# Ulixes-8/UNet-Implementations

Measured on NVIDIA B200. Metric: our_unet_512_train_images_per_sec, higher is better.
Workload: dtype bf16

## Files before the change

### include/b200unet.h

```cpp
#ifndef B200UNET_H_
#define B200UNET_H_

#include <stdint.h>

#ifdef __cplusplus
extern "C" {
#endif

#define B200UNET_VERSION 100

int b200unet_version(void);
const char* b200unet_last_error(void);
long long b200unet_launch_count(void);
int b200unet_device_ok(void);
int b200unet_set_reserved_sms(int n);
int b200unet_set_pdl(int on);

typedef struct {
  const void* x;
  int64_t x_pitch;
  const void* w;
  void* y;
  int64_t y_pitch;
  float* stats;
  int N, H, W, Cin, Cout, stride;
} b200unet_conv_fprop_args;
int b200unet_conv_fprop_partials(int N, int OH, int OW, int Cout);
int b200unet_conv_fprop(const b200unet_conv_fprop_args* a, void* stream);

typedef struct {
  const void* dy;
  int64_t dy_pitch;
  const void* wt;
  void* dx;
  int64_t dx_pitch;
  int N, H, W, Cin, Cout, stride;
  const void* bs_y;
  int64_t bs_y_pitch;
  const float* bs_a;
  const float* bs_b;
  float bs_slope;
  float* bs_part;
  void* dx2;
  int64_t dx2_pitch;
  int dx_split;
} b200unet_conv_dgrad_args;
int b200unet_conv_dgrad(const b200unet_conv_dgrad_args* a, void* stream);
int b200unet_conv_dgrad_bwd_slots(int N, int H, int W, int Cin, int Cout, int stride);

typedef struct {
  const void* x;
  int64_t x_pitch;
  const void* dy;
  int64_t dy_pitch;
  float* dw;
  float* workspace;
  int64_t workspace_bytes;
  int N, H, W, Cin, Cout, stride;
} b200unet_conv_wgrad_args;
int64_t b200unet_conv_wgrad_workspace(int N, int H, int W, int Cin, int Cout, int stride);
int b200unet_conv_wgrad(const b200unet_conv_wgrad_args* a, void* stream);

int b200unet_conv_fprop_simt_partials(int OH, int OW);
int b200unet_conv_fprop_simt(const b200unet_conv_fprop_args* a, void* stream);
int b200unet_conv_dgrad_simt(const b200unet_conv_dgrad_args* a, void* stream);
int b200unet_conv_wgrad_simt(const b200unet_conv_wgrad_args* a, void* stream);

int b200unet_pack_conv_weights(const float* w_oihw, void* w_fprop, void* w_dgrad, int Cout, int Cin, void* stream);

int b200unet_stem_partials(int H, int W);
int b200unet_stem_fprop(const float* img_nchw, const float* w_oihw, void* y, int64_t y_pitch, float* stats, int N,
                        int H, int W, void* stream);
int64_t b200unet_stem_wgrad_workspace(int N, int H, int W);
int b200unet_stem_wgrad(const float* img_nchw, const void* dy, int64_t dy_pitch, float* dw_oihw, float* workspace,
                        int64_t workspace_bytes, int N, int H, int W, void* stream);

int b200unet_in_finalize(const float* stats, int P, const float* gamma, const float* beta, const float* drop_scale,
                         float eps, float* mean, float* rstd, float* a, float* b, int N, int C, int64_t HW,
                         void* stream);
int b200unet_in_apply(const void* y, int64_t y_pitch, const float* a, const float* b, float slope, void* z,
                      int64_t z_pitch, int N, int64_t HW, int C, void* stream);
typedef struct {
  const void* dz;
  int64_t dz_pitch;
  const void* dz2;
  int64_t dz2_pitch;
  const void* y;
  int64_t y_pitch;
  const float* a;
  const float* b;
  const float* mean;
  const float* rstd;
  const float* drop_scale;
  const float* gamma;
  float slope;
  void* dy;
  int64_t dy_pitch;
  float* dgamma;
  float* dbeta;
  float* workspace;
  int64_t workspace_bytes;
  int N;
  int64_t HW;
  int C;
  const float* ext_part;
  int ext_P;
  const float* ext_part2;
  int ext_P2;
  int defer_params;
} b200unet_in_bwd_args;
int64_t b200unet_in_backward_workspace(int N, int64_t HW, int C);
int b200unet_in_backward(const b200unet_in_bwd_args* a, void* stream);
int b200unet_in_bwd_params(const float* workspace, int N, int64_t HW, int C, float* dgamma, float* dbeta, void* stream);

int b200unet_upsample2x_fwd(const void* x, int64_t x_pitch, void* out, int64_t out_pitch, int N, int H, int W, int C,
                            void* stream);
int b200unet_upsample2x_bwd(const void* dout, int64_t dout_pitch, void* dx, int64_t dx_pitch, int N, int H, int W,
                            int C, void* stream);

int b200unet_head_fwd(const void* z, int64_t z_pitch, const float* w, const float* bias, float* logits_nchw, int N,
                      int64_t HW, int C, int K, void* stream);
int64_t b200unet_head_bwd_workspace(int N, int64_t HW, int C, int K);
int b200unet_head_bwd(const float* dlogits_nchw, const void* z, int64_t z_pitch, const float* w, void* dz,
                      int64_t dz_pitch, float* dw, float* db, float* workspace, int64_t workspace_bytes, int N,
                      int64_t HW, int C, int K, void* stream);

int64_t b200unet_loss_workspace(int N, int64_t HW);
int b200unet_loss_fwd(const float* logits_nchw, const int64_t* target, const float* class_weights, int dynamic,
                      float weight_ce, float weight_dice, int ignore_index, float smooth, float* loss_out,
                      float* tables, float* workspace, int64_t workspace_bytes, int N, int64_t HW, void* stream);
int b200unet_loss_bwd(const float* logits_nchw, const int64_t* target, const float* tables, const float* grad_out,
                      float weight_ce, float weight_dice, int ignore_index, float* dlogits_nchw, int N, int64_t HW,
                      void* stream);
int b200unet_loss_fwd_u8(const float* logits_nchw, const uint8_t* target, const float* class_weights, int dynamic,
                         float weight_ce, float weight_dice, int ignore_index, float smooth, float* loss_out,
                         float* tables, float* workspace, int64_t workspace_bytes, int N, int64_t HW, void* stream);
int b200unet_loss_bwd_u8(const float* logits_nchw, const uint8_t* target, const float* tables, const float* grad_out,
                         float weight_ce, float weight_dice, int ignore_index, float* dlogits_nchw, int N, int64_t HW,
                         void* stream);

int b200unet_nchw_f32_to_nhwc_bf16(const float* src, void* dst, int64_t dst_pitch, int N, int C, int64_t HW,
                                   void* stream);
int b200unet_nhwc_bf16_to_nchw_f32(const void* src, int64_t src_pitch, float* dst, int N, int C, int64_t HW,
                                   void* stream);

int b200unet_conv_dgrad_s2_supported(int Cin, int Cout);
int b200unet_pack_s2_dgrad_weights(const void* wt, void* ws, int Cin, int Cout, void* stream);
int b200unet_conv_dgrad_s2(const b200unet_conv_dgrad_args* a, void* stream);

int b200unet_upsample2x_norm_fwd(const void* y, int64_t y_pitch, const float* a, const float* b, float slope, void* out,
                                 int64_t out_pitch, int N, int H, int W, int C, void* stream);
int b200unet_head_norm_fwd(const void* y, int64_t y_pitch, const float* a, const float* b, float slope, const float* w,
                           const float* bias, float* logits_nchw, int N, int64_t HW, int C, int K, void* stream);
int b200unet_head_norm_bwd(const float* dlogits_nchw, const void* y, int64_t y_pitch, const float* a, const float* b,
                           float slope, const float* w, void* dz, int64_t dz_pitch, float* dw, float* db,
                           float* workspace, int64_t workspace_bytes, int N, int64_t HW, int C, int K, void* stream);
int b200unet_head_bwd_stat_slots(int N, int64_t HW);
int b200unet_head_norm_bwd_stats(const float* dlogits_nchw, const void* y, int64_t y_pitch, const float* a, const float* b,
                                 float slope, const float* w, void* dz, int64_t dz_pitch, float* dw, float* db,
                                 float* workspace, int64_t workspace_bytes, float* bwd_part, int N, int64_t HW, int C, int K,
                                 void* stream);
int b200unet_head_norm_bwd_stats_f32(const float* dlogits_nchw, const void* y, int64_t y_pitch, const float* a,
                                     const float* b, float slope, const float* w, void* dz, int64_t dz_pitch, float* dw,
                                     float* db, float* workspace, int64_t workspace_bytes, float* bwd_part, int N,
                                     int64_t HW, int C, int K, void* stream);
int b200unet_upsample2x_norm_fwd_f32(const void* y, int64_t y_pitch, const float* a, const float* b, float slope,
                                     void* out, int64_t out_pitch, int N, int H, int W, int C, void* stream);
int b200unet_head_norm_fwd_f32(const void* y, int64_t y_pitch, const float* a, const float* b, float slope,
                               const float* w, const float* bias, float* logits_nchw, int N, int64_t HW, int C, int K,
                               void* stream);
int b200unet_head_norm_bwd_f32(const float* dlogits_nchw, const void* y, int64_t y_pitch, const float* a, const float* b,
                               float slope, const float* w, void* dz, int64_t dz_pitch, float* dw, float* db,
                               float* workspace, int64_t workspace_bytes, int N, int64_t HW, int C, int K, void* stream);

int b200unet_pack_conv_weights_f32(const float* w_oihw, void* w_fprop, void* w_dgrad, int Cout, int Cin, void* stream);
int b200unet_conv_fprop_f32(const b200unet_conv_fprop_args* a, void* stream);
int b200unet_conv_dgrad_f32(const b200unet_conv_dgrad_args* a, void* stream);
int b200unet_conv_wgrad_f32(const b200unet_conv_wgrad_args* a, void* stream);
int b200unet_in_apply_f32(const void* y, int64_t y_pitch, const float* a, const float* b, float slope, void* z,
                          int64_t z_pitch, int N, int64_t HW, int C, void* stream);
int b200unet_in_backward_f32(const b200unet_in_bwd_args* a, void* stream);
int b200unet_upsample2x_fwd_f32(const void* x, int64_t x_pitch, void* out, int64_t out_pitch, int N, int H, int W,
                                int C, void* stream);
int b200unet_upsample2x_bwd_f32(const void* dout, int64_t dout_pitch, void* dx, int64_t dx_pitch, int N, int H,
                                int W, int C, void* stream);
int b200unet_head_fwd_f32(const void* z, int64_t z_pitch, const float* w, const float* bias, float* logits_nchw,
                          int N, int64_t HW, int C, int K, void* stream);
int b200unet_head_bwd_f32(const float* dlogits_nchw, const void* z, int64_t z_pitch, const float* w, void* dz,
                          int64_t dz_pitch, float* dw, float* db, float* workspace, int64_t workspace_bytes, int N,
                          int64_t HW, int C, int K, void* stream);
int b200unet_nchw_f32_to_nhwc_f32(const float* src, void* dst, int64_t dst_pitch, int N, int C, int64_t HW,
                                  void* stream);

int b200unet_image_to_nhwc32_bf16(const float* src, void* dst, int N, int C, int64_t HW, void* stream);

int b200unet_preprocess_u8(const void* image_u8_nhwc, const void* mask_u8, float* image_out_nchw, int64_t* mask_out,
                           const float* mean3, const float* std3, int N, int64_t HW, void* stream);
int b200unet_preprocess_u8_nhwc32(const void* image_u8_nhwc, void* dst_nhwc32, const float* mean3, const float* std3, int N,
                                  int64_t HW, void* stream);
int b200unet_sgd_max_tensors(void);
int b200unet_sgd_nesterov_step(float* const* params, const float* const* grads, float* const* momentum_bufs,
                               const int64_t* numels, int count, float lr, float momentum, float weight_decay,
                               int nesterov, int first_step, void* stream);
typedef struct {
  int64_t offset;
  int32_t numel;
  int32_t flags;
  int32_t first_block;
  int32_t cout, cin, ksize;
  int32_t cout_pad, cin_pad;
  void* wf;
  void* wd;
  void* ws;
} b200unet_flat_tensor;
int b200unet_sgd_flat_block_elems(void);
int b200unet_sgd_flat_step(const b200unet_flat_tensor* table_dev, int count, int total_blocks, float* master,
                           const float* grad, float* momentum_buf, float lr, float momentum, float weight_decay,
                           int nesterov, float grad_scale, const float* lr_dev ,
                           void* stream);
int b200unet_adam_flat_step(const b200unet_flat_tensor* table_dev, int count, int total_blocks, float* master,
                            const float* grad, float* exp_avg, float* exp_avg_sq, float* steps, float* scalars_ws,
                            double lr, const double* lr_dev, double beta1, double beta2, double eps, double weight_decay,
                            int decoupled, float grad_scale, void* stream);
int b200unet_argmax_counts(const float* logits_nchw, const int64_t* target, int ignore_index, int64_t* pred_or_null,
                           int64_t* counts9, int N, int64_t HW, void* stream);

int b200unet_recon_head_fwd(const void* y, int64_t y_pitch, const float* bias, float* out_nchw, int N, int64_t HW,
                            int K, void* stream);
int b200unet_recon_head_fwd_f32(const void* y, int64_t y_pitch, const float* bias, float* out_nchw, int N, int64_t HW,
                                int K, void* stream);
int64_t b200unet_recon_head_bwd_workspace(int N, int64_t HW);
int b200unet_recon_head_bwd(const float* dout_nchw, const float* out_nchw, void* dpre, int64_t dpre_pitch, int Cpad,
                            float* db, float* workspace, int64_t workspace_bytes, int N, int64_t HW, int K,
                            void* stream);
int b200unet_recon_head_bwd_f32(const float* dout_nchw, const float* out_nchw, void* dpre, int64_t dpre_pitch, int Cpad,
                                float* db, float* workspace, int64_t workspace_bytes, int N, int64_t HW, int K,
                                void* stream);
int64_t b200unet_mse_workspace(int64_t n);
int b200unet_mse_fwd(const float* a, const float* b, float* loss_out, float* workspace, int64_t workspace_bytes,
                     int64_t n, void* stream);
int b200unet_mse_bwd(const float* a, const float* b, const float* grad_out, float* da, int64_t n, void* stream);

#ifdef __cplusplus
}
#endif
#endif
```

### unet-implementations_b200/_lib.py

```python
from __future__ import annotations

import ctypes
import os
from ctypes import POINTER, Structure, c_char_p, c_double, c_float, c_int, c_int64, c_void_p

_HERE = os.path.dirname(os.path.abspath(__file__))
LIB_PATH = os.environ.get("B200UNET_LIB") or os.path.join(_HERE, "libb200unet.so")

_lib = None


class ConvFpropArgs(Structure):
    _fields_ = [
        ("x", c_void_p), ("x_pitch", c_int64), ("w", c_void_p), ("y", c_void_p), ("y_pitch", c_int64),
        ("stats", c_void_p), ("N", c_int), ("H", c_int), ("W", c_int), ("Cin", c_int), ("Cout", c_int),
        ("stride", c_int),
    ]


class ConvDgradArgs(Structure):
    _fields_ = [
        ("dy", c_void_p), ("dy_pitch", c_int64), ("wt", c_void_p), ("dx", c_void_p), ("dx_pitch", c_int64),
        ("N", c_int), ("H", c_int), ("W", c_int), ("Cin", c_int), ("Cout", c_int), ("stride", c_int),
        ("bs_y", c_void_p), ("bs_y_pitch", c_int64), ("bs_a", c_void_p), ("bs_b", c_void_p), ("bs_slope", c_float),
        ("bs_part", c_void_p), ("dx2", c_void_p), ("dx2_pitch", c_int64), ("dx_split", c_int),
    ]


class ConvWgradArgs(Structure):
    _fields_ = [
        ("x", c_void_p), ("x_pitch", c_int64), ("dy", c_void_p), ("dy_pitch", c_int64), ("dw", c_void_p),
        ("workspace", c_void_p), ("workspace_bytes", c_int64), ("N", c_int), ("H", c_int), ("W", c_int),
        ("Cin", c_int), ("Cout", c_int), ("stride", c_int),
    ]


class InBwdArgs(Structure):
    _fields_ = [
        ("dz", c_void_p), ("dz_pitch", c_int64), ("dz2", c_void_p), ("dz2_pitch", c_int64), ("y", c_void_p),
        ("y_pitch", c_int64), ("a", c_void_p), ("b", c_void_p), ("mean", c_void_p), ("rstd", c_void_p),
        ("drop_scale", c_void_p), ("gamma", c_void_p), ("slope", c_float), ("dy", c_void_p), ("dy_pitch", c_int64),
        ("dgamma", c_void_p), ("dbeta", c_void_p), ("workspace", c_void_p), ("workspace_bytes", c_int64),
        ("N", c_int), ("HW", c_int64), ("C", c_int),
        ("ext_part", c_void_p), ("ext_P", c_int), ("ext_part2", c_void_p), ("ext_P2", c_int), ("defer_params", c_int),
    ]


class FlatTensor(Structure):
    _fields_ = [
        ("offset", c_int64), ("numel", c_int), ("flags", c_int), ("first_block", c_int), ("cout", c_int), ("cin", c_int),
        ("ksize", c_int), ("cout_pad", c_int), ("cin_pad", c_int), ("wf", c_void_p), ("wd", c_void_p), ("ws", c_void_p),
    ]


_P, _I, _L, _F, _D = c_void_p, c_int, c_int64, c_float, c_double

SIGNATURES = {
    "b200unet_version": (c_int, []),
    "b200unet_last_error": (c_char_p, []),
    "b200unet_device_ok": (c_int, []),
    "b200unet_set_reserved_sms": (c_int, [_I]),
    "b200unet_set_pdl": (c_int, [_I]),
    "b200unet_launch_count": (c_int64, []),
    "b200unet_conv_fprop_partials": (c_int, [_I, _I, _I, _I]),
    "b200unet_conv_fprop": (c_int, [POINTER(ConvFpropArgs), _P]),
    "b200unet_conv_dgrad": (c_int, [POINTER(ConvDgradArgs), _P]),
    "b200unet_conv_dgrad_bwd_slots": (c_int, [_I, _I, _I, _I, _I, _I]),
    "b200unet_conv_dgrad_s2_supported": (c_int, [_I, _I]),
    "b200unet_pack_s2_dgrad_weights": (c_int, [_P, _P, _I, _I, _P]),
    "b200unet_conv_dgrad_s2": (c_int, [POINTER(ConvDgradArgs), _P]),
    "b200unet_conv_wgrad_workspace": (c_int64, [_I, _I, _I, _I, _I, _I]),
    "b200unet_conv_wgrad": (c_int, [POINTER(ConvWgradArgs), _P]),
    "b200unet_conv_fprop_simt_partials": (c_int, [_I, _I]),
    "b200unet_conv_fprop_simt": (c_int, [POINTER(ConvFpropArgs), _P]),
    "b200unet_conv_dgrad_simt": (c_int, [POINTER(ConvDgradArgs), _P]),
    "b200unet_conv_wgrad_simt": (c_int, [POINTER(ConvWgradArgs), _P]),
    "b200unet_pack_conv_weights": (c_int, [_P, _P, _P, _I, _I, _P]),
    "b200unet_stem_partials": (c_int, [_I, _I]),
    "b200unet_stem_fprop": (c_int, [_P, _P, _P, _L, _P, _I, _I, _I, _P]),
    "b200unet_stem_wgrad_workspace": (c_int64, [_I, _I, _I]),
    "b200unet_stem_wgrad": (c_int, [_P, _P, _L, _P, _P, _L, _I, _I, _I, _P]),
    "b200unet_in_finalize": (c_int, [_P, _I, _P, _P, _P, _F, _P, _P, _P, _P, _I, _I, _L, _P]),
    "b200unet_in_apply": (c_int, [_P, _L, _P, _P, _F, _P, _L, _I, _L, _I, _P]),
    "b200unet_in_backward_workspace": (c_int64, [_I, _L, _I]),
    "b200unet_in_backward": (c_int, [POINTER(InBwdArgs), _P]),
    "b200unet_in_bwd_params": (c_int, [_P, _I, _L, _I, _P, _P, _P]),
    "b200unet_upsample2x_fwd": (c_int, [_P, _L, _P, _L, _I, _I, _I, _I, _P]),
    "b200unet_upsample2x_bwd": (c_int, [_P, _L, _P, _L, _I, _I, _I, _I, _P]),
    "b200unet_head_fwd": (c_int, [_P, _L, _P, _P, _P, _I, _L, _I, _I, _P]),
    "b200unet_head_bwd_workspace": (c_int64, [_I, _L, _I, _I]),
    "b200unet_head_bwd": (c_int, [_P, _P, _L, _P, _P, _L, _P, _P, _P, _L, _I, _L, _I, _I, _P]),
    "b200unet_loss_workspace": (c_int64, [_I, _L]),
    "b200unet_loss_fwd": (c_int, [_P, _P, _P, _I, _F, _F, _I, _F, _P, _P, _P, _L, _I, _L, _P]),
    "b200unet_loss_bwd": (c_int, [_P, _P, _P, _P, _F, _F, _I, _P, _I, _L, _P]),
    "b200unet_loss_fwd_u8": (c_int, [_P, _P, _P, _I, _F, _F, _I, _F, _P, _P, _P, _L, _I, _L, _P]),
    "b200unet_loss_bwd_u8": (c_int, [_P, _P, _P, _P, _F, _F, _I, _P, _I, _L, _P]),
    "b200unet_nchw_f32_to_nhwc_bf16": (c_int, [_P, _P, _L, _I, _I, _L, _P]),
    "b200unet_nhwc_bf16_to_nchw_f32": (c_int, [_P, _L, _P, _I, _I, _L, _P]),
    "b200unet_pack_conv_weights_f32": (c_int, [_P, _P, _P, _I, _I, _P]),
    "b200unet_conv_fprop_f32": (c_int, [POINTER(ConvFpropArgs), _P]),
    "b200unet_conv_dgrad_f32": (c_int, [POINTER(ConvDgradArgs), _P]),
    "b200unet_conv_wgrad_f32": (c_int, [POINTER(ConvWgradArgs), _P]),
    "b200unet_in_apply_f32": (c_int, [_P, _L, _P, _P, _F, _P, _L, _I, _L, _I, _P]),
    "b200unet_in_backward_f32": (c_int, [POINTER(InBwdArgs), _P]),
    "b200unet_upsample2x_fwd_f32": (c_int, [_P, _L, _P, _L, _I, _I, _I, _I, _P]),
    "b200unet_upsample2x_bwd_f32": (c_int, [_P, _L, _P, _L, _I, _I, _I, _I, _P]),
    "b200unet_head_fwd_f32": (c_int, [_P, _L, _P, _P, _P, _I, _L, _I, _I, _P]),
    "b200unet_head_bwd_f32": (c_int, [_P, _P, _L, _P, _P, _L, _P, _P, _P, _L, _I, _L, _I, _I, _P]),
    "b200unet_nchw_f32_to_nhwc_f32": (c_int, [_P, _P, _L, _I, _I, _L, _P]),
    "b200unet_image_to_nhwc32_bf16": (c_int, [_P, _P, _I, _I, _L, _P]),
    "b200unet_upsample2x_norm_fwd": (c_int, [_P, _L, _P, _P, _F, _P, _L, _I, _I, _I, _I, _P]),
    "b200unet_upsample2x_norm_fwd_f32": (c_int, [_P, _L, _P, _P, _F, _P, _L, _I, _I, _I, _I, _P]),
    "b200unet_head_norm_fwd": (c_int, [_P, _L, _P, _P, _F, _P, _P, _P, _I, _L, _I, _I, _P]),
    "b200unet_head_norm_fwd_f32": (c_int, [_P, _L, _P, _P, _F, _P, _P, _P, _I, _L, _I, _I, _P]),
    "b200unet_head_norm_bwd": (c_int, [_P, _P, _L, _P, _P, _F, _P, _P, _L, _P, _P, _P, _L, _I, _L, _I, _I, _P]),
    "b200unet_head_norm_bwd_f32": (c_int, [_P, _P, _L, _P, _P, _F, _P, _P, _L, _P, _P, _P, _L, _I, _L, _I, _I, _P]),
    "b200unet_head_bwd_stat_slots": (c_int, [_I, _L]),
    "b200unet_head_norm_bwd_stats": (c_int, [_P, _P, _L, _P, _P, _F, _P, _P, _L, _P, _P, _P, _L, _P, _I, _L, _I, _I, _P]),
    "b200unet_head_norm_bwd_stats_f32": (c_int, [_P, _P, _L, _P, _P, _F, _P, _P, _L, _P, _P, _P, _L, _P, _I, _L, _I, _I, _P]),
    "b200unet_preprocess_u8": (c_int, [_P, _P, _P, _P, _P, _P, _I, _L, _P]),
    "b200unet_preprocess_u8_nhwc32": (c_int, [_P, _P, _P, _P, _I, _L, _P]),
    "b200unet_sgd_flat_block_elems": (c_int, []),
    "b200unet_sgd_flat_step": (c_int, [_P, _I, _I, _P, _P, _P, _F, _F, _F, _I, _F, _P, _P]),
    "b200unet_sgd_max_tensors": (c_int, []),
    "b200unet_sgd_nesterov_step": (c_int, [_P, _P, _P, _P, _I, _F, _F, _F, _I, _I, _P]),
    "b200unet_adam_flat_step": (c_int, [_P, _I, _I, _P, _P, _P, _P, _P, _P, _D, _P, _D, _D, _D, _D, _I, _F, _P]),
    "b200unet_argmax_counts": (c_int, [_P, _P, _I, _P, _P, _I, _L, _P]),
    "b200unet_recon_head_fwd": (c_int, [_P, _L, _P, _P, _I, _L, _I, _P]),
    "b200unet_recon_head_fwd_f32": (c_int, [_P, _L, _P, _P, _I, _L, _I, _P]),
    "b200unet_recon_head_bwd_workspace": (c_int64, [_I, _L]),
    "b200unet_recon_head_bwd": (c_int, [_P, _P, _P, _L, _I, _P, _P, _L, _I, _L, _I, _P]),
    "b200unet_recon_head_bwd_f32": (c_int, [_P, _P, _P, _L, _I, _P, _P, _L, _I, _L, _I, _P]),
    "b200unet_mse_workspace": (c_int64, [_L]),
    "b200unet_mse_fwd": (c_int, [_P, _P, _P, _P, _L, _L, _P]),
    "b200unet_mse_bwd": (c_int, [_P, _P, _P, _P, _L, _P]),
}

_VALUE_FUNCS = {
    "b200unet_version", "b200unet_last_error", "b200unet_device_ok", "b200unet_set_reserved_sms", "b200unet_set_pdl", "b200unet_launch_count", "b200unet_conv_fprop_partials",
    "b200unet_conv_fprop_simt_partials", "b200unet_sgd_max_tensors", "b200unet_sgd_flat_block_elems", "b200unet_head_bwd_stat_slots", "b200unet_conv_dgrad_bwd_slots", "b200unet_recon_head_bwd_workspace",
    "b200unet_conv_dgrad_s2_supported",
    "b200unet_mse_workspace",
    "b200unet_conv_wgrad_workspace", "b200unet_stem_partials", "b200unet_stem_wgrad_workspace",
    "b200unet_in_backward_workspace", "b200unet_head_bwd_workspace", "b200unet_loss_workspace",
}


def load():
    global _lib
    if _lib is not None:
        return _lib
    if not os.path.exists(LIB_PATH):
        raise RuntimeError(
            f"b200unet: {LIB_PATH} is not built. Run `python -c 'import __graft_entry__ as g; g.build()'` "
            "(or `make -C unet-implementations_b200/csrc`). There is no CPU or PyTorch fallback."
        )
    lib = ctypes.CDLL(LIB_PATH)
    for name, (res, args) in SIGNATURES.items():
        fn = getattr(lib, name)
        fn.restype = res
        fn.argtypes = args
    _lib = lib
    return lib


def last_error() -> str:
    msg = load().b200unet_last_error()
    return msg.decode("utf-8", "replace") if msg else ""


class EventProfiler:

    def __init__(self):
        self.pairs = {}

    def totals_ms(self):
        return {k: (sum(a.elapsed_time(b) for a, b in v), len(v)) for k, v in self.pairs.items()}


PROFILER = None


def call(name: str, *args):
    fn = getattr(load(), name)
    prof = PROFILER
    if prof is not None and name not in _VALUE_FUNCS:
        import torch
        e0 = torch.cuda.Event(enable_timing=True)
        e1 = torch.cuda.Event(enable_timing=True)
        e0.record()
        rc = fn(*args)
        e1.record()
        prof.pairs.setdefault(name, []).append((e0, e1))
    else:
        rc = fn(*args)
    if name in _VALUE_FUNCS:
        return rc
    if rc != 0:
        raise RuntimeError(f"{name} failed ({rc}): {last_error()}")
    return 0
```

### unet-implementations_b200/csrc/head_loss.cu

```cuda
#include "common.cuh"
#include "ptx.cuh"
#include "vec8.cuh"

namespace b200 {

constexpr int kNC = 3;
constexpr int kLossThreads = 256;
constexpr int kLossPxPerThread = 8;
constexpr int kLossVals = 4 * kNC;

__device__ __forceinline__ float block_sum(float v, float* scratch) {
#pragma unroll
  for (int o = 16; o > 0; o >>= 1) v += __shfl_xor_sync(0xffffffffu, v, o);
  const int lane = threadIdx.x & 31, warp = threadIdx.x >> 5;
  __syncthreads();
  if (lane == 0) scratch[warp] = v;
  __syncthreads();
  float s = 0.f;
  if (threadIdx.x == 0)
    for (int w = 0; w < (blockDim.x >> 5); ++w) s += scratch[w];
  return s;
}

template <typename TT>
// ... 19 lines not shown
  } else {
#pragma unroll
    for (int j = 0; j < 4; ++j) {
      const bool in = px + j < HW;
#pragma unroll
      for (int c = 0; c < 3; ++c) a[c][j] = in ? z0[c * HW + px + j] : 0.f;
      long long q = in ? static_cast<long long>(tg[px + j]) : -1;
      t[j] = (q < -(1ll << 30) || q > (1ll << 30)) ? (1 << 30) + 1 : static_cast<int>(q);
      if (!in) t[j] = -2;
    }
  }
}

template <typename TT>
__global__ void __launch_bounds__(kLossThreads) loss_fwd_kernel(const float* __restrict__ logits,
                                                                 const TT* __restrict__ target, int ignore_index,
                                                                 float* __restrict__ part, int64_t HW) {
  pdl_launch_dependents();
  pdl_wait();
  __shared__ float scratch[kLossThreads / 32][kLossVals];
  const int n = blockIdx.y;
  const float* z0 = logits + static_cast<int64_t>(n) * kNC * HW;
  const TT* tg = target + static_cast<int64_t>(n) * HW;
  const bool vec = (HW & 3) == 0;
  float acc[kLossVals];
#pragma unroll
  for (int i = 0; i < kLossVals; ++i) acc[i] = 0.f;
  const int64_t base = static_cast<int64_t>(blockIdx.x) * kLossThreads * kLossPxPerThread;
  constexpr int kIters = kLossPxPerThread / 4;
  float a[kIters][3][4];
  int t[kIters][4];
  bool live[kIters];
#pragma unroll
  for (int k = 0; k < kIters; ++k) {
    const int64_t px = base + (static_cast<int64_t>(k) * kLossThreads + threadIdx.x) * 4;
    live[k] = px < HW;
    if (live[k]) load_px4<TT>(z0, tg, HW, px, vec, a[k], t[k]);
  }
#pragma unroll
  for (int k = 0; k < kIters; ++k) {
    if (!live[k]) continue;
    const int64_t px = base + (static_cast<int64_t>(k) * kLossThreads + threadIdx.x) * 4;
#pragma unroll
    for (int j = 0; j < 4; ++j) {
      const int tj = t[k][j];
      if (tj == ignore_index || (!vec && px + j >= HW)) continue;
      const float a0 = a[k][0][j], a1 = a[k][1][j], a2 = a[k][2][j];
      const float m = fmaxf(a0, fmaxf(a1, a2));
      const float e0 = expf(a0 - m), e1 = expf(a1 - m), e2 = expf(a2 - m);
      const float se = e0 + e1 + e2;
      const float inv = 1.f / se;
      const float p0 = e0 * inv, p1 = e1 * inv, p2 = e2 * inv;
      const float lse = m + logf(se);
      acc[9] += p0;
      acc[10] += p1;
      acc[11] += p2;
      if (tj == 0) { acc[0] += 1.f; acc[3] += lse - a0; acc[6] += p0; }
      else if (tj == 1) { acc[1] += 1.f; acc[4] += lse - a1; acc[7] += p1; }
      else if (tj == 2) { acc[2] += 1.f; acc[5] += lse - a2; acc[8] += p2; }
    }
  }
  const int lane = threadIdx.x & 31, warp = threadIdx.x >> 5;
#pragma unroll
  for (int i = 0; i < kLossVals; ++i) {
    float v = acc[i];
#pragma unroll
    for (int o = 16; o > 0; o >>= 1) v += __shfl_xor_sync(0xffffffffu, v, o);
    if (lane == 0) scratch[warp][i] = v;
  }
  __syncthreads();
  if (threadIdx.x < kLossVals) {
    float s = 0.f;
#pragma unroll
    for (int w = 0; w < kLossThreads / 32; ++w) s += scratch[w][threadIdx.x];
    part[(static_cast<int64_t>(n) * gridDim.x + blockIdx.x) * kLossVals + threadIdx.x] = s;
  }
}

__global__ void loss_finalize_kernel(const float* __restrict__ part, int blocks, const float* __restrict__ class_w,
                                     int dynamic, float weight_ce, float weight_dice, float smooth,
                                     float* __restrict__ loss_out, float* __restrict__ tables, int N) {
  pdl_launch_dependents();
  pdl_wait();
  extern __shared__ double sred[];
  double* dterm = sred + N * kLossVals;
  const int lane = threadIdx.x & 31, warp = threadIdx.x >> 5, nwarps = blockDim.x >> 5;
  constexpr int UV = 4;
  const int total = N * kLossVals;
  for (int i = warp * UV; i < total; i += nwarps * UV) {
    double s[UV];
    const float* src[UV];
#pragma unroll
    for (int u = 0; u < UV; ++u) {
      const int iu = min(i + u, total - 1);
      const int b = iu / kLossVals, v = iu - b * kLossVals;
      src[u] = part + static_cast<int64_t>(b) * blocks * kLossVals + v;
      s[u] = 0.0;
    }
    for (int k = lane; k < blocks; k += 32) {
      float x[UV];
#pragma unroll
      for (int u = 0; u < UV; ++u) x[u] = src[u][static_cast<int64_t>(k) * kLossVals];
#pragma unroll
      for (int u = 0; u < UV; ++u) s[u] += x[u];
    }
#pragma unroll
    for (int u = 0; u < UV; ++u) {
#pragma unroll
      for (int o = 16; o > 0; o >>= 1) s[u] += __shfl_xor_sync(0xffffffffu, s[u], o);
      if (lane == 0 && i + u < total) sred[i + u] = s[u];
    }
  }
  __syncthreads();
  if (threadIdx.x < N * kNC) {
    const int b = threadIdx.x / kNC, c = threadIdx.x - b * kNC;
    const double T = sred[b * kLossVals + c];
    const double I = sred[b * kLossVals + 2 * kNC + c];
    const double Pc = sred[b * kLossVals + 3 * kNC + c];
    const double U = Pc + T + smooth;
    const double two_i = 2.0 * I + smooth;
    dterm[b * kNC + c] = two_i / U;
    tables[kNC + (b * 2 + 0) * kNC + c] = static_cast<float>(-(2.0 / (kNC * static_cast<double>(N))) / U);
    tables[kNC + (b * 2 + 1) * kNC + c] = static_cast<float>((1.0 / (kNC * static_cast<double>(N))) * two_i / (U * U));
  }
  __syncthreads();
  if (threadIdx.x != 0) return;
  double cnt[kNC] = {0, 0, 0}, S[kNC] = {0, 0, 0};
  for (int b = 0; b < N; ++b)
    for (int c = 0; c < kNC; ++c) {
      cnt[c] += sred[b * kLossVals + c];
      S[c] += sred[b * kLossVals + kNC + c];
    }
  float w[kNC];
  if (class_w && !dynamic) {
    for (int c = 0; c < kNC; ++c) w[c] = class_w[c];
  } else if (dynamic) {
    const float total = static_cast<float>(cnt[0] + cnt[1] + cnt[2]);
    float wsum = 0.f;
    for (int c = 0; c < kNC; ++c) {
      const float px = cnt[c] == 0.0 ? 1.f : static_cast<float>(cnt[c]);
      w[c] = total / px;
      wsum += w[c];
    }
    for (int c = 0; c < kNC; ++c) w[c] = w[c] * (static_cast<float>(kNC) / wsum);
  } else {
    for (int c = 0; c < kNC; ++c) w[c] = 1.f;
  }
  double num = 0.0, den = 0.0;
  for (int c = 0; c < kNC; ++c) {
    num += static_cast<double>(w[c]) * S[c];
    den += static_cast<double>(w[c]) * cnt[c];
  }
  const double ce = num / den;
  double dice_loss = 0.0;
  for (int c = 0; c < kNC; ++c) {
    double dsum = 0.0;
    for (int b = 0; b < N; ++b) dsum += dterm[b * kNC + c];
    dice_loss += 1.0 - dsum / N;
  }
  dice_loss /= kNC;
  for (int c = 0; c < kNC; ++c) tables[c] = static_cast<float>(w[c] / den);
  loss_out[0] = static_cast<float>(weight_ce * ce + weight_dice * dice_loss);
  loss_out[1] = static_cast<float>(ce);
  loss_out[2] = static_cast<float>(dice_loss);
}

template <typename TT>
__global__ void __launch_bounds__(kLossThreads) loss_bwd_kernel(const float* __restrict__ logits,
                                                                 const TT* __restrict__ target,
                                                                 const float* __restrict__ tables,
                                                                 const float* __restrict__ grad_out, float weight_ce,
                                                                 float weight_dice, int ignore_index,
                                                                 float* __restrict__ dlogits, int64_t HW) {
  pdl_launch_dependents();
  pdl_wait();
  const int n = blockIdx.y;
  const float gs = grad_out ? grad_out[0] : 1.f;
  const float wn0 = tables[0], wn1 = tables[1], wn2 = tables[2];
  const float* tb = tables + kNC + n * 2 * kNC;
  const float A0 = tb[0], A1 = tb[1], A2 = tb[2], B0 = tb[3], B1 = tb[4], B2 = tb[5];
  const float* z0 = logits + static_cast<int64_t>(n) * kNC * HW;
  float* d0 = dlogits + static_cast<int64_t>(n) * kNC * HW;
  const TT* tg = target + static_cast<int64_t>(n) * HW;
  const bool vec = (HW & 3) == 0;
  const int64_t base = static_cast<int64_t>(blockIdx.x) * kLossThreads * kLossPxPerThread;
  constexpr int kIters = kLossPxPerThread / 4;
  float a[kIters][3][4];
  int t[kIters][4];
  bool live[kIters];
#pragma unroll
  for (int k = 0; k < kIters; ++k) {
    const int64_t px = base + (static_cast<int64_t>(k) * kLossThreads + threadIdx.x) * 4;
    live[k] = px < HW;
    if (live[k]) load_px4<TT>(z0, tg, HW, px, vec, a[k], t[k]);
  }
#pragma unroll
  for (int k = 0; k < kIters; ++k) {
    if (!live[k]) continue;
    const int64_t px = base + (static_cast<int64_t>(k) * kLossThreads + threadIdx.x) * 4;
    float g[3][4];
#pragma unroll
    for (int j = 0; j < 4; ++j) {
      const int tj = t[k][j];
      float g0 = 0.f, g1 = 0.f, g2 = 0.f;
      if (tj != ignore_index) {
        const float a0 = a[k][0][j], a1 = a[k][1][j], a2 = a[k][2][j];
        const float m = fmaxf(a0, fmaxf(a1, a2));
        const float e0 = expf(a0 - m), e1 = expf(a1 - m), e2 = expf(a2 - m);
        const float inv = 1.f / (e0 + e1 + e2);
        const float p0 = e0 * inv, p1 = e1 * inv, p2 = e2 * inv;
        const float wt = tj == 0 ? wn0 : (tj == 1 ? wn1 : (tj == 2 ? wn2 : 0.f));
        const float G0 = B0 + (tj == 0 ? A0 : 0.f), G1 = B1 + (tj == 1 ? A1 : 0.f), G2 = B2 + (tj == 2 ? A2 : 0.f);
        const float gp = G0 * p0 + G1 * p1 + G2 * p2;
        g0 = weight_ce * wt * (p0 - (tj == 0 ? 1.f : 0.f)) + weight_dice * p0 * (G0 - gp);
        g1 = weight_ce * wt * (p1 - (tj == 1 ? 1.f : 0.f)) + weight_dice * p1 * (G1 - gp);
        g2 = weight_ce * wt * (p2 - (tj == 2 ? 1.f : 0.f)) + weight_dice * p2 * (G2 - gp);
      }
      g[0][j] = g0 * gs;
      g[1][j] = g1 * gs;
      g[2][j] = g2 * gs;
    }
    if (vec) {
#pragma unroll
      for (int c = 0; c < 3; ++c)
        *reinterpret_cast<float4*>(d0 + c * HW + px) = make_float4(g[c][0], g[c][1], g[c][2], g[c][3]);
    } else {
#pragma unroll
      for (int j = 0; j < 4; ++j)
        if (px + j < HW) {
          d0[px + j] = g[0][j];
          d0[HW + px + j] = g[1][j];
          d0[2 * HW + px + j] = g[2][j];
        }
    }
  }
}

constexpr int kHeadMaxC = 64;
constexpr int kHeadMaxK = 4;

template <typename T, int C, int K>
__global__ void __launch_bounds__(256) head_fwd_kernel(const T* __restrict__ z, int64_t zp,
                                                        const float* __restrict__ w, const float* __restrict__ bias,
                                                        float* __restrict__ logits, int64_t HW,
                                                        const float* __restrict__ na, const float* __restrict__ nb,
                                                        float slope) {
  pdl_launch_dependents();
  pdl_wait();
  constexpr int C8N = C / 8, L = 256 / C8N, kPix = 4;
  static_assert(C8N >= K && C8N <= 32 && (C8N & (C8N - 1)) == 0, "C/8 must be a power of two in [K, 32]");
  const int n = blockIdx.y;
  const int c8 = threadIdx.x % C8N, c0 = c8 * 8;
  float wr[K][8], av[8], bv[8];
#pragma unroll
  for (int k = 0; k < K; ++k)
#pragma unroll
    for (int i = 0; i < 8; ++i) wr[k][i] = __ldg(w + k * C + c0 + i);
  if (na) {
#pragma unroll
    for (int i = 0; i < 8; ++i) {
      av[i] = __ldg(na + n * C + c0 + i);
      bv[i] = __ldg(nb + n * C + c0 + i);
    }
  }
  const float my_bias = c8 < K ? __ldg(bias + c8) : 0.f;
  const T* zn = z + static_cast<int64_t>(n) * HW * zp + c0;
  float* ln = logits + static_cast<int64_t>(n) * K * HW;
  const int64_t base = static_cast<int64_t>(blockIdx.x) * (L * kPix) + threadIdx.x / C8N;
  Vec8<T> v[kPix];
#pragma unroll
  for (int u = 0; u < kPix; ++u)
    if (base + u * L < HW) v[u] = Vec8<T>::ld_stream(zn + (base + u * L) * zp);
#pragma unroll
  for (int u = 0; u < kPix; ++u) {
    const int64_t px = base + u * L;
    if (px >= HW) break;
    float zf[8], acc[K];
    v[u].unpack(zf);
    if (na) {
#pragma unroll
      for (int i = 0; i < 8; ++i) {
        const float t = fmaf(av[i], zf[i], bv[i]);
        zf[i] = t > 0.f ? t : t * slope;
      }
    }
#pragma unroll
    for (int k = 0; k < K; ++k) {
      float a = 0.f;
#pragma unroll
      for (int i = 0; i < 8; ++i) a = fmaf(wr[k][i], zf[i], a);
      acc[k] = a;
    }
#pragma unroll
    for (int m = 1; m < C8N; m <<= 1)
#pragma unroll
      for (int k = 0; k < K; ++k) acc[k] += __shfl_xor_sync(0xffffffffu, acc[k], m);
    float mine = acc[0];
#pragma unroll
    for (int k = 1; k < K; ++k) mine = c8 == k ? acc[k] : mine;
    if (c8 < K) ln[c8 * HW + px] = mine + my_bias;
  }
}

template <typename T, int C, int K, bool STATS>
__global__ void __launch_bounds__(256, sizeof(T) == 2 ? 2 : 1) head_bwd_kernel(const float* __restrict__ dl, const T* __restrict__ z,
                                                        int64_t zp, const float* __restrict__ w,
                                                        T* __restrict__ dz, int64_t dzp,
                                                        float* __restrict__ partial, int64_t HW,
                                                        const float* __restrict__ na, const float* __restrict__ nb,
                                                        float slope, float* __restrict__ tpart) {
  pdl_launch_dependents();
  pdl_wait();
  constexpr int C8N = C / 8;
  constexpr int L = 256 / C8N;
  static_assert(C8N >= 1 && C8N <= 32 && (C8N & (C8N - 1)) == 0, "C/8 must be a power of two <= 32");
  __shared__ float red[8][K * C + K + (STATS ? 2 * C : 0)];
  const int n = blockIdx.y;
  const int c8 = threadIdx.x % C8N, c0 = c8 * 8;
  float wr[K][8];
#pragma unroll
  for (int k = 0; k < K; ++k)
#pragma unroll
    for (int i = 0; i < 8; ++i) wr[k][i] = w[k * C + c0 + i];
  float av[8], bv[8];
  if (na) {
    const float4 a0 = __ldg(reinterpret_cast<const float4*>(na + n * C + c0)), a1 = __ldg(reinterpret_cast<const float4*>(na + n * C + c0) + 1);
    const float4 b0 = __ldg(reinterpret_cast<const float4*>(nb + n * C + c0)), b1 = __ldg(reinterpret_cast<const float4*>(nb + n * C + c0) + 1);
    av[0] = a0.x; av[1] = a0.y; av[2] = a0.z; av[3] = a0.w; av[4] = a1.x; av[5] = a1.y; av[6] = a1.z; av[7] = a1.w;
    bv[0] = b0.x; bv[1] = b0.y; bv[2] = b0.z; bv[3] = b0.w; bv[4] = b1.x; bv[5] = b1.y; bv[6] = b1.z; bv[7] = b1.w;
  }
  float aw[K][8], ab[K], t1[STATS ? 8 : 1], t2[STATS ? 8 : 1];
#pragma unroll
  for (int k = 0; k < K; ++k) {
    ab[k] = 0.f;
#pragma unroll
    for (int i = 0; i < 8; ++i) aw[k][i] = 0.f;
  }
#pragma unroll
  for (int i = 0; i < (STATS ? 8 : 1); ++i) t1[i] = t2[i] = 0.f;
  const float* dln = dl + static_cast<int64_t>(n) * K * HW;
  const T* zn = z + static_cast<int64_t>(n) * HW * zp + c0;
  T* dzn = dz + static_cast<int64_t>(n) * HW * dzp + c0;
  const int64_t stride = static_cast<int64_t>(gridDim.x) * L;
  constexpr int U = STATS ? 3 : 4;
  for (int64_t g0 = static_cast<int64_t>(blockIdx.x) * L + threadIdx.x / C8N; g0 < HW; g0 += U * stride) {
    float d[U][K];
    Vec8<T> zv[U];
#pragma unroll
    for (int u = 0; u < U; ++u) {
      const int64_t px = g0 + u * stride;
      if (px < HW) {
#pragma unroll
        for (int k = 0; k < K; ++k) d[u][k] = __ldg(dln + k * HW + px);
        zv[u] = Vec8<T>::ld_stream(zn + px * zp);
      }
    }
#pragma unroll
    for (int u = 0; u < U; ++u) {
      const int64_t px = g0 + u * stride;
      if (px >= HW) break;
      float zf[8], o[8];
      zv[u].unpack(zf);
#pragma unroll
      for (int k = 0; k < K; ++k) ab[k] += d[u][k];
#pragma unroll
      for (int i = 0; i < 8; ++i) {
        const float yraw = zf[i];
        float zact = yraw, sl = 1.f;
        if (na) {
          const float t = fmaf(av[i], yraw, bv[i]);
          sl = t > 0.f ? 1.f : slope;
          zact = t * sl;
        }
        float sacc = 0.f;
#pragma unroll
        for (int k = 0; k < K; ++k) {
          sacc = fmaf(wr[k][i], d[u][k], sacc);
          aw[k][i] = fmaf(d[u][k], zact, aw[k][i]);
        }
        o[i] = sacc;
        if (STATS) {
          const float gm = to_f32(from_f32<T>(sacc)) * sl;
          t1[i] += gm;
          t2[i] = fmaf(gm, yraw, t2[i]);
        }
      }
      Vec8<T>::st(dzn + px * dzp, o);
    }
  }
  const int lane = threadIdx.x & 31, warp = threadIdx.x >> 5;
#pragma unroll
  for (int m = C8N; m < 32; m <<= 1) {
#pragma unroll
    for (int k = 0; k < K; ++k) {
#pragma unroll
      for (int i = 0; i < 8; ++i) aw[k][i] += __shfl_xor_sync(0xffffffffu, aw[k][i], m);
      ab[k] += __shfl_xor_sync(0xffffffffu, ab[k], m);
    }
    if (STATS) {
#pragma unroll
      for (int i = 0; i < 8; ++i) {
        t1[i] += __shfl_xor_sync(0xffffffffu, t1[i], m);
        t2[i] += __shfl_xor_sync(0xffffffffu, t2[i], m);
      }
    }
  }
  if (lane < C8N) {
#pragma unroll
    for (int k = 0; k < K; ++k) {
#pragma unroll
      for (int i = 0; i < 8; ++i) red[warp][k * C + c0 + i] = aw[k][i];
      if (c8 == 0) red[warp][K * C + k] = ab[k];
    }
    if (STATS) {
#pragma unroll
      for (int i = 0; i < 8; ++i) {
        red[warp][K * C + K + 2 * (c0 + i)] = t1[i];
        red[warp][K * C + K + 2 * (c0 + i) + 1] = t2[i];
      }
    }
  }
  __syncthreads();
  const int64_t row = static_cast<int64_t>(n) * gridDim.x + blockIdx.x;
  for (int i = threadIdx.x; i < K * C + K + (STATS ? 2 * C : 0); i += 256) {
    float sacc = 0.f;
#pragma unroll
    for (int wv = 0; wv < 8; ++wv) sacc += red[wv][i];
    if (i < K * C + K) partial[row * (K * C + K) + i] = sacc;
    else tpart[row * (2 * C) + (i - (K * C + K))] = sacc;
  }
}

__global__ void __launch_bounds__(1024) head_bwd_finalize_kernel(const float* __restrict__ partial, int blocks, int KC,
                                                                  int K, float* __restrict__ dw, float* __restrict__ db) {
  pdl_launch_dependents();
  pdl_wait();
  const int lane = threadIdx.x & 31, warp = threadIdx.x >> 5;
  for (int i = warp; i < KC + K; i += 32) {
    double s = 0.0;
    for (int b = lane; b < blocks; b += 32) s += partial[static_cast<int64_t>(b) * (KC + K) + i];
#pragma unroll
    for (int o = 16; o > 0; o >>= 1) s += __shfl_xor_sync(0xffffffffu, s, o);
    if (lane == 0) {
      if (i < KC) dw[i] = static_cast<float>(s);
      else db[i - KC] = static_cast<float>(s);
    }
  }
}

template <typename T>
__global__ void __launch_bounds__(256) recon_head_fwd_kernel(const T* __restrict__ y, int64_t yp,
                                                              const float* __restrict__ bias, float* __restrict__ out,
                                                              int64_t HW, int K) {
  const int n = blockIdx.y;
  const int64_t px = static_cast<int64_t>(blockIdx.x) * 256 + threadIdx.x;
  if (px >= HW) return;
  const T* src = y + (static_cast<int64_t>(n) * HW + px) * yp;
  for (int k = 0; k < K; ++k) {
    const float v = to_f32(src[k]) + bias[k];
    out[(static_cast<int64_t>(n) * K + k) * HW + px] = 1.f / (1.f + expf(-v));
  }
}

template <typename T>
__global__ void __launch_bounds__(256) recon_head_bwd_kernel(const float* __restrict__ dout, const float* __restrict__ out,
                                                              T* __restrict__ dpre, int64_t dp, int Cpad,
                                                              float* __restrict__ partial, int64_t HW, int K) {
  __shared__ float scratch[8];
  const int n = blockIdx.y;
  float acc[4] = {0.f, 0.f, 0.f, 0.f};
  const int vecs = Cpad * static_cast<int>(sizeof(T)) / 16;
  for (int64_t px = static_cast<int64_t>(blockIdx.x) * 256 + threadIdx.x; px < HW; px += static_cast<int64_t>(gridDim.x) * 256) {
    float g[4] = {0.f, 0.f, 0.f, 0.f};
#pragma unroll
    for (int k = 0; k < 4; ++k)
      if (k < K) {
        const int64_t i = (static_cast<int64_t>(n) * K + k) * HW + px;
        const float o = __ldg(out + i);
        g[k] = __ldg(dout + i) * o * (1.f - o);
        acc[k] += g[k];
      }
    uint4* dst = reinterpret_cast<uint4*>(dpre + (static_cast<int64_t>(n) * HW + px) * dp);
    if (sizeof(T) == 2) {
      dst[0] = make_uint4(pack_bf16x2(g[0], g[1]), pack_bf16x2(g[2], g[3]), 0u, 0u);
    } else {
      dst[0] = make_uint4(__float_as_uint(g[0]), __float_as_uint(g[1]), __float_as_uint(g[2]), __float_as_uint(g[3]));
    }
    const uint4 z = make_uint4(0u, 0u, 0u, 0u);
    for (int v = 1; v < vecs; ++v) dst[v] = z;
  }
  for (int k = 0; k < K && k < 4; ++k) {
    const float v = block_sum(acc[k], scratch);
    if (threadIdx.x == 0) partial[(static_cast<int64_t>(n) * gridDim.x + blockIdx.x) * 4 + k] = v;
  }
}

__global__ void recon_head_bwd_finalize_kernel(const float* __restrict__ partial, int rows, int K, float* __restrict__ db) {
  const int k = threadIdx.x;
  if (k >= K) return;
  double s = 0.0;
  for (int r = 0; r < rows; ++r) s += partial[static_cast<int64_t>(r) * 4 + k];
  db[k] = static_cast<float>(s);
}

__global__ void __launch_bounds__(256) mse_fwd_kernel(const float* __restrict__ a, const float* __restrict__ b,
                                                       float* __restrict__ partial, int64_t n) {
  __shared__ float scratch[8];
  float acc = 0.f;
  for (int64_t i = static_cast<int64_t>(blockIdx.x) * 256 + threadIdx.x; i < n; i += static_cast<int64_t>(gridDim.x) * 256) {
    const float d = a[i] - b[i];
    acc = fmaf(d, d, acc);
  }
  const float v = block_sum(acc, scratch);
  if (threadIdx.x == 0) partial[blockIdx.x] = v;
}
__global__ void mse_finalize_kernel(const float* __restrict__ partial, int blocks, double inv_n, float* __restrict__ out) {
  if (threadIdx.x != 0) return;
  double s = 0.0;
  for (int i = 0; i < blocks; ++i) s += partial[i];
  out[0] = static_cast<float>(s * inv_n);
}
__global__ void __launch_bounds__(256) mse_bwd_kernel(const float* __restrict__ a, const float* __restrict__ b,
                                                       const float* __restrict__ gout, float scale,
                                                       float* __restrict__ da, int64_t n) {
  const float g = (gout ? gout[0] : 1.f) * scale;
  for (int64_t i = static_cast<int64_t>(blockIdx.x) * 256 + threadIdx.x; i < n; i += static_cast<int64_t>(gridDim.x) * 256)
    da[i] = g * (a[i] - b[i]);
}



}

using namespace b200;

extern "C" int64_t b200unet_loss_workspace(int N, int64_t HW) {
  const int64_t blocks = ceil_div64(HW, kLossThreads * kLossPxPerThread);
  return static_cast<int64_t>(N) * blocks * kLossVals * 4;
}

template <typename TT>
static int loss_fwd_impl(const float* logits_nchw, const TT* target, const float* class_weights, int dynamic,
                         float weight_ce, float weight_dice, int ignore_index, float smooth, float* loss_out,
                         float* tables, float* workspace, int64_t workspace_bytes, int N, int64_t HW, void* stream) {
  B200_CHECK_ARG(logits_nchw && target && loss_out && tables && workspace, "loss_fwd: null pointer");
  B200_CHECK_ARG(N > 0 && HW > 0, "loss_fwd: empty batch");
  B200_CHECK_ARG(workspace_bytes >= b200unet_loss_workspace(N, HW), "loss_fwd: workspace too small");
  const int blocks = static_cast<int>(ceil_div64(HW, kLossThreads * kLossPxPerThread));
  cudaStream_t st = static_cast<cudaStream_t>(stream);
  launch_k(loss_fwd_kernel<TT>, dim3(blocks, N), dim3(kLossThreads), 0, st, logits_nchw, target, ignore_index, workspace, HW);
  B200_LAUNCH_CHECK("loss_fwd_kernel");
  const size_t smem = static_cast<size_t>(N) * (kLossVals + kNC) * sizeof(double);
  B200_CHECK_ARG(N * kNC <= 1024, "loss_fwd: batch %d too large for the finalize kernel", N);
  B200_CHECK_ARG(smem <= 48 * 1024, "loss_fwd: batch %d too large for the finalize kernel", N);
  launch_k(loss_finalize_kernel, dim3(1), dim3(1024), smem, st, workspace, blocks, class_weights, dynamic, weight_ce, weight_dice, smooth,
                                             loss_out, tables, N);
  B200_LAUNCH_CHECK("loss_finalize_kernel");
  return 0;
}

template <typename TT>
static int loss_bwd_impl(const float* logits_nchw, const TT* target, const float* tables, const float* grad_out,
                         float weight_ce, float weight_dice, int ignore_index, float* dlogits_nchw, int N, int64_t HW,
                         void* stream) {
  B200_CHECK_ARG(logits_nchw && target && tables && dlogits_nchw, "loss_bwd: null pointer");
  const int blocks = static_cast<int>(ceil_div64(HW, kLossThreads * kLossPxPerThread));
  launch_k(loss_bwd_kernel<TT>, dim3(blocks, N), dim3(kLossThreads), 0, static_cast<cudaStream_t>(stream), 
      logits_nchw, target, tables, grad_out, weight_ce, weight_dice, ignore_index, dlogits_nchw, HW);
  B200_LAUNCH_CHECK("loss_bwd_kernel");
  return 0;
}

extern "C" int b200unet_loss_fwd(const float* logits_nchw, const int64_t* target, const float* class_weights,
                                 int dynamic, float weight_ce, float weight_dice, int ignore_index, float smooth,
                                 float* loss_out, float* tables, float* workspace, int64_t workspace_bytes, int N,
                                 int64_t HW, void* stream) {
  return loss_fwd_impl<int64_t>(logits_nchw, target, class_weights, dynamic, weight_ce, weight_dice, ignore_index, smooth,
                                loss_out, tables, workspace, workspace_bytes, N, HW, stream);
}
extern "C" int b200unet_loss_fwd_u8(const float* logits_nchw, const uint8_t* target, const float* class_weights,
                                    int dynamic, float weight_ce, float weight_dice, int ignore_index, float smooth,
                                    float* loss_out, float* tables, float* workspace, int64_t workspace_bytes, int N,
                                    int64_t HW, void* stream) {
  return loss_fwd_impl<uint8_t>(logits_nchw, target, class_weights, dynamic, weight_ce, weight_dice, ignore_index, smooth,
                                loss_out, tables, workspace, workspace_bytes, N, HW, stream);
}

extern "C" int b200unet_loss_bwd(const float* logits_nchw, const int64_t* target, const float* tables,
                                 const float* grad_out, float weight_ce, float weight_dice, int ignore_index,
                                 float* dlogits_nchw, int N, int64_t HW, void* stream) {
  return loss_bwd_impl<int64_t>(logits_nchw, target, tables, grad_out, weight_ce, weight_dice, ignore_index, dlogits_nchw,
                                N, HW, stream);
}
extern "C" int b200unet_loss_bwd_u8(const float* logits_nchw, const uint8_t* target, const float* tables,
                                    const float* grad_out, float weight_ce, float weight_dice, int ignore_index,
                                    float* dlogits_nchw, int N, int64_t HW, void* stream) {
  return loss_bwd_impl<uint8_t>(logits_nchw, target, tables, grad_out, weight_ce, weight_dice, ignore_index, dlogits_nchw,
                                N, HW, stream);
}

template <typename T>
static int head_fwd_impl(const void* z, int64_t z_pitch, const float* w, const float* bias, float* logits_nchw, int N,
                         int64_t HW, int C, int K, void* stream, const float* na = nullptr, const float* nb = nullptr,
                         float slope = 0.f) {
  B200_CHECK_ARG(z && w && bias && logits_nchw, "head_fwd: null pointer");
  B200_CHECK_ARG(z_pitch % 8 == 0, "head_fwd: pitch must be a multiple of 8");
  if (!(C == 32 && K == 3)) return set_error(kErrUnsupported, "head_fwd: only C=32, K=3 is built (got C=%d K=%d)", C, K);
  dim3 grid((unsigned)ceil_div64(HW, 256), N);
  launch_k(head_fwd_kernel<T, 32, 3>, dim3(grid), dim3(256), 0, static_cast<cudaStream_t>(stream), static_cast<const T*>(z), z_pitch, w,
                                                                                  bias, logits_nchw, HW, na, nb, slope);
  B200_LAUNCH_CHECK("head_fwd_kernel");
  return 0;
}
extern "C" int b200unet_head_fwd(const void* z, int64_t z_pitch, const float* w, const float* bias, float* logits_nchw,
                                 int N, int64_t HW, int C, int K, void* stream) {
  return head_fwd_impl<__nv_bfloat16>(z, z_pitch, w, bias, logits_nchw, N, HW, C, K, stream);
}
extern "C" int b200unet_head_fwd_f32(const void* z, int64_t z_pitch, const float* w, const float* bias,
                                     float* logits_nchw, int N, int64_t HW, int C, int K, void* stream) {
  return head_fwd_impl<float>(z, z_pitch, w, bias, logits_nchw, N, HW, C, K, stream);
}

extern "C" int b200unet_head_bwd_stat_slots(int N, int64_t HW) {
  if (N <= 0 || HW <= 0) return 0;
  int64_t per = (static_cast<int64_t>(num_sms()) * 2) / N;
  const int64_t mx = ceil_div64(HW, 64);
  if (per > mx) per = mx;
  return static_cast<int>(per < 1 ? 1 : per);
}

extern "C" int64_t b200unet_head_bwd_workspace(int N, int64_t HW, int C, int K) {
  return static_cast<int64_t>(b200unet_head_bwd_stat_slots(N, HW)) * N * (K * C + K) * 4;
}

template <typename T>
static int head_bwd_impl(const float* dlogits_nchw, const void* z, int64_t z_pitch, const float* w, void* dz,
                         int64_t dz_pitch, float* dw, float* db, float* workspace, int64_t workspace_bytes, int N,
                         int64_t HW, int C, int K, void* stream, const float* na = nullptr, const float* nb = nullptr,
                         float slope = 0.f, float* tpart = nullptr) {
  B200_CHECK_ARG(dlogits_nchw && z && w && dz && dw && db && workspace, "head_bwd: null pointer");
  B200_CHECK_ARG(z_pitch % 8 == 0 && dz_pitch % 8 == 0, "head_bwd: pitches must be multiples of 8");
  B200_CHECK_ARG(N > 0 && N <= 65535, "head_bwd: batch must fit the grid");
  if (!(C == 32 && K == 3)) return set_error(kErrUnsupported, "head_bwd: only C=32, K=3 is built (got C=%d K=%d)", C, K);
  B200_CHECK_ARG(!tpart || (na && nb), "head_bwd: the norm-backward partial sums need the fused producer (a, b)");
  const int bpi = b200unet_head_bwd_stat_slots(N, HW);
  B200_CHECK_ARG(workspace_bytes >= b200unet_head_bwd_workspace(N, HW, C, K), "head_bwd: workspace too small");
  cudaStream_t st = static_cast<cudaStream_t>(stream);
  if (tpart)
    launch_k(head_bwd_kernel<T, 32, 3, true>, dim3(bpi, N), dim3(256), 0, st, dlogits_nchw, static_cast<const T*>(z), z_pitch, w,
                                                                  static_cast<T*>(dz), dz_pitch, workspace, HW, na, nb,
                                                                  slope, tpart);
  else
    launch_k(head_bwd_kernel<T, 32, 3, false>, dim3(bpi, N), dim3(256), 0, st, dlogits_nchw, static_cast<const T*>(z), z_pitch, w,
                                                                   static_cast<T*>(dz), dz_pitch, workspace, HW, na, nb,
                                                                   slope, nullptr);
  B200_LAUNCH_CHECK("head_bwd_kernel");
  launch_k(head_bwd_finalize_kernel, dim3(1), dim3(1024), 0, st, workspace, bpi * N, K * C, K, dw, db);
  B200_LAUNCH_CHECK("head_bwd_finalize_kernel");
  return 0;
}

extern "C" int b200unet_head_bwd(const float* dlogits_nchw, const void* z, int64_t z_pitch, const float* w, void* dz,
                                 int64_t dz_pitch, float* dw, float* db, float* workspace, int64_t workspace_bytes,
                                 int N, int64_t HW, int C, int K, void* stream) {
  return head_bwd_impl<__nv_bfloat16>(dlogits_nchw, z, z_pitch, w, dz, dz_pitch, dw, db, workspace, workspace_bytes, N,
                                      HW, C, K, stream);
}
extern "C" int b200unet_head_bwd_f32(const float* dlogits_nchw, const void* z, int64_t z_pitch, const float* w,
                                     void* dz, int64_t dz_pitch, float* dw, float* db, float* workspace,
                                     int64_t workspace_bytes, int N, int64_t HW, int C, int K, void* stream) {
  return head_bwd_impl<float>(dlogits_nchw, z, z_pitch, w, dz, dz_pitch, dw, db, workspace, workspace_bytes, N, HW, C,
                              K, stream);
}

static int recon_blocks(int64_t HW, int N) {
  int64_t per = ceil_div64(static_cast<int64_t>(num_sms()) * 8, N);
  const int64_t mx = ceil_div64(HW, 256);
  if (per > mx) per = mx;
  return static_cast<int>(per < 1 ? 1 : per);
}

template <typename T>
static int recon_head_fwd_impl(const void* y, int64_t y_pitch, const float* bias, float* out_nchw, int N, int64_t HW,
                               int K, void* stream) {
  B200_CHECK_ARG(y && bias && out_nchw, "recon_head_fwd: null pointer");
  B200_CHECK_ARG(K >= 1 && K <= 4 && y_pitch >= K && N <= 65535, "recon_head_fwd: K must be in [1,4]");
  recon_head_fwd_kernel<T><<<dim3((unsigned)ceil_div64(HW, 256), N), 256, 0, static_cast<cudaStream_t>(stream)>>>(
      static_cast<const T*>(y), y_pitch, bias, out_nchw, HW, K);
  B200_LAUNCH_CHECK("recon_head_fwd_kernel");
  return 0;
}
extern "C" int b200unet_recon_head_fwd(const void* y, int64_t y_pitch, const float* bias, float* out_nchw, int N,
                                       int64_t HW, int K, void* stream) {
  return recon_head_fwd_impl<__nv_bfloat16>(y, y_pitch, bias, out_nchw, N, HW, K, stream);
}
extern "C" int b200unet_recon_head_fwd_f32(const void* y, int64_t y_pitch, const float* bias, float* out_nchw, int N,
                                           int64_t HW, int K, void* stream) {
  return recon_head_fwd_impl<float>(y, y_pitch, bias, out_nchw, N, HW, K, stream);
}

extern "C" int64_t b200unet_recon_head_bwd_workspace(int N, int64_t HW) {
  return static_cast<int64_t>(N) * recon_blocks(HW, N) * 4 * 4;
}

template <typename T>
static int recon_head_bwd_impl(const float* dout_nchw, const float* out_nchw, void* dpre, int64_t dpre_pitch, int Cpad,
                               float* db, float* workspace, int64_t workspace_bytes, int N, int64_t HW, int K,
                               void* stream) {
  B200_CHECK_ARG(dout_nchw && out_nchw && dpre && db && workspace, "recon_head_bwd: null pointer");
  B200_CHECK_ARG(K >= 1 && K <= 4 && Cpad >= K && dpre_pitch >= Cpad && N <= 65535, "recon_head_bwd: bad channel counts");
  B200_CHECK_ARG(Cpad % 8 == 0 && dpre_pitch % 8 == 0 && (reinterpret_cast<uintptr_t>(dpre) & 15) == 0,
                 "recon_head_bwd: Cpad and the pitch must be multiples of 8, dpre 16-byte aligned");
  B200_CHECK_ARG(workspace_bytes >= b200unet_recon_head_bwd_workspace(N, HW), "recon_head_bwd: workspace too small");
  cudaStream_t st = static_cast<cudaStream_t>(stream);
  const int blocks = recon_blocks(HW, N);
  recon_head_bwd_kernel<T><<<dim3(blocks, N), 256, 0, st>>>(dout_nchw, out_nchw, static_cast<T*>(dpre), dpre_pitch, Cpad,
                                                            workspace, HW, K);
  B200_LAUNCH_CHECK("recon_head_bwd_kernel");
  recon_head_bwd_finalize_kernel<<<1, 32, 0, st>>>(workspace, N * blocks, K, db);
  B200_LAUNCH_CHECK("recon_head_bwd_finalize_kernel");
  return 0;
}
extern "C" int b200unet_recon_head_bwd(const float* dout_nchw, const float* out_nchw, void* dpre, int64_t dpre_pitch,
                                       int Cpad, float* db, float* workspace, int64_t workspace_bytes, int N, int64_t HW,
                                       int K, void* stream) {
  return recon_head_bwd_impl<__nv_bfloat16>(dout_nchw, out_nchw, dpre, dpre_pitch, Cpad, db, workspace, workspace_bytes,
                                            N, HW, K, stream);
}
extern "C" int b200unet_recon_head_bwd_f32(const float* dout_nchw, const float* out_nchw, void* dpre, int64_t dpre_pitch,
                                           int Cpad, float* db, float* workspace, int64_t workspace_bytes, int N,
                                           int64_t HW, int K, void* stream) {
  return recon_head_bwd_impl<float>(dout_nchw, out_nchw, dpre, dpre_pitch, Cpad, db, workspace, workspace_bytes, N, HW,
                                    K, stream);
}

static int mse_blocks(int64_t n) {
  const int64_t mx = ceil_div64(n, 256 * 8);
  const int64_t cap = static_cast<int64_t>(num_sms()) * 8;
  return static_cast<int>(mx < 1 ? 1 : (mx > cap ? cap : mx));
}
extern "C" int64_t b200unet_mse_workspace(int64_t n) { return static_cast<int64_t>(mse_blocks(n)) * 4; }

extern "C" int b200unet_mse_fwd(const float* a, const float* b, float* loss_out, float* workspace,
                                int64_t workspace_bytes, int64_t n, void* stream) {
  B200_CHECK_ARG(a && b && loss_out && workspace && n > 0, "mse_fwd: null pointer or empty input");
  B200_CHECK_ARG(workspace_bytes >= b200unet_mse_workspace(n), "mse_fwd: workspace too small");
  cudaStream_t st = static_cast<cudaStream_t>(stream);
  const int blocks = mse_blocks(n);
  mse_fwd_kernel<<<blocks, 256, 0, st>>>(a, b, workspace, n);
  B200_LAUNCH_CHECK("mse_fwd_kernel");
  mse_finalize_kernel<<<1, 32, 0, st>>>(workspace, blocks, 1.0 / static_cast<double>(n), loss_out);
  B200_LAUNCH_CHECK("mse_finalize_kernel");
  return 0;
}

extern "C" int b200unet_mse_bwd(const float* a, const float* b, const float* grad_out, float* da, int64_t n,
                                void* stream) {
  B200_CHECK_ARG(a && b && da && n > 0, "mse_bwd: null pointer or empty input");
  mse_bwd_kernel<<<mse_blocks(n), 256, 0, static_cast<cudaStream_t>(stream)>>>(a, b, grad_out,
                                                                               static_cast<float>(2.0 / static_cast<double>(n)), da, n);
  B200_LAUNCH_CHECK("mse_bwd_kernel");
  return 0;
}

extern "C" int b200unet_head_norm_fwd(const void* y, int64_t y_pitch, const float* a, const float* b, float slope,
                                      const float* w, const float* bias, float* logits_nchw, int N, int64_t HW, int C,
                                      int K, void* stream) {
  B200_CHECK_ARG(a && b, "head_norm_fwd: null affine");
  return head_fwd_impl<__nv_bfloat16>(y, y_pitch, w, bias, logits_nchw, N, HW, C, K, stream, a, b, slope);
}
extern "C" int b200unet_head_norm_fwd_f32(const void* y, int64_t y_pitch, const float* a, const float* b, float slope,
                                          const float* w, const float* bias, float* logits_nchw, int N, int64_t HW,
                                          int C, int K, void* stream) {
  B200_CHECK_ARG(a && b, "head_norm_fwd: null affine");
  return head_fwd_impl<float>(y, y_pitch, w, bias, logits_nchw, N, HW, C, K, stream, a, b, slope);
}
extern "C" int b200unet_head_norm_bwd(const float* dlogits_nchw, const void* y, int64_t y_pitch, const float* a,
                                      const float* b, float slope, const float* w, void* dz, int64_t dz_pitch, float* dw,
                                      float* db, float* workspace, int64_t workspace_bytes, int N, int64_t HW, int C,
                                      int K, void* stream) {
  B200_CHECK_ARG(a && b, "head_norm_bwd: null affine");
  return head_bwd_impl<__nv_bfloat16>(dlogits_nchw, y, y_pitch, w, dz, dz_pitch, dw, db, workspace, workspace_bytes, N,
                                      HW, C, K, stream, a, b, slope);
}
extern "C" int b200unet_head_norm_bwd_stats(const float* dlogits_nchw, const void* y, int64_t y_pitch, const float* a,
                                            const float* b, float slope, const float* w, void* dz, int64_t dz_pitch,
                                            float* dw, float* db, float* workspace, int64_t workspace_bytes,
                                            float* bwd_part, int N, int64_t HW, int C, int K, void* stream) {
  B200_CHECK_ARG(a && b && bwd_part, "head_norm_bwd_stats: null affine or partial buffer");
  return head_bwd_impl<__nv_bfloat16>(dlogits_nchw, y, y_pitch, w, dz, dz_pitch, dw, db, workspace, workspace_bytes, N,
                                      HW, C, K, stream, a, b, slope, bwd_part);
}
extern "C" int b200unet_head_norm_bwd_stats_f32(const float* dlogits_nchw, const void* y, int64_t y_pitch, const float* a,
                                                const float* b, float slope, const float* w, void* dz, int64_t dz_pitch,
                                                float* dw, float* db, float* workspace, int64_t workspace_bytes,
                                                float* bwd_part, int N, int64_t HW, int C, int K, void* stream) {
  B200_CHECK_ARG(a && b && bwd_part, "head_norm_bwd_stats: null affine or partial buffer");
  return head_bwd_impl<float>(dlogits_nchw, y, y_pitch, w, dz, dz_pitch, dw, db, workspace, workspace_bytes, N, HW, C, K,
                              stream, a, b, slope, bwd_part);
}
extern "C" int b200unet_head_norm_bwd_f32(const float* dlogits_nchw, const void* y, int64_t y_pitch, const float* a,
                                          const float* b, float slope, const float* w, void* dz, int64_t dz_pitch,
                                          float* dw, float* db, float* workspace, int64_t workspace_bytes, int N,
                                          int64_t HW, int C, int K, void* stream) {
  B200_CHECK_ARG(a && b, "head_norm_bwd: null affine");
  return head_bwd_impl<float>(dlogits_nchw, y, y_pitch, w, dz, dz_pitch, dw, db, workspace, workspace_bytes, N, HW, C, K,
                              stream, a, b, slope);
}
```

### unet-implementations_b200/csrc/norm.cu

```cuda
#include "common.cuh"
#include "ptx.cuh"
#include "vec8.cuh"
#include <stdlib.h>

namespace b200 {

constexpr int kNormThreads = 256;

struct PixelMap {
  int c8n;
  int threads;
  int lanes;
};
static PixelMap make_map(int C) {
  PixelMap m;
  m.c8n = C >> 3;
  m.lanes = kNormThreads / m.c8n;
  if (m.lanes < 1) m.lanes = 1;
  m.threads = m.lanes * m.c8n;
  return m;
}
static int blocks_per_sm() {
  static int v = 0;
  if (v == 0) {
    const char* e = getenv("B200UNET_NORM_BPS");
    v = e ? atoi(e) : 8;
    if (v < 1) v = 8;
  }
  return v;
}
static int64_t pixels_per_block(int64_t HW, int N, const PixelMap& m, int bps) {
  int64_t per_img = ceil_div64(static_cast<int64_t>(num_sms()) * bps, N);
  if (per_img < 1) per_img = 1;
  int64_t chunk = ceil_div64(HW, per_img);
  const int64_t q = static_cast<int64_t>(m.lanes) * 4;
  chunk = ceil_div64(chunk, q) * q;
  return chunk;
}

__device__ __forceinline__ void ld8f(const float* p, float (&f)[8]) {
  const float4 u = *reinterpret_cast<const float4*>(p);
  const float4 v = *reinterpret_cast<const float4*>(p + 4);
  f[0] = u.x; f[1] = u.y; f[2] = u.z; f[3] = u.w; f[4] = v.x; f[5] = v.y; f[6] = v.z; f[7] = v.w;
}

__global__ void __launch_bounds__(256) in_finalize_kernel(const float* __restrict__ stats, int P,
                                                           const float* __restrict__ gamma,
                                                           const float* __restrict__ beta,
                                                           const float* __restrict__ drop, float eps,
                                                           float* __restrict__ mean, float* __restrict__ rstd,
                                                           float* __restrict__ a, float* __restrict__ b, int C,
                                                           double inv_hw) {
  pdl_launch_dependents();
  pdl_wait();
  __shared__ double red[8][32][2];
  const int n = blockIdx.x;
  const int cl = threadIdx.x & 31, pg = threadIdx.x >> 5;
  const int c = blockIdx.y * 32 + cl;
  double s1 = 0.0, s2 = 0.0;
  if (c < C) {
    const float2* sp = reinterpret_cast<const float2*>(stats) + static_cast<int64_t>(n) * P * C + c;
    for (int p = pg; p < P; p += 32) {
      float2 v[4];
#pragma unroll
      for (int u = 0; u < 4; ++u)
        v[u] = (p + 8 * u < P) ? __ldg(sp + static_cast<int64_t>(p + 8 * u) * C) : make_float2(0.f, 0.f);
#pragma unroll
      for (int u = 0; u < 4; ++u) {
        s1 += v[u].x;
        s2 += v[u].y;
      }
    }
  }
  red[pg][cl][0] = s1;
  red[pg][cl][1] = s2;
  __syncthreads();
  if (pg != 0 || c >= C) return;
  s1 = s2 = 0.0;
#pragma unroll
  for (int k = 0; k < 8; ++k) {
    s1 += red[k][cl][0];
    s2 += red[k][cl][1];
  }
  const int i = n * C + c;
  const double m = s1 * inv_hw;
  double var = s2 * inv_hw - m * m;
  if (var < 0.0) var = 0.0;
  const double r = 1.0 / sqrt(var + static_cast<double>(eps));
  const float s = drop ? drop[i] : 1.f;
  const double gr = static_cast<double>(gamma[c]) * r;
  mean[i] = static_cast<float>(m);
  rstd[i] = static_cast<float>(r);
  a[i] = static_cast<float>(s * gr);
  b[i] = static_cast<float>(s * (static_cast<double>(beta[c]) - m * gr));
}

template <typename T>
__global__ void __launch_bounds__(kNormThreads) in_apply_kernel(const T* __restrict__ y, int64_t yp,
                                                                 const float* __restrict__ a,
                                                                 const float* __restrict__ b, float slope,
                                                                 T* __restrict__ z, int64_t zp, int64_t HW,
                                                                 int C, int c8n, int lanes, int64_t chunk) {
  pdl_launch_dependents();
  pdl_wait();
  const int n = gridDim.y - 1 - blockIdx.y;
  const int c0 = (threadIdx.x % c8n) << 3;
  const int lane = threadIdx.x / c8n;
  float ra[8], rb[8];
  ld8f(a + n * C + c0, ra);
  ld8f(b + n * C + c0, rb);
  const int64_t lo = blockIdx.x * chunk;
  int64_t hi = lo + chunk;
  if (hi > HW) hi = HW;
  const T* yb = y + static_cast<int64_t>(n) * HW * yp + c0;
  T* zb = z + static_cast<int64_t>(n) * HW * zp + c0;
  for (int64_t px = lo + lane; px < hi; px += 4 * lanes) {
    Vec8<T> v[4];
#pragma unroll
    for (int u = 0; u < 4; ++u)
      if (px + u * lanes < hi) v[u] = Vec8<T>::ld_stream(yb + (px + u * lanes) * yp);
#pragma unroll
    for (int u = 0; u < 4; ++u) {
      if (px + u * lanes >= hi) break;
      float f[8];
      v[u].unpack(f);
#pragma unroll
      for (int j = 0; j < 8; ++j) {
        const float t = fmaf(ra[j], f[j], rb[j]);
        f[j] = t > 0.f ? t : t * slope;
      }
      Vec8<T>::st(zb + (px + u * lanes) * zp, f);
    }
  }
}

template <typename T>
struct InBwdK {
  const T* dz;
  int64_t dzp;
  const T* dz2;
  int64_t dz2p;
  const T* y;
  int64_t yp;
  const float *a, *b, *mean;
  float slope;
  int64_t HW;
  int C, c8n, lanes;
  int64_t chunk;
  int n0;
};

template <typename T, bool HAS2>
__global__ void __launch_bounds__(kNormThreads, (HAS2 || sizeof(T) != 2) ? 2 : 3) in_bwd_reduce_kernel(InBwdK<T> K, float* __restrict__ part, int P) {
  pdl_launch_dependents();
  pdl_wait();
  using Acc = typename AccT<T>::type;
  extern __shared__ __align__(8) unsigned char red_raw[];
  Acc* red = reinterpret_cast<Acc*>(red_raw);
  const int n = K.n0 + (gridDim.y - 1 - blockIdx.y);
  const int c8 = threadIdx.x % K.c8n;
  const int c0 = c8 << 3;
  const int lane = threadIdx.x / K.c8n;
  float ra[8], rb[8], rm[8];
  ld8f(K.a + n * K.C + c0, ra);
  ld8f(K.b + n * K.C + c0, rb);
  ld8f(K.mean + n * K.C + c0, rm);
  Acc t1[8], t2[8];
#pragma unroll
  for (int j = 0; j < 8; ++j) t1[j] = t2[j] = 0;
  const int64_t lo = blockIdx.x * K.chunk;
  int64_t hi = lo + K.chunk;
  if (hi > K.HW) hi = K.HW;
  const T* yb = K.y + static_cast<int64_t>(n) * K.HW * K.yp + c0;
  const T* db = K.dz + static_cast<int64_t>(n) * K.HW * K.dzp + c0;
  const T* d2b = HAS2 ? K.dz2 + static_cast<int64_t>(n) * K.HW * K.dz2p + c0 : nullptr;
  const int lanes = K.lanes;
  constexpr int U = 4;
  for (int64_t px = lo + lane; px < hi; px += U * lanes) {
    Vec8<T> vy[U], vd[U], vd2[HAS2 ? U : 1];
#pragma unroll
    for (int u = 0; u < U; ++u)
      if (px + u * lanes < hi) {
        vy[u] = Vec8<T>::ld_stream(yb + (px + u * lanes) * K.yp);
        vd[u] = Vec8<T>::ld_stream(db + (px + u * lanes) * K.dzp);
        if (HAS2) vd2[HAS2 ? u : 0] = Vec8<T>::ld_stream(d2b + (px + u * lanes) * K.dz2p);
      }
#pragma unroll
    for (int u = 0; u < U; ++u) {
      if (px + u * lanes >= hi) break;
      float yv[8], d[8];
      vy[u].unpack(yv);
      vd[u].unpack(d);
      if (HAS2) {
        float d2[8];
        vd2[HAS2 ? u : 0].unpack(d2);
#pragma unroll
        for (int j = 0; j < 8; ++j) d[j] += d2[j];
      }
#pragma unroll
      for (int j = 0; j < 8; ++j) {
        const float pre = fmaf(ra[j], yv[j], rb[j]);
        const float gm = pre > 0.f ? d[j] : d[j] * K.slope;
        t1[j] += gm;
        t2[j] += static_cast<Acc>(gm) * static_cast<Acc>(yv[j] - rm[j]);
      }
    }
  }
  Acc* mine = red + static_cast<size_t>(threadIdx.x) * 16;
#pragma unroll
  for (int j = 0; j < 8; ++j) {
    mine[j] = t1[j];
    mine[8 + j] = t2[j];
  }
  __syncthreads();
  for (int t = threadIdx.x; t < K.C * 2; t += blockDim.x) {
    const int c = t >> 1, k = t & 1;
    const int cc8 = c >> 3, j = c & 7;
    Acc s = 0;
    for (int l = 0; l < lanes; ++l) s += red[(l * K.c8n + cc8) * 16 + k * 8 + j];
    part[((static_cast<int64_t>(n) * P + blockIdx.x) * K.C + c) * 2 + k] = static_cast<float>(s);
  }
}

__global__ void __launch_bounds__(256) in_bwd_finalize_kernel(const float* __restrict__ part, int P,
                                                               const float* __restrict__ part2, int P2,
                                                               const float* __restrict__ raw_mean,
                                                               const float* __restrict__ gamma,
                                                               const float* __restrict__ rstd,
                                                               const float* __restrict__ drop,
                                                               float* __restrict__ coef, float* __restrict__ imgsum,
                                                               int C, int n0, double inv_hw) {
  pdl_launch_dependents();
  pdl_wait();
  __shared__ double red[8][32][2];
  const int n = n0 + blockIdx.x;
  const int cl = threadIdx.x & 31, pg = threadIdx.x >> 5;
  const int c = blockIdx.y * 32 + cl;
  double t1 = 0.0, t2 = 0.0;
  if (c < C) {
    for (int set = 0; set < 2; ++set) {
      const float* pp = set ? part2 : part;
      const int PP = set ? P2 : P;
      if (!pp) continue;
      const float2* sp = reinterpret_cast<const float2*>(pp) + static_cast<int64_t>(n) * PP * C + c;
      for (int p = pg; p < PP; p += 32) {
        float2 v[4];
#pragma unroll
        for (int u = 0; u < 4; ++u)
          v[u] = (p + 8 * u < PP) ? sp[static_cast<int64_t>(p + 8 * u) * C] : make_float2(0.f, 0.f);
#pragma unroll
        for (int u = 0; u < 4; ++u) {
          t1 += v[u].x;
          t2 += v[u].y;
        }
      }
    }
  }
  red[pg][cl][0] = t1;
  red[pg][cl][1] = t2;
  __syncthreads();
  if (pg != 0 || c >= C) return;
  t1 = t2 = 0.0;
#pragma unroll
  for (int k = 0; k < 8; ++k) {
    t1 += red[k][cl][0];
    t2 += red[k][cl][1];
  }
  const int i = n * C + c;
  if (raw_mean) t2 -= static_cast<double>(raw_mean[i]) * t1;
  const double s = drop ? static_cast<double>(drop[i]) : 1.0;
  const double r = rstd[i];
  const double S1 = s * t1, S2 = s * r * t2;
  const double gr = static_cast<double>(gamma[c]) * r;
  float4 k4;
  k4.x = static_cast<float>(gr * s);
  k4.y = static_cast<float>(gr * r * S2 * inv_hw);
  k4.z = static_cast<float>(gr * S1 * inv_hw);
  k4.w = 0.f;
  reinterpret_cast<float4*>(coef)[i] = k4;
  imgsum[i * 2 + 0] = static_cast<float>(S1);
  imgsum[i * 2 + 1] = static_cast<float>(S2);
}

__global__ void __launch_bounds__(256) in_bwd_param_kernel(const float* __restrict__ imgsum, float* __restrict__ dgamma,
                                                            float* __restrict__ dbeta, int N, int C) {
  pdl_launch_dependents();
  pdl_wait();
  __shared__ double red[8][32][2];
  const int cl = threadIdx.x & 31, ng = threadIdx.x >> 5;
  const int c = blockIdx.x * 32 + cl;
  double dg = 0.0, db = 0.0;
  if (c < C) {
    const float2* sp = reinterpret_cast<const float2*>(imgsum) + c;
#pragma unroll 4
    for (int n = ng; n < N; n += 8) {
      const float2 v = sp[static_cast<int64_t>(n) * C];
      db += v.x;
      dg += v.y;
    }
  }
  red[ng][cl][0] = db;
  red[ng][cl][1] = dg;
  __syncthreads();
  if (ng != 0 || c >= C) return;
  db = dg = 0.0;
#pragma unroll
  for (int k = 0; k < 8; ++k) {
    db += red[k][cl][0];
    dg += red[k][cl][1];
  }
  dgamma[c] = static_cast<float>(dg);
  dbeta[c] = static_cast<float>(db);
}

template <typename T, bool HAS2>
__global__ void __launch_bounds__(kNormThreads, 2) in_bwd_apply_kernel(InBwdK<T> K, const float* __restrict__ coef,
                                                                        T* __restrict__ dy, int64_t dyp) {
  pdl_launch_dependents();
  pdl_wait();
  const int n = K.n0 + blockIdx.y;
  const int c0 = (threadIdx.x % K.c8n) << 3;
  const int lane = threadIdx.x / K.c8n;
  float ra[8], rb[8], k1[8], k2[8], k3[8];
  ld8f(K.a + n * K.C + c0, ra);
  ld8f(K.b + n * K.C + c0, rb);
  {
    float rm[8];
    ld8f(K.mean + n * K.C + c0, rm);
#pragma unroll
    for (int j = 0; j < 8; ++j) {
      const float4 k = reinterpret_cast<const float4*>(coef)[n * K.C + c0 + j];
      k1[j] = k.x;
      k2[j] = k.y;
      k3[j] = fmaf(k.y, rm[j], -k.z);
    }
  }
  const int64_t lo = blockIdx.x * K.chunk;
  int64_t hi = lo + K.chunk;
  if (hi > K.HW) hi = K.HW;
  const T* yb = K.y + static_cast<int64_t>(n) * K.HW * K.yp + c0;
  const T* db = K.dz + static_cast<int64_t>(n) * K.HW * K.dzp + c0;
  const T* d2b = HAS2 ? K.dz2 + static_cast<int64_t>(n) * K.HW * K.dz2p + c0 : nullptr;
  T* ob = dy + static_cast<int64_t>(n) * K.HW * dyp + c0;
  const int lanes = K.lanes;
  constexpr int U = 4;
  for (int64_t px = lo + lane; px < hi; px += U * lanes) {
    Vec8<T> vy[U], vd[U], vd2[HAS2 ? U : 1];
#pragma unroll
    for (int u = 0; u < U; ++u)
      if (px + u * lanes < hi) {
        vy[u] = Vec8<T>::ld_stream(yb + (px + u * lanes) * K.yp);
        vd[u] = Vec8<T>::ld_stream(db + (px + u * lanes) * K.dzp);
        if (HAS2) vd2[HAS2 ? u : 0] = Vec8<T>::ld_stream(d2b + (px + u * lanes) * K.dz2p);
      }
#pragma unroll
    for (int u = 0; u < U; ++u) {
      if (px + u * lanes >= hi) break;
      float yv[8], d[8], o[8];
      vy[u].unpack(yv);
      vd[u].unpack(d);
      if (HAS2) {
        float d2[8];
        vd2[HAS2 ? u : 0].unpack(d2);
#pragma unroll
        for (int j = 0; j < 8; ++j) d[j] += d2[j];
      }
#pragma unroll
      for (int j = 0; j < 8; ++j) {
        const float pre = fmaf(ra[j], yv[j], rb[j]);
        const float gm = pre > 0.f ? d[j] : d[j] * K.slope;
        o[j] = fmaf(k1[j], gm, fmaf(-k2[j], yv[j], k3[j]));
      }
      Vec8<T>::st(ob + (px + u * lanes) * dyp, o);
    }
  }
}

template <bool HAS2>
__global__ void __launch_bounds__(256, 2) in_bwd_fused_kernel(InBwdK<__nv_bfloat16> K, const float* __restrict__ gamma,
                                                               const float* __restrict__ rstd,
                                                               const float* __restrict__ drop,
                                                               __nv_bfloat16* __restrict__ dy, int64_t dyp,
                                                               float* __restrict__ imgsum, int cg8, double inv_hw) {
  pdl_launch_dependents();
  pdl_wait();
  using T = __nv_bfloat16;
  extern __shared__ __align__(16) unsigned char fz_raw[];
  const int HW = static_cast<int>(K.HW);
  uint4* ty = reinterpret_cast<uint4*>(fz_raw);
  uint4* td = ty + static_cast<size_t>(HW) * cg8;
  uint4* td2 = td + static_cast<size_t>(HW) * cg8;
  float* red = reinterpret_cast<float*>(td + static_cast<size_t>(HW) * cg8 * (HAS2 ? 2 : 1));
  float* coef = red + 256 * 16;
  const int n = blockIdx.y;
  const int CG = cg8 << 3;
  const int cbase = blockIdx.x * CG;
  const int c8 = threadIdx.x % cg8, lane = threadIdx.x / cg8, lanes = 256 / cg8;
  const int c0 = cbase + (c8 << 3);
  float ra[8], rb[8], rm[8];
  ld8f(K.a + n * K.C + c0, ra);
  ld8f(K.b + n * K.C + c0, rb);
  ld8f(K.mean + n * K.C + c0, rm);
  float t1[8], t2[8];
#pragma unroll
  for (int j = 0; j < 8; ++j) t1[j] = t2[j] = 0.f;
  const T* yb = K.y + static_cast<int64_t>(n) * HW * K.yp + c0;
  const T* db = K.dz + static_cast<int64_t>(n) * HW * K.dzp + c0;
  const T* d2b = HAS2 ? K.dz2 + static_cast<int64_t>(n) * HW * K.dz2p + c0 : nullptr;
  constexpr int U = 4;
  for (int px = lane; px < HW; px += U * lanes) {
    Vec8<T> vy[U], vd[U], vd2[HAS2 ? U : 1];
#pragma unroll
    for (int u = 0; u < U; ++u)
      if (px + u * lanes < HW) {
        vy[u] = Vec8<T>::ld_stream(yb + static_cast<int64_t>(px + u * lanes) * K.yp);
        vd[u] = Vec8<T>::ld_stream(db + static_cast<int64_t>(px + u * lanes) * K.dzp);
        if (HAS2) vd2[HAS2 ? u : 0] = Vec8<T>::ld_stream(d2b + static_cast<int64_t>(px + u * lanes) * K.dz2p);
      }
#pragma unroll
    for (int u = 0; u < U; ++u) {
      const int q = px + u * lanes;
      if (q >= HW) break;
      ty[q * cg8 + c8] = vy[u].r;
      td[q * cg8 + c8] = vd[u].r;
      float yv[8], d[8];
      vy[u].unpack(yv);
      vd[u].unpack(d);
      if (HAS2) {
        td2[q * cg8 + c8] = vd2[HAS2 ? u : 0].r;
        float d2[8];
        vd2[HAS2 ? u : 0].unpack(d2);
#pragma unroll
        for (int j = 0; j < 8; ++j) d[j] += d2[j];
      }
#pragma unroll
      for (int j = 0; j < 8; ++j) {
        const float pre = fmaf(ra[j], yv[j], rb[j]);
        const float gm = pre > 0.f ? d[j] : d[j] * K.slope;
        t1[j] += gm;
        t2[j] += gm * (yv[j] - rm[j]);
      }
    }
  }
  float* mine = red + threadIdx.x * 16;
#pragma unroll
  for (int j = 0; j < 8; ++j) {
    mine[j] = t1[j];
    mine[8 + j] = t2[j];
  }
  __syncthreads();
  if (threadIdx.x < CG) {
    const int cl = threadIdx.x, cc8 = cl >> 3, j = cl & 7;
    float s1 = 0.f, s2 = 0.f;
    for (int l = 0; l < lanes; ++l) {
      s1 += red[(l * cg8 + cc8) * 16 + j];
      s2 += red[(l * cg8 + cc8) * 16 + 8 + j];
    }
    const int c = cbase + cl;
    const int i = n * K.C + c;
    const double sc = drop ? static_cast<double>(drop[i]) : 1.0;
    const double r = rstd[i];
    const double S1 = sc * static_cast<double>(s1), S2 = sc * r * static_cast<double>(s2);
    const double gr = static_cast<double>(gamma[c]) * r;
    const float k1 = static_cast<float>(gr * sc);
    const float k2 = static_cast<float>(gr * r * S2 * inv_hw);
    const float k3 = static_cast<float>(gr * S1 * inv_hw);
    coef[cl * 4 + 0] = k1;
    coef[cl * 4 + 1] = k2;
    coef[cl * 4 + 2] = fmaf(k2, K.mean[i], -k3);
    imgsum[i * 2 + 0] = static_cast<float>(S1);
    imgsum[i * 2 + 1] = static_cast<float>(S2);
  }
  __syncthreads();
  float k1[8], k2[8], k3[8];
#pragma unroll
  for (int j = 0; j < 8; ++j) {
    k1[j] = coef[((c8 << 3) + j) * 4 + 0];
    k2[j] = coef[((c8 << 3) + j) * 4 + 1];
    k3[j] = coef[((c8 << 3) + j) * 4 + 2];
  }
  T* ob = dy + static_cast<int64_t>(n) * HW * dyp + c0;
  for (int q = lane; q < HW; q += lanes) {
    Vec8<T> vy, vd;
    vy.r = ty[q * cg8 + c8];
    vd.r = td[q * cg8 + c8];
    float yv[8], d[8], o[8];
    vy.unpack(yv);
    vd.unpack(d);
    if (HAS2) {
      Vec8<T> v2;
      v2.r = td2[q * cg8 + c8];
      float d2[8];
      v2.unpack(d2);
#pragma unroll
      for (int j = 0; j < 8; ++j) d[j] += d2[j];
    }
#pragma unroll
    for (int j = 0; j < 8; ++j) {
      const float pre = fmaf(ra[j], yv[j], rb[j]);
      const float gm = pre > 0.f ? d[j] : d[j] * K.slope;
      o[j] = fmaf(k1[j], gm, fmaf(-k2[j], yv[j], k3[j]));
    }
    Vec8<T>::st(ob + static_cast<int64_t>(q) * dyp, o);
  }
}

static int bwd_fused_group(int64_t HW, int C, bool has2) {
  static const bool off = [] { const char* e = getenv("B200UNET_NO_NORM_FUSED"); return e && e[0] == '1'; }();
  if (off || HW > 4096) return 0;
  if (has2 && HW > 256) return 0;
  const int64_t per_ch = HW * 2 * (has2 ? 3 : 2);
  const int64_t budget = 96 * 1024;
  for (int cg = 64; cg >= 16; cg >>= 1)
    if (C % cg == 0 && per_ch * cg <= budget && HW >= 256 / (cg / 8)) return cg;
  return 0;
}

static int check_nhwc(const char* what, int C, int64_t p0, int64_t p1, int64_t p2) {
  if (C % 8 != 0 || C <= 0 || C > 2048) return set_error(kErrInvalid, "%s: C=%d must be a multiple of 8 in (0,2048]", what, C);
  if (p0 % 8 || p1 % 8 || p2 % 8) return set_error(kErrInvalid, "%s: pitches must be multiples of 8 elements", what);
  return 0;
}

}

using namespace b200;

extern "C" int b200unet_in_finalize(const float* stats, int P, const float* gamma, const float* beta,
                                    const float* drop_scale, float eps, float* mean, float* rstd, float* a, float* b,
                                    int N, int C, int64_t HW, void* stream) {
  B200_CHECK_ARG(stats && gamma && beta && mean && rstd && a && b, "in_finalize: null pointer");
  B200_CHECK_ARG(P > 0 && HW > 0 && N > 0 && C > 0, "in_finalize: bad sizes");
  launch_k(in_finalize_kernel, dim3(N, ceil_div(C, 32)), dim3(256), 0, static_cast<cudaStream_t>(stream), 
      stats, P, gamma, beta, drop_scale, eps, mean, rstd, a, b, C, 1.0 / static_cast<double>(HW));
  B200_LAUNCH_CHECK("in_finalize_kernel");
  return 0;
}

template <typename T>
static int in_apply_impl(const void* y, int64_t y_pitch, const float* a, const float* b, float slope, void* z,
                         int64_t z_pitch, int N, int64_t HW, int C, void* stream) {
  B200_CHECK_ARG(y && a && b && z, "in_apply: null pointer");
  int rc = check_nhwc("in_apply", C, y_pitch, z_pitch, 0);
  if (rc) return rc;
  const PixelMap m = make_map(C);
  const int64_t chunk = pixels_per_block(HW, N, m, 4 * blocks_per_sm());
  launch_k(in_apply_kernel<T>, dim3((unsigned)ceil_div64(HW, chunk), N), dim3(m.threads), 0, static_cast<cudaStream_t>(stream), 
      static_cast<const T*>(y), y_pitch, a, b, slope, static_cast<T*>(z), z_pitch, HW, C, m.c8n, m.lanes, chunk);
  B200_LAUNCH_CHECK("in_apply_kernel");
  return 0;
}

extern "C" int b200unet_in_apply(const void* y, int64_t y_pitch, const float* a, const float* b, float slope, void* z,
                                 int64_t z_pitch, int N, int64_t HW, int C, void* stream) {
  return in_apply_impl<__nv_bfloat16>(y, y_pitch, a, b, slope, z, z_pitch, N, HW, C, stream);
}
extern "C" int b200unet_in_apply_f32(const void* y, int64_t y_pitch, const float* a, const float* b, float slope,
                                     void* z, int64_t z_pitch, int N, int64_t HW, int C, void* stream) {
  return in_apply_impl<float>(y, y_pitch, a, b, slope, z, z_pitch, N, HW, C, stream);
}

static int bwd_images_per_chunk(int N, int64_t HW, int C, bool has_dz2) {
  (void)HW;
  (void)C;
  (void)has_dz2;
  return N;
}
static int bwd_partials(int N, int64_t HW, int C, bool has_dz2) {
  const PixelMap m = make_map(C);
  const int ipc = bwd_images_per_chunk(N, HW, C, has_dz2);
  const int64_t chunk = pixels_per_block(HW, ipc, m, blocks_per_sm());
  return static_cast<int>(ceil_div64(HW, chunk));
}

extern "C" int64_t b200unet_in_backward_workspace(int N, int64_t HW, int C) {
  const int P0 = bwd_partials(N, HW, C, false), P1 = bwd_partials(N, HW, C, true);
  const int P = P0 > P1 ? P0 : P1;
  return (static_cast<int64_t>(N) * P * C * 2 + static_cast<int64_t>(N) * C * 6) * 4;
}

template <typename T>
static int in_backward_impl(const b200unet_in_bwd_args* A, void* stream) {
  B200_CHECK_ARG(A && A->dz && A->y && A->a && A->b && A->mean && A->rstd && A->gamma && A->dy && A->dgamma &&
                     A->dbeta && A->workspace,
                 "in_backward: null pointer");
  int rc = check_nhwc("in_backward", A->C, A->dz_pitch, A->dz2 ? A->dz2_pitch : 0, A->y_pitch);
  if (rc) return rc;
  B200_CHECK_ARG(A->dy_pitch % 8 == 0, "in_backward: dy pitch must be a multiple of 8");
  const int N = A->N, C = A->C;
  const int64_t HW = A->HW;
  B200_CHECK_ARG(A->workspace_bytes >= b200unet_in_backward_workspace(N, HW, C), "in_backward: workspace too small");
  cudaStream_t st = static_cast<cudaStream_t>(stream);
  const bool has2 = A->dz2 != nullptr;
  const PixelMap m = make_map(C);
  const int ipc = bwd_images_per_chunk(N, HW, C, has2);
  const int64_t chunk = pixels_per_block(HW, ipc, m, blocks_per_sm());
  const int64_t chunk_apply = chunk;
  const int P = static_cast<int>(ceil_div64(HW, chunk));
  float* imgsum = A->workspace;
  float* coef = imgsum + static_cast<int64_t>(N) * C * 2;
  float* part = coef + static_cast<int64_t>(N) * C * 4;
  InBwdK<T> K;
  K.dz = static_cast<const T*>(A->dz);
  K.dzp = A->dz_pitch;
  K.dz2 = static_cast<const T*>(A->dz2);
  K.dz2p = A->dz2_pitch;
  K.y = static_cast<const T*>(A->y);
  K.yp = A->y_pitch;
  K.a = A->a;
  K.b = A->b;
  K.mean = A->mean;
  K.slope = A->slope;
  K.HW = HW;
  K.C = C;
  K.c8n = m.c8n;
  K.lanes = m.lanes;
  K.chunk = chunk;
  const size_t red_bytes = static_cast<size_t>(m.threads) * 16 * sizeof(typename AccT<T>::type);
  const double inv_hw = 1.0 / static_cast<double>(HW);
  if constexpr (sizeof(T) == 2) {
    const bool ext_given = A->ext_part != nullptr && (!has2 || A->ext_part2 != nullptr);
    const int cg = ext_given ? 0 : bwd_fused_group(HW, C, has2);
    if (cg) {
      const size_t smem = static_cast<size_t>(HW) * cg * 2 * (has2 ? 3 : 2) + (256 * 16 + 64 * 4) * sizeof(float);
      auto kern = has2 ? in_bwd_fused_kernel<true> : in_bwd_fused_kernel<false>;
      static bool attr_set[2] = {false, false};
      if (!attr_set[has2 ? 1 : 0]) {
        B200_CUDA(cudaFuncSetAttribute(kern, cudaFuncAttributeMaxDynamicSharedMemorySize, 220 * 1024));
        attr_set[has2 ? 1 : 0] = true;
      }
      K.n0 = 0;
      launch_k(kern, dim3(C / cg, N), dim3(256), smem, st, K, A->gamma, A->rstd, A->drop_scale, static_cast<T*>(A->dy), A->dy_pitch,
                                              imgsum, cg / 8, inv_hw);
      B200_LAUNCH_CHECK("in_bwd_fused_kernel");
      if (!A->defer_params) {
        launch_k(in_bwd_param_kernel, dim3(ceil_div(C, 32)), dim3(256), 0, st, imgsum, A->dgamma, A->dbeta, N, C);
        B200_LAUNCH_CHECK("in_bwd_param_kernel");
      }
      return 0;
    }
  }
  const bool ext = A->ext_part != nullptr && (!has2 || A->ext_part2 != nullptr);
  for (int n0 = 0; n0 < N; n0 += ipc) {
    const int nn = (N - n0 < ipc) ? N - n0 : ipc;
    K.n0 = n0;
    if (ext) {
      launch_k(in_bwd_finalize_kernel, dim3(nn, ceil_div(C, 32)), dim3(256), 0, st, A->ext_part, A->ext_P, has2 ? A->ext_part2 : nullptr,
                                                                       A->ext_P2, A->mean, A->gamma, A->rstd, A->drop_scale,
                                                                       coef, imgsum, C, n0, inv_hw);
    } else {
      if (has2) launch_k(in_bwd_reduce_kernel<T, true>, dim3(P, nn), dim3(m.threads), red_bytes, st, K, part, P);
      else launch_k(in_bwd_reduce_kernel<T, false>, dim3(P, nn), dim3(m.threads), red_bytes, st, K, part, P);
      B200_LAUNCH_CHECK("in_bwd_reduce_kernel");
      launch_k(in_bwd_finalize_kernel, dim3(nn, ceil_div(C, 32)), dim3(256), 0, st, part, P, nullptr, 0, nullptr, A->gamma, A->rstd,
                                                                       A->drop_scale, coef, imgsum, C, n0, inv_hw);
    }
    B200_LAUNCH_CHECK("in_bwd_finalize_kernel");
    K.chunk = chunk_apply;
    if (has2)
      launch_k(in_bwd_apply_kernel<T, true>, dim3((unsigned)ceil_div64(HW, chunk_apply), nn), dim3(m.threads), 0, st, 
          K, coef, static_cast<T*>(A->dy), A->dy_pitch);
    else
      launch_k(in_bwd_apply_kernel<T, false>, dim3((unsigned)ceil_div64(HW, chunk_apply), nn), dim3(m.threads), 0, st, 
          K, coef, static_cast<T*>(A->dy), A->dy_pitch);
    K.chunk = chunk;
    B200_LAUNCH_CHECK("in_bwd_apply_kernel");
  }
  if (!A->defer_params) {
    launch_k(in_bwd_param_kernel, dim3(ceil_div(C, 32)), dim3(256), 0, st, imgsum, A->dgamma, A->dbeta, N, C);
    B200_LAUNCH_CHECK("in_bwd_param_kernel");
  }
  return 0;
}

extern "C" int b200unet_in_bwd_params(const float* workspace, int N, int64_t HW, int C, float* dgamma, float* dbeta,
                                      void* stream) {
  B200_CHECK_ARG(workspace && dgamma && dbeta && N > 0 && HW > 0 && C > 0, "in_bwd_params: null pointer or bad sizes");
  (void)HW;
  const float* imgsum = workspace;
  launch_k(in_bwd_param_kernel, dim3(ceil_div(C, 32)), dim3(256), 0, static_cast<cudaStream_t>(stream), imgsum, dgamma, dbeta, N, C);
  B200_LAUNCH_CHECK("in_bwd_param_kernel");
  return 0;
}

extern "C" int b200unet_in_backward(const b200unet_in_bwd_args* A, void* stream) {
  return in_backward_impl<__nv_bfloat16>(A, stream);
}
extern "C" int b200unet_in_backward_f32(const b200unet_in_bwd_args* A, void* stream) {
  return in_backward_impl<float>(A, stream);
}
```

### unet-implementations_b200/csrc/resample.cu

```cuda
#include "common.cuh"
#include "ptx.cuh"
#include "vec8.cuh"

namespace b200 {

template <typename T, int R>
__global__ void __launch_bounds__(256, 2) upsample2x_fwd_kernel(const T* __restrict__ x, int64_t xp,
                                                                 T* __restrict__ out, int64_t op, int H, int W,
                                                                 int c8n, int c8shift, const float* __restrict__ na,
                                                                 const float* __restrict__ nb, float slope) {
  pdl_launch_dependents();
  pdl_wait();
  const int t = blockIdx.x * 256 + threadIdx.x;
  const int iw = t >> c8shift;
  if (iw >= W) return;
  const int c0 = (t & (c8n - 1)) << 3;
  const int ih0 = blockIdx.y * R, n = blockIdx.z;
  const int wm = iw > 0 ? iw - 1 : 0, wp = iw < W - 1 ? iw + 1 : W - 1;
  const T* b = x + static_cast<int64_t>(n) * H * W * xp + c0;
  const int64_t om = static_cast<int64_t>(wm) * xp, oc = static_cast<int64_t>(iw) * xp, od = static_cast<int64_t>(wp) * xp;
  float ra[8], rb[8];
  if (na) {
    const int C = c8n << 3;
    const float4* pa = reinterpret_cast<const float4*>(na + n * C + c0);
    const float4* pb = reinterpret_cast<const float4*>(nb + n * C + c0);
    const float4 a0 = __ldg(pa), a1 = __ldg(pa + 1), b0 = __ldg(pb), b1 = __ldg(pb + 1);
    ra[0] = a0.x; ra[1] = a0.y; ra[2] = a0.z; ra[3] = a0.w; ra[4] = a1.x; ra[5] = a1.y; ra[6] = a1.z; ra[7] = a1.w;
    rb[0] = b0.x; rb[1] = b0.y; rb[2] = b0.z; rb[3] = b0.w; rb[4] = b1.x; rb[5] = b1.y; rb[6] = b1.z; rb[7] = b1.w;
  }
  auto hmix = [&](int row, float (&Lo)[8], float (&Ro)[8]) {
    const T* rp = b + static_cast<int64_t>(row) * W * xp;
    float a[8], c[8], d[8];
    Vec8<T>::ldg(rp + om).unpack(a);
    Vec8<T>::ldg(rp + oc).unpack(c);
    Vec8<T>::ldg(rp + od).unpack(d);
    if (na) {
#pragma unroll
      for (int j = 0; j < 8; ++j) {
        const float t0 = fmaf(ra[j], a[j], rb[j]), t1 = fmaf(ra[j], c[j], rb[j]), t2 = fmaf(ra[j], d[j], rb[j]);
        a[j] = t0 > 0.f ? t0 : t0 * slope;
        c[j] = t1 > 0.f ? t1 : t1 * slope;
        d[j] = t2 > 0.f ? t2 : t2 * slope;
      }
    }
#pragma unroll
    for (int j = 0; j < 8; ++j) {
      Lo[j] = 0.75f * c[j] + 0.25f * a[j];
      Ro[j] = 0.75f * c[j] + 0.25f * d[j];
    }
  };
  float L[3][8], Rr[3][8];
  hmix(ih0 > 0 ? ih0 - 1 : 0, L[0], Rr[0]);
  hmix(ih0, L[1], Rr[1]);
  const int OW = 2 * W;
  T* o = out + (static_cast<int64_t>(n) * 2 * H + 2 * ih0) * OW * op + static_cast<int64_t>(2 * iw) * op + c0;
  const int64_t orow = static_cast<int64_t>(OW) * op;
#pragma unroll
  for (int r = 0; r < R; ++r) {
    const int ih = ih0 + r;
    if (ih >= H) break;
    float (&Lp)[8] = L[r % 3], (&Lc)[8] = L[(r + 1) % 3], (&Ln)[8] = L[(r + 2) % 3];
    float (&Rp)[8] = Rr[r % 3], (&Rc)[8] = Rr[(r + 1) % 3], (&Rn)[8] = Rr[(r + 2) % 3];
    hmix(ih < H - 1 ? ih + 1 : H - 1, Ln, Rn);
    float v[8];
#pragma unroll
    for (int j = 0; j < 8; ++j) v[j] = 0.75f * Lc[j] + 0.25f * Lp[j];
    Vec8<T>::st(o, v);
#pragma unroll
    for (int j = 0; j < 8; ++j) v[j] = 0.75f * Rc[j] + 0.25f * Rp[j];
    Vec8<T>::st(o + op, v);
#pragma unroll
    for (int j = 0; j < 8; ++j) v[j] = 0.75f * Lc[j] + 0.25f * Ln[j];
    Vec8<T>::st(o + orow, v);
#pragma unroll
    for (int j = 0; j < 8; ++j) v[j] = 0.75f * Rc[j] + 0.25f * Rn[j];
    Vec8<T>::st(o + orow + op, v);
    o += 2 * orow;
  }
}

constexpr int kUpRows = 4;

template <typename T>
__global__ void __launch_bounds__(256) upsample2x_bwd_kernel(const T* __restrict__ dout, int64_t dp,
                                                              T* __restrict__ dx, int64_t xp, int H, int W,
                                                              int c8n, int c8shift) {
  pdl_launch_dependents();
  pdl_wait();
  const int t = blockIdx.x * 256 + threadIdx.x;
  const int iw = t >> c8shift;
  if (iw >= W) return;
  const int c0 = (t & (c8n - 1)) << 3;
  const int ih0 = blockIdx.y * kUpRows, n = blockIdx.z;
  const int OH = 2 * H, OW = 2 * W;
  const T* b = dout + static_cast<int64_t>(n) * OH * OW * dp + c0;
  int cols[4];
#pragma unroll
  for (int a = 0; a < 4; ++a) {
    const int ow = 2 * iw - 1 + a;
    cols[a] = ow < 0 ? 0 : (ow >= OW ? OW - 1 : ow);
  }
  float acc[kUpRows][8];
#pragma unroll
  for (int r = 0; r < kUpRows; ++r)
#pragma unroll
    for (int j = 0; j < 8; ++j) acc[r][j] = 0.f;
#pragma unroll
  for (int k = 0; k < 2 * kUpRows + 2; ++k) {
    const int oh_u = 2 * ih0 - 1 + k;
    const int oh = oh_u < 0 ? 0 : (oh_u >= OH ? OH - 1 : oh_u);
    const T* rp = b + static_cast<int64_t>(oh) * OW * dp;
    Vec8<T> raw[4];
#pragma unroll
    for (int bb = 0; bb < 4; ++bb) raw[bb] = Vec8<T>::ldg(rp + static_cast<int64_t>(cols[bb]) * dp);
    float d0[8], d1[8], d2[8], d3[8], hs[8];
    raw[0].unpack(d0);
    raw[1].unpack(d1);
    raw[2].unpack(d2);
    raw[3].unpack(d3);
#pragma unroll
    for (int j = 0; j < 8; ++j) hs[j] = 0.25f * (d0[j] + d3[j]) + 0.75f * (d1[j] + d2[j]);
#pragma unroll
    for (int r = 0; r < kUpRows; ++r) {
      const int a = k - 2 * r;
      if (a >= 0 && a < 4) {
        const float wgt = (a == 0 || a == 3) ? 0.25f : 0.75f;
#pragma unroll
        for (int j = 0; j < 8; ++j) acc[r][j] = fmaf(wgt, hs[j], acc[r][j]);
      }
    }
  }
#pragma unroll
  for (int r = 0; r < kUpRows; ++r) {
    const int ih = ih0 + r;
    if (ih < H) Vec8<T>::st(dx + ((static_cast<int64_t>(n) * H + ih) * W + iw) * xp + c0, acc[r]);
  }
}

template <typename T>
__global__ void nchw_to_nhwc_kernel(const float* __restrict__ src, T* __restrict__ dst, int64_t dp, int C,
                                    int64_t HW) {
  __shared__ float tile[32][33];
  const int n = blockIdx.z;
  const int64_t p0 = static_cast<int64_t>(blockIdx.x) * 32;
  const int c0 = blockIdx.y * 32;
  for (int j = threadIdx.y; j < 32; j += blockDim.y) {
    const int c = c0 + j;
    const int64_t p = p0 + threadIdx.x;
    tile[j][threadIdx.x] = (c < C && p < HW) ? src[(static_cast<int64_t>(n) * C + c) * HW + p] : 0.f;
  }
  __syncthreads();
  for (int j = threadIdx.y; j < 32; j += blockDim.y) {
    const int64_t p = p0 + j;
    const int c = c0 + threadIdx.x;
    if (c < C && p < HW) dst[(static_cast<int64_t>(n) * HW + p) * dp + c] = from_f32<T>(tile[threadIdx.x][j]);
  }
}

__global__ void nhwc_to_nchw_kernel(const __nv_bfloat16* __restrict__ src, int64_t sp, float* __restrict__ dst, int C,
                                    int64_t HW) {
  __shared__ float tile[32][33];
  const int n = blockIdx.z;
  const int64_t p0 = static_cast<int64_t>(blockIdx.x) * 32;
  const int c0 = blockIdx.y * 32;
  for (int j = threadIdx.y; j < 32; j += blockDim.y) {
    const int64_t p = p0 + j;
    const int c = c0 + threadIdx.x;
    tile[j][threadIdx.x] = (c < C && p < HW) ? __bfloat162float(src[(static_cast<int64_t>(n) * HW + p) * sp + c]) : 0.f;
  }
  __syncthreads();
  for (int j = threadIdx.y; j < 32; j += blockDim.y) {
    const int c = c0 + j;
    const int64_t p = p0 + threadIdx.x;
    if (c < C && p < HW) dst[(static_cast<int64_t>(n) * C + c) * HW + p] = tile[threadIdx.x][j];
  }
}


__global__ void __launch_bounds__(256) image_to_nhwc32_kernel(const float* __restrict__ src, __nv_bfloat16* __restrict__ dst,
                                                               int C, int64_t HW) {
  pdl_launch_dependents();
  pdl_wait();
  const int n = blockIdx.y;
  const int64_t p = static_cast<int64_t>(blockIdx.x) * 256 + threadIdx.x;
  if (p >= HW) return;
  float f[8];
#pragma unroll
  for (int c = 0; c < 8; ++c) f[c] = c < C ? __ldg(src + (static_cast<int64_t>(n) * C + c) * HW + p) : 0.f;
  uint4* o = reinterpret_cast<uint4*>(dst + (static_cast<int64_t>(n) * HW + p) * 32);
  o[0] = make_uint4(pack_bf16x2(f[0], f[1]), pack_bf16x2(f[2], f[3]), pack_bf16x2(f[4], f[5]), pack_bf16x2(f[6], f[7]));
  const uint4 z = make_uint4(0u, 0u, 0u, 0u);
  o[1] = z;
  o[2] = z;
  o[3] = z;
}

}

using namespace b200;

static int ilog2_exact(int v) {
  int s = 0;
  while ((1 << s) < v) ++s;
  return (1 << s) == v ? s : -1;
}

template <typename T>
static int upsample_fwd_impl(const void* x, int64_t x_pitch, void* out, int64_t out_pitch, int N, int H, int W, int C,
                             void* stream, const float* na = nullptr, const float* nb = nullptr, float slope = 0.f) {
  B200_CHECK_ARG(x && out, "upsample2x_fwd: null pointer");
  B200_CHECK_ARG(C % 8 == 0 && x_pitch % 8 == 0 && out_pitch % 8 == 0, "upsample2x_fwd: C and pitches must be multiples of 8");
  const int c8n = C / 8, sh = ilog2_exact(c8n);
  B200_CHECK_ARG(sh >= 0, "upsample2x_fwd: C/8 = %d must be a power of two", c8n);
  B200_CHECK_ARG(H <= 65535 && N <= 65535, "upsample2x_fwd: H and N must fit the grid");
  const dim3 block(256);
#define B200_UP_LAUNCH(RR)                                                                                             \
  launch_k(upsample2x_fwd_kernel<T, RR>, dim3(ceil_div(W * c8n, 256), ceil_div(H, RR), N), block, 0,                     \
           static_cast<cudaStream_t>(stream), static_cast<const T*>(x), x_pitch, static_cast<T*>(out), out_pitch, H, W,  \
           c8n, sh, na, nb, slope)
  if (H >= 64) B200_UP_LAUNCH(8);
  else B200_UP_LAUNCH(2);
#undef B200_UP_LAUNCH
  B200_LAUNCH_CHECK("upsample2x_fwd_kernel");
  return 0;
}

template <typename T>
static int upsample_bwd_impl(const void* dout, int64_t dout_pitch, void* dx, int64_t dx_pitch, int N, int H, int W,
                             int C, void* stream) {
  B200_CHECK_ARG(dout && dx, "upsample2x_bwd: null pointer");
  B200_CHECK_ARG(C % 8 == 0 && dout_pitch % 8 == 0 && dx_pitch % 8 == 0, "upsample2x_bwd: C and pitches must be multiples of 8");
  const int c8n = C / 8, sh = ilog2_exact(c8n);
  B200_CHECK_ARG(sh >= 0, "upsample2x_bwd: C/8 = %d must be a power of two", c8n);
  B200_CHECK_ARG(H <= 65535 && N <= 65535, "upsample2x_bwd: H and N must fit the grid");
  launch_k(upsample2x_bwd_kernel<T>, dim3(ceil_div(W * c8n, 256), ceil_div(H, kUpRows), N), dim3(256), 0, static_cast<cudaStream_t>(stream), 
      static_cast<const T*>(dout), dout_pitch, static_cast<T*>(dx), dx_pitch, H, W, c8n, sh);
  B200_LAUNCH_CHECK("upsample2x_bwd_kernel");
  return 0;
}

extern "C" int b200unet_upsample2x_fwd(const void* x, int64_t x_pitch, void* out, int64_t out_pitch, int N, int H,
                                       int W, int C, void* stream) {
  return upsample_fwd_impl<__nv_bfloat16>(x, x_pitch, out, out_pitch, N, H, W, C, stream);
}
extern "C" int b200unet_upsample2x_fwd_f32(const void* x, int64_t x_pitch, void* out, int64_t out_pitch, int N, int H,
                                           int W, int C, void* stream) {
  return upsample_fwd_impl<float>(x, x_pitch, out, out_pitch, N, H, W, C, stream);
}
extern "C" int b200unet_upsample2x_norm_fwd(const void* y, int64_t y_pitch, const float* a, const float* b, float slope,
                                            void* out, int64_t out_pitch, int N, int H, int W, int C, void* stream) {
  B200_CHECK_ARG(a && b, "upsample2x_norm_fwd: null affine");
  return upsample_fwd_impl<__nv_bfloat16>(y, y_pitch, out, out_pitch, N, H, W, C, stream, a, b, slope);
}
extern "C" int b200unet_upsample2x_norm_fwd_f32(const void* y, int64_t y_pitch, const float* a, const float* b,
                                                float slope, void* out, int64_t out_pitch, int N, int H, int W, int C,
                                                void* stream) {
  B200_CHECK_ARG(a && b, "upsample2x_norm_fwd: null affine");
  return upsample_fwd_impl<float>(y, y_pitch, out, out_pitch, N, H, W, C, stream, a, b, slope);
}
extern "C" int b200unet_upsample2x_bwd(const void* dout, int64_t dout_pitch, void* dx, int64_t dx_pitch, int N, int H,
                                       int W, int C, void* stream) {
  return upsample_bwd_impl<__nv_bfloat16>(dout, dout_pitch, dx, dx_pitch, N, H, W, C, stream);
}
extern "C" int b200unet_upsample2x_bwd_f32(const void* dout, int64_t dout_pitch, void* dx, int64_t dx_pitch, int N,
                                           int H, int W, int C, void* stream) {
  return upsample_bwd_impl<float>(dout, dout_pitch, dx, dx_pitch, N, H, W, C, stream);
}

extern "C" int b200unet_nchw_f32_to_nhwc_bf16(const float* src, void* dst, int64_t dst_pitch, int N, int C, int64_t HW,
                                              void* stream) {
  B200_CHECK_ARG(src && dst, "nchw_f32_to_nhwc_bf16: null pointer");
  dim3 grid((unsigned)ceil_div64(HW, 32), ceil_div(C, 32), N);
  nchw_to_nhwc_kernel<__nv_bfloat16><<<grid, dim3(32, 8), 0, static_cast<cudaStream_t>(stream)>>>(
      src, static_cast<__nv_bfloat16*>(dst), dst_pitch, C, HW);
  B200_LAUNCH_CHECK("nchw_to_nhwc_kernel");
  return 0;
}
extern "C" int b200unet_nchw_f32_to_nhwc_f32(const float* src, void* dst, int64_t dst_pitch, int N, int C, int64_t HW,
                                             void* stream) {
  B200_CHECK_ARG(src && dst, "nchw_f32_to_nhwc_f32: null pointer");
  dim3 grid((unsigned)ceil_div64(HW, 32), ceil_div(C, 32), N);
  nchw_to_nhwc_kernel<float><<<grid, dim3(32, 8), 0, static_cast<cudaStream_t>(stream)>>>(
      src, static_cast<float*>(dst), dst_pitch, C, HW);
  B200_LAUNCH_CHECK("nchw_to_nhwc_kernel");
  return 0;
}

extern "C" int b200unet_nhwc_bf16_to_nchw_f32(const void* src, int64_t src_pitch, float* dst, int N, int C, int64_t HW,
                                              void* stream) {
  B200_CHECK_ARG(src && dst, "nhwc_bf16_to_nchw_f32: null pointer");
  dim3 grid((unsigned)ceil_div64(HW, 32), ceil_div(C, 32), N);
  nhwc_to_nchw_kernel<<<grid, dim3(32, 8), 0, static_cast<cudaStream_t>(stream)>>>(
      static_cast<const __nv_bfloat16*>(src), src_pitch, dst, C, HW);
  B200_LAUNCH_CHECK("nhwc_to_nchw_kernel");
  return 0;
}

extern "C" int b200unet_image_to_nhwc32_bf16(const float* src, void* dst, int N, int C, int64_t HW, void* stream) {
  B200_CHECK_ARG(src && dst, "image_to_nhwc32_bf16: null pointer");
  B200_CHECK_ARG(C >= 1 && C <= 8 && N <= 65535, "image_to_nhwc32_bf16: C must be in [1,8]");
  launch_k(image_to_nhwc32_kernel, dim3((unsigned)ceil_div64(HW, 256), N), dim3(256), 0, static_cast<cudaStream_t>(stream), 
      src, static_cast<__nv_bfloat16*>(dst), C, HW);
  B200_LAUNCH_CHECK("image_to_nhwc32_kernel");
  return 0;
}
```

### unet-implementations_b200/csrc/vec8.cuh

```cuda
#pragma once
#include "ptx.cuh"

namespace b200 {

template <typename T>
struct Vec8;

template <>
struct Vec8<__nv_bfloat16> {
  uint4 r;
  __device__ __forceinline__ static Vec8 ld_stream(const __nv_bfloat16* p) {
    Vec8 v;
    asm volatile("ld.global.nc.L1::no_allocate.v4.u32 {%0, %1, %2, %3}, [%4];"
                 : "=r"(v.r.x), "=r"(v.r.y), "=r"(v.r.z), "=r"(v.r.w)
                 : "l"(p));
    return v;
  }
  __device__ __forceinline__ static Vec8 ldg(const __nv_bfloat16* p) {
    Vec8 v;
    v.r = __ldg(reinterpret_cast<const uint4*>(p));
    return v;
  }
  __device__ __forceinline__ void unpack(float (&f)[8]) const {
    const __nv_bfloat162* h = reinterpret_cast<const __nv_bfloat162*>(&r);
#pragma unroll
    for (int i = 0; i < 4; ++i) {
      const float2 t = __bfloat1622float2(h[i]);
      f[2 * i] = t.x;
      f[2 * i + 1] = t.y;
    }
  }
  __device__ __forceinline__ static void st(__nv_bfloat16* p, const float (&f)[8]) {
    *reinterpret_cast<uint4*>(p) = make_uint4(pack_bf16x2(f[0], f[1]), pack_bf16x2(f[2], f[3]),
                                              pack_bf16x2(f[4], f[5]), pack_bf16x2(f[6], f[7]));
  }
};

template <>
struct Vec8<float> {
  float4 a, b;
  __device__ __forceinline__ static Vec8 ld_stream(const float* p) { return ldg(p); }
  __device__ __forceinline__ static Vec8 ldg(const float* p) {
    Vec8 v;
    v.a = __ldg(reinterpret_cast<const float4*>(p));
    v.b = __ldg(reinterpret_cast<const float4*>(p) + 1);
    return v;
  }
  __device__ __forceinline__ void unpack(float (&f)[8]) const {
    f[0] = a.x; f[1] = a.y; f[2] = a.z; f[3] = a.w; f[4] = b.x; f[5] = b.y; f[6] = b.z; f[7] = b.w;
  }
  __device__ __forceinline__ static void st(float* p, const float (&f)[8]) {
    reinterpret_cast<float4*>(p)[0] = make_float4(f[0], f[1], f[2], f[3]);
    reinterpret_cast<float4*>(p)[1] = make_float4(f[4], f[5], f[6], f[7]);
  }
};

template <typename T>
struct AccT {
  using type = float;
};
template <>
struct AccT<float> {
  using type = double;
};

__device__ __forceinline__ float to_f32(__nv_bfloat16 v) { return __bfloat162float(v); }
__device__ __forceinline__ float to_f32(float v) { return v; }
template <typename T>
__device__ __forceinline__ T from_f32(float v);
template <>
__device__ __forceinline__ __nv_bfloat16 from_f32<__nv_bfloat16>(float v) { return __float2bfloat16_rn(v); }
template <>
__device__ __forceinline__ float from_f32<float>(float v) { return v; }

}
```

### unet-implementations_b200/models/unet.py

```python
from __future__ import annotations

from typing import Dict, List, Optional, Tuple, Type, Union

import os

import torch
import torch.nn as nn
import torch.nn.functional as F

try:
    from .. import ops
except ImportError:
    from unet_implementations_b200 import ops

BF16 = torch.bfloat16


def _lib_call(name, *args):
    return ops._lib.call(name, *args)


class SpatialDropout2d(nn.Module):

    def __init__(self, drop_prob):
# ... 310 lines not shown
    out = _to_nchw_f32(y_nhwc)
    if conv.bias is not None:
        out = out + conv.bias.detach().view(1, -1, 1, 1)
    inp = x_nchw_or_nhwc if is_nchw_input else _to_nchw_f32(x_nchw_or_nhwc)
    for hook in list(conv._forward_hooks.values()):
        if hook(conv, (inp,), out) is not None:
            raise NotImplementedError("b200unet: a forward hook on an inner Conv2d may observe its output, not replace it")


def _fire_backward_hooks(conv: nn.Conv2d, dx_nhwc, dy_nhwc):
    go = (_to_nchw_f32(dy_nhwc),)
    gi = (_to_nchw_f32(dx_nhwc),)
    for hook in list(conv._backward_hooks.values()):
        if hook(conv, gi, go) is not None:
            raise NotImplementedError("b200unet: a backward hook on an inner Conv2d may observe gradients, not replace them")


def _use_tc(cin: int, cout: int) -> bool:
    return cin % 32 == 0 and cout % 32 == 0


def _conv_fwd(x, wf, stride, out=None):
    cout, cin = wf.shape[0], wf.shape[3]
    return ops.conv_fprop(x, wf, stride, out=out, want_stats=True, simt=not _use_tc(cin, cout))


class _UNetFunction(torch.autograd.Function):

    @staticmethod
    def forward(ctx, model: UNet, x: torch.Tensor, *params):
        ops.require_device()
        with torch.cuda.device(x.device):
            return _forward_impl(ctx, model, x, params)

    @staticmethod
    def backward(ctx, dlogits):
        sink = getattr(getattr(ctx, "model", None), "_grad_sink", None)
        reserve = int(getattr(sink, "reserve_sms", 0) or 0)
        prev = _lib_call("b200unet_set_reserved_sms", reserve) if reserve else 0
        try:
            with torch.cuda.device(dlogits.device):
                grads = _backward_impl(ctx, dlogits)
        finally:
            if reserve:
                _lib_call("b200unet_set_reserved_sms", prev)
        return (None, None) + tuple(grads)


def _forward_impl(ctx, model: UNet, x: torch.Tensor, params):
    x = x.detach()
    x_u8 = None
    if x.dtype == torch.uint8:
        x_u8 = x.contiguous()
        B, H, W, _ = x_u8.shape
        x = None
    else:
        if x.dtype != torch.float32 or not x.is_contiguous():
            x = x.float().contiguous()
        B, _, H, W = x.shape

    def _image():
        nonlocal x
        if x is None:
            from ..data import preprocess_batch
            x = preprocess_batch(x_u8, None, model.input_mean, model.input_std)[0]
        return x
    n = model.n_stages
    feats = list(model.features_per_stage)
    layers = model._layers()
    training = model.training
    if model.precision not in ("bf16", "fp32"):
        raise ValueError(f"b200unet: precision must be 'bf16' or 'fp32', got {model.precision!r}")
    adt = torch.float32 if model.precision == "fp32" else BF16
    need_grad = any(ctx.needs_input_grad[2:])
    dev = x_u8.device if x_u8 is not None else x.device

    sizes = []
    h, w = H, W
    for s in range(n):
        st = model.encoder_stages[s].block[0].stride[0]
        h, w = ops.conv_out_hw(h, w, st)
        sizes.append((h, w))
    for d in range(n - 1):
        if sizes[d] != (2 * sizes[d + 1][0], 2 * sizes[d + 1][1]):
            raise NotImplementedError(
                f"b200unet: the upsample kernel is the exact 2x case of F.interpolate (unet.py:220-225); level {d} is "
                f"{sizes[d]} over {sizes[d + 1]} -- use an input size divisible by {2 ** (n - 1)}")

    cat = [torch.empty((B, sizes[d][0], sizes[d][1], feats[d + 1] + feats[d]), dtype=adt, device=dev)
           for d in range(n - 1)]

    _f32_like = x if x is not None else torch.empty(0, dtype=torch.float32, device=dev)
    override = list(model._mask_override) if model._mask_override is not None else None
    used_masks = []

    def draw(drop: Optional[SpatialDropout2d], c: int):
        if drop is None or not training or drop.drop_prob == 0:
            return None
        if override is not None:
            m = override.pop(0).to(device=dev, dtype=torch.float32)
        else:
            m = drop.draw(_f32_like, B, c)
        m = m.reshape(B, c).contiguous()
        used_masks.append(m)
        return m

    extra = getattr(model, "_extra_features", None)
    fusion = model._fusion_unit() if extra is not None else None
    catf = None
    const_extra = False
    if fusion is not None:
        fh, fw = sizes[-1]
        const_extra = model.skip_constant_features and extra.dim() == 4 and (
            tuple(extra.shape[2:]) == (1, 1) or (extra.stride(2) == 0 and extra.stride(3) == 0))
        if not const_extra:
            if extra.shape[2:] != (fh, fw):
                extra = F.interpolate(extra.float(), size=(fh, fw), mode="bilinear", align_corners=False)
            catf = torch.empty((B, fh, fw, feats[-1] + extra.shape[1]), dtype=adt, device=dev)
            ops.nchw_to_nhwc(extra.detach().float().contiguous(), out=catf[..., feats[-1]:])
        layers = [L for L in layers if L["kind"] == "enc"] + [dict(kind="fusion", stage=0, idx=0, last=True, unit=fusion)] + \
                 [L for L in layers if L["kind"] == "dec"]

    saved = []
    cur = None
    cur_norm = None
    for li_f, L in enumerate(layers):
        conv, norm, act, drop = L["unit"]
        cin, cout = conv.in_channels, conv.out_channels
        stride = conv.stride[0]
        rec = dict(L=L, stride=stride)
        if L["kind"] == "dec" and L["idx"] == 0:
            d = n - 2 - L["stage"]
            c_low = feats[d + 1]
            ops.upsample2x(cur, cat[d][..., :c_low], norm=cur_norm)
            if model._trace_fwd is not None:
                model._trace_fwd.append(dict(kind="up", src=cur, norm=cur_norm, out=cat[d][..., :c_low]))
            rec["low"] = cur
            cur = cat[d]
            cur_norm = None
        first = L["kind"] == "enc" and L["stage"] == 0 and L["idx"] == 0
        if first:
            if cin <= 8 and cout == 32 and stride == 1 and adt == BF16 and W >= 64:
                if x_u8 is not None:
                    xin32 = ops.preprocess_u8_nhwc32(x_u8, model.input_mean, model.input_std)
                else:
                    xin32 = ops.image_to_nhwc32(x)
                y, stats = ops.conv_fprop(xin32, model._packed_stem(conv), 1, want_stats=True)
                rec["stem"] = True
                rec["xin32"] = xin32 if need_grad else None
            elif cin == 3 and cout == 32 and stride == 1 and adt == BF16:
                y, stats = ops.stem_fprop(_image(), conv.weight)
                rec["stem"] = True
            else:
                xin = ops.nchw_to_nhwc(_image(), out=_padded_nhwc(B, H, W, cin, dev, adt))
                wf, wd = model._packed(conv, False, adt)
                y, stats = _conv_fwd(xin, wf, stride)
                rec["xin"] = xin
                rec["stem"] = False
        else:
            if L["kind"] == "fusion":
                if conv.kernel_size != (1, 1) or conv.in_channels != feats[-1] + extra.shape[1]:
                    raise NotImplementedError("b200unet: the fusion layer must be a 1x1 conv over cat([bottleneck, features])")
                if const_extra:
                    wf, wd = model._packed_1x1(conv, need_grad, adt, cin_used=feats[-1])
                    rec["cin_used"] = feats[-1]
                else:
                    cur = catf
                    wf, wd = model._packed_1x1(conv, need_grad, adt)
            else:
                wf, wd = model._packed(conv, need_grad, adt)
            y, stats = _conv_fwd(cur, wf, stride)
            rec["xin"] = cur
            rec["wd"] = wd
        if conv._forward_hooks:
            _fire_forward_hooks(conv, _image() if first else cur, y, first)
        scale = draw(drop, cout)
        oh, ow = y.shape[1], y.shape[2]
        mean, rstd, a, b = ops.in_finalize(stats, norm.weight, norm.bias, scale, norm.eps, oh * ow)
        dst = None
        if L["kind"] == "enc" and L["last"] and L["stage"] < n - 1:
            d = L["stage"]
            dst = cat[d][..., feats[d + 1]:]
        elif L["kind"] == "enc" and L["last"] and catf is not None:
            dst = catf[..., :feats[-1]]
        nxt = layers[li_f + 1] if li_f + 1 < len(layers) else None
        fuse_into_consumer = model._trace is None and dst is None and (
            (nxt is not None and nxt["kind"] == "dec" and nxt["idx"] == 0) or (nxt is None and model.head_kind == "seg1x1"))
        if fuse_into_consumer:
            z, cur_norm = y, (a, b, act.negative_slope)
        else:
            z, cur_norm = ops.in_apply(y, a, b, act.negative_slope, out=dst), None
        rec.update(y=y, mean=mean, rstd=rstd, a=a, b=b, scale=scale, slope=act.negative_slope, conv=conv, norm=norm)
        if model._trace_fwd is not None:
            model._trace_fwd.append(dict(kind="unit", li=li_f, L=L, conv=conv, norm=norm, stride=stride, slope=act.negative_slope,
                                         xin=rec.get("xin32") if rec.get("xin32") is not None else rec.get("xin"),
                                         y=y, mean=mean, rstd=rstd, a=a, b=b, scale=scale,
                                         z=None if fuse_into_consumer else z))
        saved.append(rec)
        cur = z
        if model._trace is not None:
            model._trace.append((y, z))
    head = model._head_conv()
    if model.head_kind == "seg1x1":
        if head.in_channels != 32 or head.out_channels != 3 or head.bias is None:
            raise NotImplementedError("b200unet: the head kernel is built for Conv2d(32 -> 3, 1x1, bias) (unet.py:374-381)")
        logits = ops.head_forward(cur, head.weight, head.bias, norm=cur_norm)
        if model._trace_fwd is not None:
            model._trace_fwd.append(dict(kind="head", z=cur, norm=cur_norm, logits=logits))
        if need_grad:
            ctx.head_norm = cur_norm
    else:
        if head.out_channels > 4 or head.bias is None or head.in_channels % 32 != 0:
            raise NotImplementedError("b200unet: the reconstruction head is built for Conv2d(32k -> <=4, 3x3, bias) + Sigmoid")
        wfh, wdh = model._packed_head(head, need_grad, adt)
        yh, _ = ops.conv_fprop(cur, wfh, 1, want_stats=False, simt=not _use_tc(head.in_channels, wfh.shape[0]))
        logits = ops.recon_head_forward(yh[..., :head.out_channels], head.bias)
        if need_grad:
            ctx.head_out = logits
            ctx.head_wd = wdh
    model.last_dropout_masks = used_masks
    if need_grad:
        ctx.model = model
        ctx.saved = saved
        ctx.image = x
        ctx.image_u8 = x_u8
        ctx.z_last = cur
        ctx.cat = cat
        ctx.sizes = sizes
        ctx.param_ids = {id(p): i for i, p in enumerate(params)}
        ctx.param_req = [p.requires_grad for p in params]
        ctx.n_params = len(params)
    else:
        ctx.saved = None
    return logits


def _padded_nhwc(B, H, W, C, dev, dtype=BF16):
    pitch = (C + 7) // 8 * 8
    buf = torch.zeros((B, H, W, pitch), dtype=dtype, device=dev)
    return buf[..., :C]


def _backward_impl(ctx, dlogits):
    if ctx.saved is None:
        raise RuntimeError("b200unet: backward called on a forward that ran without grad")
    model: UNet = ctx.model
    saved = ctx.saved
    n = model.n_stages
    feats = list(model.features_per_stage)
    grads: List[Optional[torch.Tensor]] = [None] * ctx.n_params
    ids = ctx.param_ids
    req = ctx.param_req
    sink = model._grad_sink

    in_place = sink is not None and hasattr(sink, "dest")

    def wants(p: Optional[nn.Parameter]) -> bool:
        return p is not None and req[ids[id(p)]]

    def dest(p: Optional[nn.Parameter]):
        if sink is None or not wants(p) or not hasattr(sink, "dest"):
            return None
        return sink.dest(p)

    def put(p: Optional[nn.Parameter], g_fn):
        if not wants(p):
            return
        g = g_fn()
        if sink is not None:
            g = sink(p, g)
            if in_place and p.grad is None:
                p.grad = g
                return
        grads[ids[id(p)]] = g

    dead_bias = [rec["conv"].bias for rec in saved if wants(rec["conv"].bias)]
    zero_pool, zero_off = None, [0]
    if dead_bias and (sink is None or not hasattr(sink, "dest")):
        zero_pool = torch.zeros(sum((b.numel() + 3) // 4 * 4 for b in dead_bias), dtype=torch.float32, device=dlogits.device)

    def zero_grad_of(b: nn.Parameter):
        d = dest(b)
        if d is not None:
            return d
        if zero_pool is None:
            return torch.zeros_like(b)
        v = zero_pool[zero_off[0]:zero_off[0] + b.numel()].view(b.shape)
        zero_off[0] += (b.numel() + 3) // 4 * 4
        return v

    btrace = model._trace_bwd

    first_needed = len(saved)
    for li, rec in enumerate(saved):
        ps = [rec["conv"].weight, rec["conv"].bias, rec["norm"].weight, rec["norm"].bias]
        if any(p is not None and req[ids[id(p)]] for p in ps):
            first_needed = li
            break

    head = model._head_conv()
    if dlogits.dtype != torch.float32:
        dlogits = dlogits.float()
    ext_part = None
    if model.head_kind == "seg1x1":
        if ctx.head_norm is not None and model.producer_sums:
            dz, dwh, dbh, ext_part = ops.head_backward(dlogits, ctx.z_last, head.weight, norm=ctx.head_norm,
                                                       out_dw=dest(head.weight), out_db=dest(head.bias), want_bwd_part=True)
        else:
            dz, dwh, dbh = ops.head_backward(dlogits, ctx.z_last, head.weight, norm=ctx.head_norm, out_dw=dest(head.weight),
                                             out_db=dest(head.bias))
    else:
        z_last, wdh = ctx.z_last, ctx.head_wd
        cpad = wdh.shape[3]
        dpre, dbh = ops.recon_head_backward(dlogits, ctx.head_out, cpad, z_last.dtype)
        simt_h = not _use_tc(head.in_channels, cpad)
        dz = ops.conv_dgrad(dpre, wdh, (z_last.shape[1], z_last.shape[2]), 1, simt=simt_h)
        dwh = ops.conv_wgrad(z_last, dpre, 1, simt=simt_h)[:head.out_channels].contiguous()
        ctx.head_out = None
    if btrace is not None:
        btrace.append(dict(kind="head", dlogits=dlogits, dz=dz, dw=dwh, db=dbh))
    put(head.weight, lambda: dwh)
    put(head.bias, lambda: dbh)

    main = torch.cuda.current_stream()
    overlap = bool(model.overlap_wgrad)
    side = None
    if overlap:
        side = model._side_streams.get(main.device.index)
        if side is None:
            side = model._side_streams[main.device.index] = torch.cuda.Stream(device=main.device)
    pending = []

    def collect():
        while pending:
            p, g, ev, _inputs = pending.pop(0)
            main.wait_event(ev)
            g.record_stream(main)
            put(p, lambda: g)

    def wgrad_async(p: Optional[nn.Parameter], fn, inputs, trec=None):
        if not wants(p):
            return
        if not overlap:
            g = fn()
            if trec is not None:
                trec["dw"] = g
            put(p, lambda: g)
            return
        side.wait_stream(main)
        with torch.cuda.stream(side):
            g = fn()
            ev = torch.cuda.Event()
            ev.record(side)
        if trec is not None:
            trec["dw"] = g
        pending.append((p, g, ev, list(inputs)))

    dskip: Dict[int, torch.Tensor] = {}
    dz2 = None
    for li in range(len(saved) - 1, -1, -1):
        if li < first_needed:
            break
        rec = saved[li]
        L = rec["L"]
        conv, norm = rec["conv"], rec["norm"]
        if L["kind"] == "enc" and L["last"] and L["stage"] < n - 1:
            dz2 = dskip.pop(L["stage"])
        else:
            dz2 = None
        dgd, dbd = dest(norm.weight), dest(norm.bias)
        if dgd is None or dbd is None:
            dgd = dbd = None
        defer = overlap and (wants(norm.weight) or wants(norm.bias))
        res = ops.in_backward(dz, dz2, rec["y"], rec["a"], rec["b"], rec["mean"], rec["rstd"], rec["scale"],
                              norm.weight, rec["slope"], out_dgamma=dgd, out_dbeta=dbd,
                              ext_part=ext_part if dz2 is None else None, defer_params=defer)
        ext_part = None
        rec_y = rec["y"]
        rec["y"] = None
        collect()
        if defer:
            dy, finish_params = res
            side.wait_stream(main)
            with torch.cuda.stream(side):
                dgamma, dbeta = finish_params()
                ev_p = torch.cuda.Event()
                ev_p.record(side)
            pending.append((norm.weight, dgamma, ev_p, [finish_params.keep]))
            pending.append((norm.bias, dbeta, ev_p, [finish_params.keep]))
        else:
            dy, dgamma, dbeta = res
            put(norm.weight, lambda: dgamma)
            put(norm.bias, lambda: dbeta)
        trec = None
        if btrace is not None:
            trec = dict(kind="unit", li=li, dz=dz, dz2=dz2, y=rec_y, dy=dy, dgamma=dgamma, dbeta=dbeta, xin=rec.get("xin"),
                        xin32=rec.get("xin32"))
            btrace.append(trec)
        put(conv.bias, lambda: zero_grad_of(conv.bias))
        stride = rec["stride"]
        cin, cout = conv.in_channels, conv.out_channels
        simt = not _use_tc(cin, cout)
        if rec.get("stem") is True:
            if conv._backward_hooks:
                _fire_backward_hooks(conv, None, dy)
            xin32 = rec.get("xin32")
            if xin32 is None and ctx.image is None:
                from ..data import preprocess_batch
                ctx.image = preprocess_batch(ctx.image_u8, None, model.input_mean, model.input_std)[0]
            wgrad_async(conv.weight, lambda: ops.stem_wgrad_tc(ctx.image, dy, xin32, out=dest(conv.weight), channels=cin),
                        [ctx.image, dy, xin32], trec)
            break
        xin = rec["xin"]
        last = li == first_needed or rec.get("stem") is False
        dx = None
        if not last:
            wd = rec["wd"]
            ws2 = model._packed_s2(conv, wd) if (stride == 2 and not simt and wd.dtype == BF16) else None
            split_out = None
            if (L["kind"] == "dec" and L["idx"] == 0 and not simt and stride == 1 and dy.dtype == BF16
                    and cin == 96 and feats[n - 1 - L["stage"]] == 64 and model.split_concat_grad):
                split_out = feats[n - 1 - L["stage"]]
            if ws2 is not None:
                dx = ops.conv_dgrad_s2(dy, ws2, (xin.shape[1], xin.shape[2]))
            elif split_out is not None:
                dx = ops.conv_dgrad_split(dy, wd, (xin.shape[1], xin.shape[2]), split_out)
            elif model.producer_sums_dgrad and L["idx"] > 0 and L["kind"] != "fusion" and li - 1 >= first_needed \
                    and saved[li - 1]["y"] is not None:
                prev = saved[li - 1]
                dx, ext_part = ops.conv_dgrad(dy, wd, (xin.shape[1], xin.shape[2]), stride, simt=simt,
                                              bwd_sums=(prev["y"], prev["a"], prev["b"], prev["slope"]))
            else:
                dx = ops.conv_dgrad(dy, wd, (xin.shape[1], xin.shape[2]), stride, simt=simt)
        if L["kind"] == "fusion":
            def fusion_dw():
                g = ops.conv_wgrad(xin, dy, stride, simt=simt)[:, :, 1:2, 1:2]
                if rec.get("cin_used") is None:
                    return g.contiguous()
                full = torch.zeros_like(conv.weight)
                full[:, :rec["cin_used"]] = g
                return full
            wgrad_async(conv.weight, fusion_dw, [xin, dy], trec)
        else:
            wgrad_async(conv.weight, lambda: ops.conv_wgrad(xin, dy, stride, simt=simt, out=dest(conv.weight)), [xin, dy], trec)
        if trec is not None:
            trec["dx"] = torch.cat(dx, dim=-1) if isinstance(dx, tuple) else dx
        if conv._backward_hooks:
            _fire_backward_hooks(conv, torch.cat(dx, dim=-1) if isinstance(dx, tuple) else dx, dy)
        if last:
            break
        rec["xin"] = None
        if L["kind"] == "dec" and L["idx"] == 0:
            d = n - 2 - L["stage"]
            c_low = feats[d + 1]
            dup, dsk = dx if isinstance(dx, tuple) else (dx[..., :c_low], dx[..., c_low:])
            dskip[d] = dsk
            dz = ops.upsample2x_backward(dup)
            if btrace is not None:
                btrace.append(dict(kind="up", d=d, dout=dup, dx=dz))
        elif L["kind"] == "fusion":
            dz = dx[..., :feats[-1]]
        else:
            dz = dx
    collect()
    if sink is not None and hasattr(sink, "finish"):
        sink.finish()
    ctx.saved = None
    ctx.cat = None
    ctx.z_last = None
    return grads


class _BlockFunction(torch.autograd.Function):
    @staticmethod
    def forward(ctx, block: ConvBlock, x, *params):
        ops.require_device()
        units = block.units()
        xin = ops.nchw_to_nhwc(x.detach().float().contiguous(),
                               out=_padded_nhwc(x.size(0), x.size(2), x.size(3), x.size(1), x.device))
        cur = xin
        recs = []
        need_grad = any(ctx.needs_input_grad)
        for conv, norm, act, drop in units:
            wf, wd = ops.pack_conv_weights(conv.weight, need_dgrad=need_grad)
            y, stats = _conv_fwd(cur, wf, conv.stride[0])
            scale = None
            if drop is not None and block.training and drop.drop_prob > 0:
                scale = drop.draw(x, x.size(0), conv.out_channels).reshape(x.size(0), -1).float().contiguous()
            mean, rstd, a, b = ops.in_finalize(stats, norm.weight, norm.bias, scale, norm.eps, y.shape[1] * y.shape[2])
            z = ops.in_apply(y, a, b, act.negative_slope)
            recs.append(dict(xin=cur, y=y, wd=wd, mean=mean, rstd=rstd, a=a, b=b, scale=scale, conv=conv, norm=norm,
                             slope=act.negative_slope))
            cur = z
        ctx.recs = recs if need_grad else None
        ctx.x_needs = x.requires_grad
        ctx.params = params
        return ops.nhwc_to_nchw(cur)

    @staticmethod
    def backward(ctx, dout):
        recs = ctx.recs
        dz = ops.nchw_to_nhwc(dout.float().contiguous())
        pg = {}
        for i in range(len(recs) - 1, -1, -1):
            r = recs[i]
            conv, norm = r["conv"], r["norm"]
            dy, dg, db = ops.in_backward(dz, None, r["y"], r["a"], r["b"], r["mean"], r["rstd"], r["scale"], norm.weight,
                                         r["slope"])
            simt = not _use_tc(conv.in_channels, conv.out_channels)
            pg[id(norm.weight)], pg[id(norm.bias)] = dg, db
            pg[id(conv.weight)] = ops.conv_wgrad(r["xin"], dy, conv.stride[0], simt=simt)
            if conv.bias is not None:
                pg[id(conv.bias)] = torch.zeros_like(conv.bias)
            if i > 0 or ctx.x_needs:
                xin = r["xin"]
                dxp = _padded_nhwc(xin.shape[0], xin.shape[1], xin.shape[2], xin.shape[3], xin.device)
                dz = ops.conv_dgrad(dy, r["wd"], (xin.shape[1], xin.shape[2]), conv.stride[0], out=dxp, simt=simt)
        dx = ops.nhwc_to_nchw(dz) if ctx.x_needs else None
        return (None, dx) + tuple(pg.get(id(p)) if p.requires_grad else None for p in ctx.params)


class _UpsampleCatFunction(torch.autograd.Function):

    @staticmethod
    def forward(ctx, x, skip):
        ops.require_device()
        B, c_low, h, w = x.shape
        c_skip = skip.shape[1]
        if tuple(skip.shape[2:]) != (2 * h, 2 * w):
            raise NotImplementedError("b200unet: UpBlock implements the exact 2x case of F.interpolate (unet.py:220-225); "
                                      f"got {tuple(x.shape[2:])} -> {tuple(skip.shape[2:])}")
        if c_low % 8 or c_skip % 8:
            raise NotImplementedError("b200unet: UpBlock needs channel counts that are multiples of 8")
        with torch.cuda.device(x.device):
            cat = torch.empty((B, 2 * h, 2 * w, c_low + c_skip), dtype=BF16, device=x.device)
            xl = ops.nchw_to_nhwc(x.detach().float().contiguous())
            ops.upsample2x(xl, cat[..., :c_low])
            ops.nchw_to_nhwc(skip.detach().float().contiguous(), out=cat[..., c_low:])
            out = ops.nhwc_to_nchw(cat)
        ctx.c_low = c_low
        return out

    @staticmethod
    def backward(ctx, dout):
        c_low = ctx.c_low
        with torch.cuda.device(dout.device):
            d = ops.nchw_to_nhwc(dout.float().contiguous())
            dx = ops.nhwc_to_nchw(ops.upsample2x_backward(d[..., :c_low])) if ctx.needs_input_grad[0] else None
            dskip = dout[:, c_low:].float().contiguous() if ctx.needs_input_grad[1] else None
        return dx, dskip


def _run_block_standalone(block: ConvBlock, x: torch.Tensor):
    if not x.is_cuda:
        raise RuntimeError("b200unet: ConvBlock needs a CUDA tensor on an sm_100 device; there is no CPU path")
    return _BlockFunction.apply(block, x, *list(block.parameters()))
```

### unet-implementations_b200/ops.py

```python
from __future__ import annotations

import ctypes

import torch

from . import _lib
from ._lib import ConvDgradArgs, ConvFpropArgs, ConvWgradArgs, InBwdArgs

BF16 = torch.bfloat16
F32 = torch.float32


def _sfx(t: torch.Tensor) -> str:
    if t.dtype == BF16:
        return ""
    if t.dtype == F32:
        return "_f32"
    raise TypeError(f"b200unet: activations must be bf16 or fp32, got {t.dtype}")


def _p(t):
    return ctypes.c_void_p(t.data_ptr()) if t is not None else ctypes.c_void_p(0)


def _stream():
    return ctypes.c_void_p(torch.cuda.current_stream().cuda_stream)


def pitch_of(t: torch.Tensor) -> int:
    assert t.dim() == 4 and t.dtype in (BF16, F32) and t.is_cuda, "expected a CUDA bf16/fp32 [N,H,W,C] tensor"
    n, h, w, c = t.shape
    pitch = t.stride(2)
    assert t.stride(3) == 1 and pitch >= c, f"channels must be contiguous (strides {t.stride()})"
    assert (h == 1 or t.stride(1) == w * pitch) and (n == 1 or t.stride(0) == h * w * pitch), (
        f"not a pitched NHWC view: shape {tuple(t.shape)} strides {t.stride()}"
    )
    assert pitch % 8 == 0 and t.data_ptr() % 16 == 0, "pitch must be a multiple of 8 elements, base 16-byte aligned"
    return pitch


def _f32(t: torch.Tensor) -> torch.Tensor:
    assert t.dtype == torch.float32 and t.is_cuda and t.is_contiguous()
    return t


def require_device():
    if not torch.cuda.is_available():
        raise RuntimeError("b200unet: no CUDA device; this path has no CPU fallback")
    if _lib.call("b200unet_device_ok") != 1:
        raise RuntimeError("b200unet: the current device is not compute capability 10.x (B200, sm_100a)")


def pack_conv_weights(w_oihw: torch.Tensor, need_dgrad: bool = True, dtype=BF16):
    w = _f32(w_oihw.detach())
    cout, cin, kh, kw = w.shape
    assert kh == 3 and kw == 3
    wf = torch.empty((cout, 3, 3, cin), dtype=dtype, device=w.device)
    wd = torch.empty((cin, 3, 3, cout), dtype=dtype, device=w.device) if need_dgrad else None
    _lib.call("b200unet_pack_conv_weights" + _sfx(wf), _p(w), _p(wf), _p(wd), cout, cin, _stream())
    return wf, wd


def conv_out_hw(h: int, w: int, stride: int):
    return (h - 1) // stride + 1, (w - 1) // stride + 1


def conv_fprop(x, w_fprop, stride=1, out=None, want_stats=True, simt=False):
    n, h, w, cin = x.shape
    cout = w_fprop.shape[0]
    assert w_fprop.shape == (cout, 3, 3, cin) and w_fprop.dtype == x.dtype and w_fprop.is_contiguous()
    oh, ow = conv_out_hw(h, w, stride)
    y = out if out is not None else torch.empty((n, oh, ow, cout), dtype=x.dtype, device=x.device)
    assert tuple(y.shape) == (n, oh, ow, cout) and y.dtype == x.dtype
    f32 = x.dtype == F32
    simt = simt or f32
    stats = None
    if want_stats:
        if simt:
            parts = _lib.call("b200unet_conv_fprop_simt_partials", oh, ow)
        else:
            parts = _lib.call("b200unet_conv_fprop_partials", n, oh, ow, cout)
            if parts < 0:
                raise RuntimeError(f"conv_fprop: Cout={cout} outside the tensor-core envelope")
        stats = torch.empty((n, parts, cout, 2), dtype=torch.float32, device=x.device)
    a = ConvFpropArgs(_p(x), pitch_of(x), _p(w_fprop), _p(y), pitch_of(y), _p(stats), n, h, w, cin, cout, stride)
    name = "b200unet_conv_fprop_f32" if f32 else ("b200unet_conv_fprop_simt" if simt else "b200unet_conv_fprop")
    _lib.call(name, ctypes.byref(a), _stream())
    return y, stats


def pack_s2_dgrad_weights(w_dgrad):
    cin, _, _, cout = w_dgrad.shape
    if w_dgrad.dtype != BF16 or _lib.call("b200unet_conv_dgrad_s2_supported", cin, cout) != 1:
        return None
    ws = torch.empty((4 * cin, 4, cout), dtype=BF16, device=w_dgrad.device)
    _lib.call("b200unet_pack_s2_dgrad_weights", _p(w_dgrad), _p(ws), cin, cout, _stream())
    return ws


def conv_dgrad_s2(dy, w_stacked, in_hw, out=None):
    n, oh, ow, cout = dy.shape
    cin = w_stacked.shape[0] // 4
    h, w = in_hw
    assert conv_out_hw(h, w, 2) == (oh, ow) and w_stacked.shape == (4 * cin, 4, cout) and dy.dtype == BF16
    dx = out if out is not None else torch.empty((n, h, w, cin), dtype=BF16, device=dy.device)
    a = ConvDgradArgs(_p(dy), pitch_of(dy), _p(w_stacked), _p(dx), pitch_of(dx), n, h, w, cin, cout, 2)
    _lib.call("b200unet_conv_dgrad_s2", ctypes.byref(a), _stream())
    return dx


def conv_dgrad_split(dy, w_dgrad, in_hw, split):
    n, oh, ow, cout = dy.shape
    cin = w_dgrad.shape[0]
    h, w = in_hw
    assert w_dgrad.shape == (cin, 3, 3, cout) and w_dgrad.dtype == dy.dtype == BF16 and (oh, ow) == (h, w) and 0 < split < cin
    d1 = torch.empty((n, h, w, split), dtype=BF16, device=dy.device)
    d2 = torch.empty((n, h, w, cin - split), dtype=BF16, device=dy.device)
    a = ConvDgradArgs(_p(dy), pitch_of(dy), _p(w_dgrad), _p(d1), pitch_of(d1), n, h, w, cin, cout, 1)
    a.dx2, a.dx2_pitch, a.dx_split = d2.data_ptr(), pitch_of(d2), split
    _lib.call("b200unet_conv_dgrad", ctypes.byref(a), _stream())
    return d1, d2


def conv_dgrad(dy, w_dgrad, in_hw, stride=1, out=None, simt=False, bwd_sums=None):
    n, oh, ow, cout = dy.shape
    cin = w_dgrad.shape[0]
    h, w = in_hw
    assert w_dgrad.shape == (cin, 3, 3, cout) and w_dgrad.dtype == dy.dtype and w_dgrad.is_contiguous()
    assert conv_out_hw(h, w, stride) == (oh, ow)
    dx = out if out is not None else torch.empty((n, h, w, cin), dtype=dy.dtype, device=dy.device)
    a = ConvDgradArgs(_p(dy), pitch_of(dy), _p(w_dgrad), _p(dx), pitch_of(dx), n, h, w, cin, cout, stride)
    name = "b200unet_conv_dgrad_f32" if dy.dtype == F32 else ("b200unet_conv_dgrad_simt" if simt else "b200unet_conv_dgrad")
    part = None
    if bwd_sums is not None and name == "b200unet_conv_dgrad":
        y, sa, sb, slope = bwd_sums
        slots = _lib.call("b200unet_conv_dgrad_bwd_slots", n, h, w, cin, cout, stride)
        if slots > 0 and y.dtype == BF16 and tuple(y.shape) == (n, h, w, cin):
            part = torch.empty((n, slots, cin, 2), dtype=torch.float32, device=dy.device)
            a.bs_y, a.bs_y_pitch, a.bs_a, a.bs_b = y.data_ptr(), pitch_of(y), _f32(sa).data_ptr(), _f32(sb).data_ptr()
            a.bs_slope, a.bs_part = float(slope), part.data_ptr()
    _lib.call(name, ctypes.byref(a), _stream())
    return (dx, part) if bwd_sums is not None else dx


def conv_wgrad(x, dy, stride=1, simt=False, out=None):
    n, h, w, cin = x.shape
    _, oh, ow, cout = dy.shape
    assert conv_out_hw(h, w, stride) == (oh, ow)
    if out is not None:
        assert tuple(out.shape) == (cout, cin, 3, 3) and out.dtype == torch.float32 and out.is_contiguous()
        dw = out
    else:
        dw = torch.empty((cout, cin, 3, 3), dtype=torch.float32, device=x.device)
    assert x.dtype == dy.dtype
    if simt or x.dtype == F32:
        a = ConvWgradArgs(_p(x), pitch_of(x), _p(dy), pitch_of(dy), _p(dw), None, 0, n, h, w, cin, cout, stride)
        _lib.call("b200unet_conv_wgrad_f32" if x.dtype == F32 else "b200unet_conv_wgrad_simt", ctypes.byref(a), _stream())
        return dw
    nbytes = _lib.call("b200unet_conv_wgrad_workspace", n, h, w, cin, cout, stride)
    if nbytes < 0:
        raise RuntimeError(f"conv_wgrad: unsupported shape: {_lib.last_error()}")
    ws = torch.empty((max(nbytes, 4) // 4,), dtype=torch.float32, device=x.device)
    a = ConvWgradArgs(_p(x), pitch_of(x), _p(dy), pitch_of(dy), _p(dw), _p(ws), nbytes, n, h, w, cin, cout, stride)
    _lib.call("b200unet_conv_wgrad", ctypes.byref(a), _stream())
    return dw


def stem_fprop(img_nchw, w_oihw, out=None, want_stats=True):
    img = _f32(img_nchw)
    n, c, h, w = img.shape
    assert c == 3 and tuple(w_oihw.shape) == (32, 3, 3, 3)
    y = out if out is not None else torch.empty((n, h, w, 32), dtype=BF16, device=img.device)
    stats = None
    if want_stats:
        parts = _lib.call("b200unet_stem_partials", h, w)
        stats = torch.empty((n, parts, 32, 2), dtype=torch.float32, device=img.device)
    _lib.call("b200unet_stem_fprop", _p(img), _p(_f32(w_oihw.detach())), _p(y), pitch_of(y), _p(stats), n, h, w,
              _stream())
    return y, stats


def image_to_nhwc32(img_nchw):
    img = _f32(img_nchw)
    n, c, h, w = img.shape
    assert c <= 8
    xp = torch.empty((n, h, w, 32), dtype=BF16, device=img.device)
    _lib.call("b200unet_image_to_nhwc32_bf16", _p(img), _p(xp), n, c, h * w, _stream())
    return xp


def preprocess_u8_nhwc32(images_u8, mean, std):
    assert images_u8.dtype == torch.uint8 and images_u8.dim() == 4 and images_u8.size(3) == 3 and images_u8.is_cuda
    x = images_u8.contiguous()
    n, h, w, _ = x.shape
    xp = torch.empty((n, h, w, 32), dtype=BF16, device=x.device)
    m3 = (ctypes.c_float * 3)(*[float(v) for v in mean])
    s3 = (ctypes.c_float * 3)(*[float(v) for v in std])
    _lib.call("b200unet_preprocess_u8_nhwc32", _p(x), _p(xp), m3, s3, n, h * w, _stream())
    return xp


def pack_stem_weights(w_oihw):
    cout, c = w_oihw.shape[0], w_oihw.shape[1]
    w32 = torch.zeros((cout, 32, 3, 3), dtype=torch.float32, device=w_oihw.device)
    w32[:, :c] = w_oihw.detach()
    return pack_conv_weights(w32, need_dgrad=False)[0]


def stem_wgrad_tc(img_nchw, dy, xp=None, out=None, channels=None):
    c = channels if channels is not None else img_nchw.shape[1]
    assert dy.dtype == BF16
    if xp is None:
        xp = image_to_nhwc32(img_nchw)
    full = conv_wgrad(xp, dy, 1)
    if out is not None:
        out.copy_(full[:, :c])
        return out
    return full[:, :c].contiguous()


def stem_wgrad(img_nchw, dy):
    img = _f32(img_nchw)
    n, c, h, w = img.shape
    nbytes = _lib.call("b200unet_stem_wgrad_workspace", n, h, w)
    ws = torch.empty((nbytes // 4,), dtype=torch.float32, device=img.device)
    dw = torch.empty((32, 3, 3, 3), dtype=torch.float32, device=img.device)
    _lib.call("b200unet_stem_wgrad", _p(img), _p(dy), pitch_of(dy), _p(dw), _p(ws), nbytes, n, h, w, _stream())
    return dw


def in_finalize(stats, gamma, beta, drop_scale, eps, hw):
    n, parts, c, _ = stats.shape
    out = torch.empty((4, n, c), dtype=torch.float32, device=stats.device)
    mean, rstd, a, b = out[0], out[1], out[2], out[3]
    _lib.call("b200unet_in_finalize", _p(stats), parts, _p(_f32(gamma.detach())), _p(_f32(beta.detach())),
              _p(drop_scale), float(eps), _p(mean), _p(rstd), _p(a), _p(b), n, c, hw, _stream())
    return mean, rstd, a, b


def in_apply(y, a, b, slope, out=None):
    n, h, w, c = y.shape
    z = out if out is not None else torch.empty((n, h, w, c), dtype=y.dtype, device=y.device)
    assert tuple(z.shape) == (n, h, w, c) and z.dtype == y.dtype
    _lib.call("b200unet_in_apply" + _sfx(y), _p(y), pitch_of(y), _p(a), _p(b), float(slope), _p(z), pitch_of(z), n, h * w, c,
              _stream())
    return z


def in_backward(dz, dz2, y, a, b, mean, rstd, drop_scale, gamma, slope, out_dgamma=None, out_dbeta=None,
                ext_part=None, ext_part2=None, defer_params=False):
    n, h, w, c = y.shape
    hw = h * w
    nbytes = _lib.call("b200unet_in_backward_workspace", n, hw, c)
    ws = torch.empty((nbytes // 4,), dtype=torch.float32, device=y.device)
    if out_dgamma is not None and out_dbeta is not None:
        assert out_dgamma.numel() == c and out_dbeta.numel() == c and out_dgamma.dtype == torch.float32
        dgb = (out_dgamma, out_dbeta)
    else:
        dgb = torch.empty((2, c), dtype=torch.float32, device=y.device)
    dy = torch.empty((n, h, w, c), dtype=y.dtype, device=y.device)
    assert dz.dtype == y.dtype and (dz2 is None or dz2.dtype == y.dtype)
    ep, ep2 = ext_part, ext_part2
    if ep is not None:
        assert ep.dtype == torch.float32 and ep.is_contiguous() and ep.shape[0] == n and tuple(ep.shape[2:]) == (c, 2)
    if ep2 is not None:
        assert ep2.dtype == torch.float32 and ep2.is_contiguous() and ep2.shape[0] == n and tuple(ep2.shape[2:]) == (c, 2)
    args = InBwdArgs(_p(dz), pitch_of(dz), _p(dz2), pitch_of(dz2) if dz2 is not None else 0, _p(y), pitch_of(y), _p(a),
                     _p(b), _p(mean), _p(rstd), _p(drop_scale), _p(_f32(gamma.detach())), float(slope), _p(dy),
                     pitch_of(dy), _p(dgb[0]), _p(dgb[1]), _p(ws), nbytes, n, hw, c,
                     _p(ep), ep.shape[1] if ep is not None else 0, _p(ep2), ep2.shape[1] if ep2 is not None else 0,
                     1 if defer_params else 0)
    _lib.call("b200unet_in_backward" + _sfx(y), ctypes.byref(args), _stream())
    if defer_params:
        def finish_params():
            _lib.call("b200unet_in_bwd_params", _p(ws), n, hw, c, _p(dgb[0]), _p(dgb[1]), _stream())
            return dgb[0], dgb[1]
        finish_params.keep = (ws, dgb)
        return dy, finish_params
    return dy, dgb[0], dgb[1]


def upsample2x(x, out, norm=None):
    n, h, w, c = x.shape
    assert tuple(out.shape) == (n, 2 * h, 2 * w, c) and out.dtype == x.dtype
    if norm is None:
        _lib.call("b200unet_upsample2x_fwd" + _sfx(x), _p(x), pitch_of(x), _p(out), pitch_of(out), n, h, w, c, _stream())
    else:
        a, b, slope = norm
        _lib.call("b200unet_upsample2x_norm_fwd" + _sfx(x), _p(x), pitch_of(x), _p(a), _p(b), float(slope), _p(out),
                  pitch_of(out), n, h, w, c, _stream())
    return out


def upsample2x_backward(dout, out=None):
    n, oh, ow, c = dout.shape
    assert oh % 2 == 0 and ow % 2 == 0
    dx = out if out is not None else torch.empty((n, oh // 2, ow // 2, c), dtype=dout.dtype, device=dout.device)
    _lib.call("b200unet_upsample2x_bwd" + _sfx(dout), _p(dout), pitch_of(dout), _p(dx), pitch_of(dx), n, oh // 2, ow // 2, c,
              _stream())
    return dx


def nchw_to_nhwc(x_nchw, out=None):
    x = _f32(x_nchw)
    n, c, h, w = x.shape
    y = out if out is not None else torch.empty((n, h, w, c), dtype=BF16, device=x.device)
    name = "b200unet_nchw_f32_to_nhwc_f32" if y.dtype == F32 else "b200unet_nchw_f32_to_nhwc_bf16"
    _lib.call(name, _p(x), _p(y), y.stride(2), n, c, h * w, _stream())
    return y


def nhwc_to_nchw(x):
    n, h, w, c = x.shape
    y = torch.empty((n, c, h, w), dtype=torch.float32, device=x.device)
    _lib.call("b200unet_nhwc_bf16_to_nchw_f32", _p(x), x.stride(2), _p(y), n, c, h * w, _stream())
    return y


def head_forward(z, weight, bias, norm=None):
    n, h, w, c = z.shape
    k = weight.shape[0]
    logits = torch.empty((n, k, h, w), dtype=torch.float32, device=z.device)
    if norm is None:
        _lib.call("b200unet_head_fwd" + _sfx(z), _p(z), pitch_of(z), _p(_f32(weight.detach().reshape(k, c))),
                  _p(_f32(bias.detach())), _p(logits), n, h * w, c, k, _stream())
    else:
        a, b, slope = norm
        _lib.call("b200unet_head_norm_fwd" + _sfx(z), _p(z), pitch_of(z), _p(a), _p(b), float(slope),
                  _p(_f32(weight.detach().reshape(k, c))), _p(_f32(bias.detach())), _p(logits), n, h * w, c, k, _stream())
    return logits


def head_backward(dlogits, z, weight, norm=None, out_dw=None, out_db=None, want_bwd_part=False):
    n, h, w, c = z.shape
    k = weight.shape[0]
    dl = _f32(dlogits.contiguous())
    nbytes = _lib.call("b200unet_head_bwd_workspace", n, h * w, c, k)
    ws = torch.empty((nbytes // 4,), dtype=torch.float32, device=z.device)
    dz = torch.empty((n, h, w, c), dtype=z.dtype, device=z.device)
    dw = out_dw if out_dw is not None else torch.empty((k, c, 1, 1), dtype=torch.float32, device=z.device)
    db = out_db if out_db is not None else torch.empty((k,), dtype=torch.float32, device=z.device)
    assert dw.numel() == k * c and db.numel() == k and dw.is_contiguous() and db.is_contiguous()
    if norm is None:
        _lib.call("b200unet_head_bwd" + _sfx(z), _p(dl), _p(z), pitch_of(z), _p(_f32(weight.detach().reshape(k, c))), _p(dz),
                  pitch_of(dz), _p(dw), _p(db), _p(ws), nbytes, n, h * w, c, k, _stream())
    elif want_bwd_part:
        a, b, slope = norm
        slots = _lib.call("b200unet_head_bwd_stat_slots", n, h * w)
        part = torch.empty((n, slots, c, 2), dtype=torch.float32, device=z.device)
        _lib.call("b200unet_head_norm_bwd_stats" + _sfx(z), _p(dl), _p(z), pitch_of(z), _p(a), _p(b), float(slope),
                  _p(_f32(weight.detach().reshape(k, c))), _p(dz), pitch_of(dz), _p(dw), _p(db), _p(ws), nbytes, _p(part),
                  n, h * w, c, k, _stream())
        return dz, dw, db, part
    else:
        a, b, slope = norm
        _lib.call("b200unet_head_norm_bwd" + _sfx(z), _p(dl), _p(z), pitch_of(z), _p(a), _p(b), float(slope),
                  _p(_f32(weight.detach().reshape(k, c))), _p(dz), pitch_of(dz), _p(dw), _p(db), _p(ws), nbytes, n, h * w, c,
                  k, _stream())
    return dz, dw, db


def loss_forward(logits, target, class_weights, dynamic, weight_ce, weight_dice, ignore_index, smooth):
    lg = _f32(logits)
    n, k, h, w = lg.shape
    assert k == 3, "SimpleLoss kernels are built for 3 classes (losses.py:40)"
    assert target.dtype in (torch.int64, torch.uint8) and target.is_cuda and target.is_contiguous()
    assert tuple(target.shape) == (n, h, w)
    hw = h * w
    nbytes = _lib.call("b200unet_loss_workspace", n, hw)
    ws = torch.empty((nbytes // 4,), dtype=torch.float32, device=lg.device)
    out = torch.empty((3,), dtype=torch.float32, device=lg.device)
    tables = torch.empty((3 + 6 * n,), dtype=torch.float32, device=lg.device)
    cw = _f32(class_weights) if class_weights is not None else None
    _lib.call("b200unet_loss_fwd" + ("_u8" if target.dtype == torch.uint8 else ""), _p(lg), _p(target), _p(cw),
              int(bool(dynamic)), float(weight_ce),
              float(weight_dice), int(ignore_index), float(smooth), _p(out), _p(tables), _p(ws), nbytes, n, hw,
              _stream())
    return out, tables


def loss_backward(logits, target, tables, grad_out, weight_ce, weight_dice, ignore_index):
    lg = _f32(logits)
    n, k, h, w = lg.shape
    dl = torch.empty_like(lg)
    go = _f32(grad_out.reshape(1).contiguous()) if grad_out is not None else None
    _lib.call("b200unet_loss_bwd" + ("_u8" if target.dtype == torch.uint8 else ""), _p(lg), _p(target), _p(tables), _p(go),
              float(weight_ce), float(weight_dice),
              int(ignore_index), _p(dl), n, h * w, _stream())
    return dl


def recon_head_forward(y, bias):
    n, h, w, _ = y.shape
    k = bias.numel()
    out = torch.empty((n, k, h, w), dtype=torch.float32, device=y.device)
    _lib.call("b200unet_recon_head_fwd" + _sfx(y), _p(y), pitch_of(y), _p(_f32(bias.detach())), _p(out), n, h * w, k,
              _stream())
    return out


def recon_head_backward(dout, out, cpad, dtype):
    do, o = _f32(dout.contiguous()), _f32(out)
    n, k, h, w = o.shape
    dpre = torch.empty((n, h, w, cpad), dtype=dtype, device=o.device)
    db = torch.empty((k,), dtype=torch.float32, device=o.device)
    nbytes = _lib.call("b200unet_recon_head_bwd_workspace", n, h * w)
    ws = torch.empty((nbytes // 4,), dtype=torch.float32, device=o.device)
    _lib.call("b200unet_recon_head_bwd" + _sfx(dpre), _p(do), _p(o), _p(dpre), pitch_of(dpre), cpad, _p(db), _p(ws), nbytes,
              n, h * w, k, _stream())
    return dpre, db


def mse_forward(a, b):
    a, b = _f32(a), _f32(b)
    assert a.shape == b.shape
    n = a.numel()
    nbytes = _lib.call("b200unet_mse_workspace", n)
    ws = torch.empty((nbytes // 4,), dtype=torch.float32, device=a.device)
    out = torch.empty((1,), dtype=torch.float32, device=a.device)
    _lib.call("b200unet_mse_fwd", _p(a), _p(b), _p(out), _p(ws), nbytes, n, _stream())
    return out


def mse_backward(a, b, grad_out):
    a, b = _f32(a), _f32(b)
    da = torch.empty_like(a)
    go = _f32(grad_out.reshape(1).contiguous()) if grad_out is not None else None
    _lib.call("b200unet_mse_bwd", _p(a), _p(b), _p(go), _p(da), a.numel(), _stream())
    return da
```

Measured before the change: 1588.

## Recompute head dz inside norm backward, tile upsample through shared memory

The head backward no longer writes the bf16 dz tensor when the following instance-norm backward can rebuild it. The norm apply kernel instead reads the three fp32 logit gradients per pixel and the head weights, and recomputes dz with the same bf16 rounding. This removes a full-resolution 32-channel write and read. Separately, the upsample forward and backward kernels now stage input rows into shared memory with cp.async instead of doing repeated global loads. The image-to-NHWC grid sizing also changes. The trade-off is more per-pixel arithmetic in the apply kernel, and larger shared-memory use that may lower occupancy in the upsample kernels.

```diff
diff --git a/include/b200unet.h b/include/b200unet.h
--- a/include/b200unet.h
+++ b/include/b200unet.h
@@ -108,6 +108,9 @@
   const float* ext_part2;
   int ext_P2;
   int defer_params;
+  const float* head_dl;
+  const float* head_w;
+  int head_K;
 } b200unet_in_bwd_args;
 int64_t b200unet_in_backward_workspace(int N, int64_t HW, int C);
 int b200unet_in_backward(const b200unet_in_bwd_args* a, void* stream);
diff --git a/unet-implementations_b200/_lib.py b/unet-implementations_b200/_lib.py
--- a/unet-implementations_b200/_lib.py
+++ b/unet-implementations_b200/_lib.py
@@ -43,6 +43,7 @@
         ("dgamma", c_void_p), ("dbeta", c_void_p), ("workspace", c_void_p), ("workspace_bytes", c_int64),
         ("N", c_int), ("HW", c_int64), ("C", c_int),
         ("ext_part", c_void_p), ("ext_P", c_int), ("ext_part2", c_void_p), ("ext_P2", c_int), ("defer_params", c_int),
+        ("head_dl", c_void_p), ("head_w", c_void_p), ("head_K", c_int),
     ]
 
 
diff --git a/unet-implementations_b200/csrc/head_loss.cu b/unet-implementations_b200/csrc/head_loss.cu
--- a/unet-implementations_b200/csrc/head_loss.cu
+++ b/unet-implementations_b200/csrc/head_loss.cu
@@ -345,7 +345,7 @@
   }
 }
 
-template <typename T, int C, int K, bool STATS>
+template <typename T, int C, int K, bool STATS, bool DZ = true>
 __global__ void __launch_bounds__(256, sizeof(T) == 2 ? 2 : 1) head_bwd_kernel(const float* __restrict__ dl, const T* __restrict__ z,
                                                         int64_t zp, const float* __restrict__ w,
                                                         T* __restrict__ dz, int64_t dzp,
@@ -383,9 +383,9 @@
   for (int i = 0; i < (STATS ? 8 : 1); ++i) t1[i] = t2[i] = 0.f;
   const float* dln = dl + static_cast<int64_t>(n) * K * HW;
   const T* zn = z + static_cast<int64_t>(n) * HW * zp + c0;
-  T* dzn = dz + static_cast<int64_t>(n) * HW * dzp + c0;
+  T* dzn = DZ ? dz + static_cast<int64_t>(n) * HW * dzp + c0 : nullptr;
   const int64_t stride = static_cast<int64_t>(gridDim.x) * L;
-  constexpr int U = STATS ? 3 : 4;
+  constexpr int U = STATS && DZ ? 3 : 4;
   for (int64_t g0 = static_cast<int64_t>(blockIdx.x) * L + threadIdx.x / C8N; g0 < HW; g0 += U * stride) {
     float d[U][K];
     Vec8<T> zv[U];
@@ -428,7 +428,7 @@
           t2[i] = fmaf(gm, yraw, t2[i]);
         }
       }
-      Vec8<T>::st(dzn + px * dzp, o);
+      if (DZ) Vec8<T>::st(dzn + px * dzp, o);
     }
   }
   const int lane = threadIdx.x & 31, warp = threadIdx.x >> 5;
@@ -681,7 +681,7 @@
                          int64_t dz_pitch, float* dw, float* db, float* workspace, int64_t workspace_bytes, int N,
                          int64_t HW, int C, int K, void* stream, const float* na = nullptr, const float* nb = nullptr,
                          float slope = 0.f, float* tpart = nullptr) {
-  B200_CHECK_ARG(dlogits_nchw && z && w && dz && dw && db && workspace, "head_bwd: null pointer");
+  B200_CHECK_ARG(dlogits_nchw && z && w && (dz || tpart) && dw && db && workspace, "head_bwd: null pointer");
   B200_CHECK_ARG(z_pitch % 8 == 0 && dz_pitch % 8 == 0, "head_bwd: pitches must be multiples of 8");
   B200_CHECK_ARG(N > 0 && N <= 65535, "head_bwd: batch must fit the grid");
   if (!(C == 32 && K == 3)) return set_error(kErrUnsupported, "head_bwd: only C=32, K=3 is built (got C=%d K=%d)", C, K);
@@ -689,7 +689,10 @@
   const int bpi = b200unet_head_bwd_stat_slots(N, HW);
   B200_CHECK_ARG(workspace_bytes >= b200unet_head_bwd_workspace(N, HW, C, K), "head_bwd: workspace too small");
   cudaStream_t st = static_cast<cudaStream_t>(stream);
-  if (tpart)
+  if (tpart && !dz)
+    launch_k(head_bwd_kernel<T, 32, 3, true, false>, dim3(bpi, N), dim3(256), 0, st, dlogits_nchw, static_cast<const T*>(z),
+             z_pitch, w, static_cast<T*>(dz), dz_pitch, workspace, HW, na, nb, slope, tpart);
+  else if (tpart)
     launch_k(head_bwd_kernel<T, 32, 3, true>, dim3(bpi, N), dim3(256), 0, st, dlogits_nchw, static_cast<const T*>(z), z_pitch, w,
                                                                   static_cast<T*>(dz), dz_pitch, workspace, HW, na, nb,
                                                                   slope, tpart);
diff --git a/unet-implementations_b200/csrc/norm.cu b/unet-implementations_b200/csrc/norm.cu
--- a/unet-implementations_b200/csrc/norm.cu
+++ b/unet-implementations_b200/csrc/norm.cu
@@ -148,6 +148,8 @@
   int C, c8n, lanes;
   int64_t chunk;
   int n0;
+  const float* dl;
+  const float* hw;
 };
 
 template <typename T, bool HAS2>
@@ -313,9 +315,11 @@
   dbeta[c] = static_cast<float>(db);
 }
 
-template <typename T, bool HAS2>
+constexpr int kHeadK = 3;
+template <typename T, bool HAS2, bool HEAD = false>
 __global__ void __launch_bounds__(kNormThreads, 2) in_bwd_apply_kernel(InBwdK<T> K, const float* __restrict__ coef,
                                                                         T* __restrict__ dy, int64_t dyp) {
+  static_assert(!(HAS2 && HEAD), "the head's unit has no skip gradient");
   pdl_launch_dependents();
   pdl_wait();
   const int n = K.n0 + blockIdx.y;
@@ -335,22 +339,34 @@
       k3[j] = fmaf(k.y, rm[j], -k.z);
     }
   }
+  float wr[HEAD ? kHeadK : 1][8];
+  if (HEAD) {
+#pragma unroll
+    for (int k = 0; k < kHeadK; ++k) ld8f(K.hw + k * K.C + c0, wr[HEAD ? k : 0]);
+  }
   const int64_t lo = blockIdx.x * K.chunk;
   int64_t hi = lo + K.chunk;
   if (hi > K.HW) hi = K.HW;
   const T* yb = K.y + static_cast<int64_t>(n) * K.HW * K.yp + c0;
-  const T* db = K.dz + static_cast<int64_t>(n) * K.HW * K.dzp + c0;
+  const T* db = HEAD ? nullptr : K.dz + static_cast<int64_t>(n) * K.HW * K.dzp + c0;
   const T* d2b = HAS2 ? K.dz2 + static_cast<int64_t>(n) * K.HW * K.dz2p + c0 : nullptr;
+  const float* dlb = HEAD ? K.dl + static_cast<int64_t>(n) * kHeadK * K.HW : nullptr;
   T* ob = dy + static_cast<int64_t>(n) * K.HW * dyp + c0;
   const int lanes = K.lanes;
   constexpr int U = 4;
   for (int64_t px = lo + lane; px < hi; px += U * lanes) {
-    Vec8<T> vy[U], vd[U], vd2[HAS2 ? U : 1];
+    Vec8<T> vy[U], vd[HEAD ? 1 : U], vd2[HAS2 ? U : 1];
+    float vl[HEAD ? U : 1][kHeadK];
 #pragma unroll
     for (int u = 0; u < U; ++u)
       if (px + u * lanes < hi) {
         vy[u] = Vec8<T>::ld_stream(yb + (px + u * lanes) * K.yp);
-        vd[u] = Vec8<T>::ld_stream(db + (px + u * lanes) * K.dzp);
+        if (HEAD) {
+#pragma unroll
+          for (int k = 0; k < kHeadK; ++k) vl[HEAD ? u : 0][k] = __ldg(dlb + k * K.HW + px + u * lanes);
+        } else {
+          vd[HEAD ? 0 : u] = Vec8<T>::ld_stream(db + (px + u * lanes) * K.dzp);
+        }
         if (HAS2) vd2[HAS2 ? u : 0] = Vec8<T>::ld_stream(d2b + (px + u * lanes) * K.dz2p);
       }
 #pragma unroll
@@ -358,7 +374,17 @@
       if (px + u * lanes >= hi) break;
       float yv[8], d[8], o[8];
       vy[u].unpack(yv);
-      vd[u].unpack(d);
+      if (HEAD) {
+#pragma unroll
+        for (int j = 0; j < 8; ++j) {
+          float sacc = 0.f;
+#pragma unroll
+          for (int k = 0; k < kHeadK; ++k) sacc = fmaf(wr[HEAD ? k : 0][j], vl[HEAD ? u : 0][k], sacc);
+          d[j] = to_f32(from_f32<T>(sacc));
+        }
+      } else {
+        vd[HEAD ? 0 : u].unpack(d);
+      }
       if (HAS2) {
         float d2[8];
         vd2[HAS2 ? u : 0].unpack(d2);
@@ -581,7 +607,7 @@
 
 template <typename T>
 static int in_backward_impl(const b200unet_in_bwd_args* A, void* stream) {
-  B200_CHECK_ARG(A && A->dz && A->y && A->a && A->b && A->mean && A->rstd && A->gamma && A->dy && A->dgamma &&
+  B200_CHECK_ARG(A && (A->dz || A->head_dl) && A->y && A->a && A->b && A->mean && A->rstd && A->gamma && A->dy && A->dgamma &&
                      A->dbeta && A->workspace,
                  "in_backward: null pointer");
   int rc = check_nhwc("in_backward", A->C, A->dz_pitch, A->dz2 ? A->dz2_pitch : 0, A->y_pitch);
@@ -592,6 +618,13 @@
   B200_CHECK_ARG(A->workspace_bytes >= b200unet_in_backward_workspace(N, HW, C), "in_backward: workspace too small");
   cudaStream_t st = static_cast<cudaStream_t>(stream);
   const bool has2 = A->dz2 != nullptr;
+  const bool head = A->head_dl != nullptr;
+  if (head) {
+    B200_CHECK_ARG(A->head_w && !A->dz && !has2 && A->ext_part,
+                   "in_backward: head_dl needs head_w and the head backward's sums, and takes no dz / dz2");
+    if (!(C == 32 && A->head_K == kHeadK))
+      return set_error(kErrUnsupported, "in_backward: head_dl: only C=32, K=3 is built (got C=%d K=%d)", C, A->head_K);
+  }
   const PixelMap m = make_map(C);
   const int ipc = bwd_images_per_chunk(N, HW, C, has2);
   const int64_t chunk = pixels_per_block(HW, ipc, m, blocks_per_sm());
@@ -616,6 +649,8 @@
   K.c8n = m.c8n;
   K.lanes = m.lanes;
   K.chunk = chunk;
+  K.dl = A->head_dl;
+  K.hw = A->head_w;
   const size_t red_bytes = static_cast<size_t>(m.threads) * 16 * sizeof(typename AccT<T>::type);
   const double inv_hw = 1.0 / static_cast<double>(HW);
   if constexpr (sizeof(T) == 2) {
@@ -657,7 +692,10 @@
     }
     B200_LAUNCH_CHECK("in_bwd_finalize_kernel");
     K.chunk = chunk_apply;
-    if (has2)
+    if (head)
+      launch_k(in_bwd_apply_kernel<T, false, true>, dim3((unsigned)ceil_div64(HW, chunk_apply), nn), dim3(m.threads), 0, st,
+          K, coef, static_cast<T*>(A->dy), A->dy_pitch);
+    else if (has2)
       launch_k(in_bwd_apply_kernel<T, true>, dim3((unsigned)ceil_div64(HW, chunk_apply), nn), dim3(m.threads), 0, st, 
           K, coef, static_cast<T*>(A->dy), A->dy_pitch);
     else
diff --git a/unet-implementations_b200/csrc/resample.cu b/unet-implementations_b200/csrc/resample.cu
--- a/unet-implementations_b200/csrc/resample.cu
+++ b/unet-implementations_b200/csrc/resample.cu
@@ -3,6 +3,15 @@
 #include "vec8.cuh"
 
 namespace b200 {
+
+__device__ __forceinline__ void cp_async16(void* smem, const void* gmem) {
+  asm volatile("cp.async.cg.shared.global [%0], [%1], 16;" ::"r"(smem_u32(smem)), "l"(gmem) : "memory");
+}
+
+template <typename T>
+static size_t up_fwd_smem(int R, int c8n) {
+  return static_cast<size_t>(R + 2) * (256 / c8n + 2) * c8n * 8 * sizeof(T);
+}
 
 template <typename T, int R>
 __global__ void __launch_bounds__(256, 2) upsample2x_fwd_kernel(const T* __restrict__ x, int64_t xp,
@@ -11,29 +20,50 @@
                                                                  const float* __restrict__ nb, float slope) {
   pdl_launch_dependents();
   pdl_wait();
-  const int t = blockIdx.x * 256 + threadIdx.x;
-  const int iw = t >> c8shift;
+  extern __shared__ __align__(16) unsigned char up_tile_raw[];
+  T* tile = reinterpret_cast<T*>(up_tile_raw);
+  constexpr int kChunk = 16 / sizeof(T);
+  const int C = c8n << 3;
+  const int ncols = 256 >> c8shift;
+  const int iw0 = blockIdx.x * ncols;
+  const int ih0 = blockIdx.y * R, n = blockIdx.z;
+  const T* b = x + static_cast<int64_t>(n) * H * W * xp;
+  {
+    const int row_chunks = ((ncols + 2) * C) / kChunk;
+    const int cshift = c8shift + (sizeof(T) == 2 ? 0 : 1);
+#pragma unroll
+    for (int k = 0; k < R + 2; ++k) {
+      const int ih = min(max(ih0 - 1 + k, 0), H - 1);
+      const T* rp = b + static_cast<int64_t>(ih) * W * xp;
+      T* trow = tile + static_cast<int64_t>(k) * (ncols + 2) * C;
+      for (int i = threadIdx.x; i < row_chunks; i += 256) {
+        const int j = i >> cshift, q = i & ((1 << cshift) - 1);
+        const int iw = min(max(iw0 - 1 + j, 0), W - 1);
+        cp_async16(trow + j * C + q * kChunk, rp + static_cast<int64_t>(iw) * xp + q * kChunk);
+      }
+    }
+    asm volatile("cp.async.commit_group;\n cp.async.wait_group 0;" ::: "memory");
+  }
+  __syncthreads();
+  const int jl = threadIdx.x >> c8shift;
+  const int iw = iw0 + jl;
   if (iw >= W) return;
-  const int c0 = (t & (c8n - 1)) << 3;
-  const int ih0 = blockIdx.y * R, n = blockIdx.z;
-  const int wm = iw > 0 ? iw - 1 : 0, wp = iw < W - 1 ? iw + 1 : W - 1;
-  const T* b = x + static_cast<int64_t>(n) * H * W * xp + c0;
-  const int64_t om = static_cast<int64_t>(wm) * xp, oc = static_cast<int64_t>(iw) * xp, od = static_cast<int64_t>(wp) * xp;
+  const int c0 = (threadIdx.x & (c8n - 1)) << 3;
   float ra[8], rb[8];
   if (na) {
-    const int C = c8n << 3;
     const float4* pa = reinterpret_cast<const float4*>(na + n * C + c0);
     const float4* pb = reinterpret_cast<const float4*>(nb + n * C + c0);
     const float4 a0 = __ldg(pa), a1 = __ldg(pa + 1), b0 = __ldg(pb), b1 = __ldg(pb + 1);
     ra[0] = a0.x; ra[1] = a0.y; ra[2] = a0.z; ra[3] = a0.w; ra[4] = a1.x; ra[5] = a1.y; ra[6] = a1.z; ra[7] = a1.w;
     rb[0] = b0.x; rb[1] = b0.y; rb[2] = b0.z; rb[3] = b0.w; rb[4] = b1.x; rb[5] = b1.y; rb[6] = b1.z; rb[7] = b1.w;
   }
-  auto hmix = [&](int row, float (&Lo)[8], float (&Ro)[8]) {
-    const T* rp = b + static_cast<int64_t>(row) * W * xp;
+  const T* tb = tile + jl * C + c0;
+  auto hmix = [&](int k, float (&Lo)[8], float (&Ro)[8]) {
+    const T* rp = tb + k * (ncols + 2) * C;
     float a[8], c[8], d[8];
-    Vec8<T>::ldg(rp + om).unpack(a);
-    Vec8<T>::ldg(rp + oc).unpack(c);
-    Vec8<T>::ldg(rp + od).unpack(d);
+    Vec8<T>::lds(rp).unpack(a);
+    Vec8<T>::lds(rp + C).unpack(c);
+    Vec8<T>::lds(rp + 2 * C).unpack(d);
     if (na) {
 #pragma unroll
       for (int j = 0; j < 8; ++j) {
@@ -50,8 +80,8 @@
     }
   };
   float L[3][8], Rr[3][8];
-  hmix(ih0 > 0 ? ih0 - 1 : 0, L[0], Rr[0]);
-  hmix(ih0, L[1], Rr[1]);
+  hmix(0, L[0], Rr[0]);
+  hmix(1, L[1], Rr[1]);
   const int OW = 2 * W;
   T* o = out + (static_cast<int64_t>(n) * 2 * H + 2 * ih0) * OW * op + static_cast<int64_t>(2 * iw) * op + c0;
   const int64_t orow = static_cast<int64_t>(OW) * op;
@@ -61,7 +91,7 @@
     if (ih >= H) break;
     float (&Lp)[8] = L[r % 3], (&Lc)[8] = L[(r + 1) % 3], (&Ln)[8] = L[(r + 2) % 3];
     float (&Rp)[8] = Rr[r % 3], (&Rc)[8] = Rr[(r + 1) % 3], (&Rn)[8] = Rr[(r + 2) % 3];
-    hmix(ih < H - 1 ? ih + 1 : H - 1, Ln, Rn);
+    hmix(r + 2, Ln, Rn);
     float v[8];
 #pragma unroll
     for (int j = 0; j < 8; ++j) v[j] = 0.75f * Lc[j] + 0.25f * Lp[j];
@@ -79,49 +109,66 @@
   }
 }
 
-constexpr int kUpRows = 4;
-
-template <typename T>
+template <typename T>
+static size_t up_bwd_smem(int R, int c8n) {
+  return static_cast<size_t>(2 * R + 2) * (512 / c8n + 2) * c8n * 8 * sizeof(T);
+}
+
+template <typename T, int R>
 __global__ void __launch_bounds__(256) upsample2x_bwd_kernel(const T* __restrict__ dout, int64_t dp,
                                                               T* __restrict__ dx, int64_t xp, int H, int W,
                                                               int c8n, int c8shift) {
   pdl_launch_dependents();
   pdl_wait();
-  const int t = blockIdx.x * 256 + threadIdx.x;
-  const int iw = t >> c8shift;
+  extern __shared__ __align__(16) unsigned char up_tile_raw[];
+  T* tile = reinterpret_cast<T*>(up_tile_raw);
+  constexpr int kChunk = 16 / sizeof(T);
+  const int C = c8n << 3;
+  const int ncols = 256 >> c8shift;
+  const int tcols = 2 * ncols + 2;
+  const int iw0 = blockIdx.x * ncols;
+  const int ih0 = blockIdx.y * R, n = blockIdx.z;
+  const int OH = 2 * H, OW = 2 * W;
+  const T* b = dout + static_cast<int64_t>(n) * OH * OW * dp;
+  {
+    const int row_chunks = (tcols * C) / kChunk;
+    const int cshift = c8shift + (sizeof(T) == 2 ? 0 : 1);
+#pragma unroll
+    for (int k = 0; k < 2 * R + 2; ++k) {
+      const int oh = min(max(2 * ih0 - 1 + k, 0), OH - 1);
+      const T* rp = b + static_cast<int64_t>(oh) * OW * dp;
+      T* trow = tile + static_cast<int64_t>(k) * tcols * C;
+      for (int i = threadIdx.x; i < row_chunks; i += 256) {
+        const int j = i >> cshift, q = i & ((1 << cshift) - 1);
+        const int ow = min(max(2 * iw0 - 1 + j, 0), OW - 1);
+        cp_async16(trow + j * C + q * kChunk, rp + static_cast<int64_t>(ow) * dp + q * kChunk);
+      }
+    }
+    asm volatile("cp.async.commit_group;\n cp.async.wait_group 0;" ::: "memory");
+  }
+  __syncthreads();
+  const int jl = threadIdx.x >> c8shift;
+  const int iw = iw0 + jl;
   if (iw >= W) return;
-  const int c0 = (t & (c8n - 1)) << 3;
-  const int ih0 = blockIdx.y * kUpRows, n = blockIdx.z;
-  const int OH = 2 * H, OW = 2 * W;
-  const T* b = dout + static_cast<int64_t>(n) * OH * OW * dp + c0;
-  int cols[4];
-#pragma unroll
-  for (int a = 0; a < 4; ++a) {
-    const int ow = 2 * iw - 1 + a;
-    cols[a] = ow < 0 ? 0 : (ow >= OW ? OW - 1 : ow);
-  }
-  float acc[kUpRows][8];
-#pragma unroll
-  for (int r = 0; r < kUpRows; ++r)
+  const int c0 = (threadIdx.x & (c8n - 1)) << 3;
+  const T* tb = tile + 2 * jl * C + c0;
+  float acc[R][8];
+#pragma unroll
+  for (int r = 0; r < R; ++r)
 #pragma unroll
     for (int j = 0; j < 8; ++j) acc[r][j] = 0.f;
 #pragma unroll
-  for (int k = 0; k < 2 * kUpRows + 2; ++k) {
-    const int oh_u = 2 * ih0 - 1 + k;
-    const int oh = oh_u < 0 ? 0 : (oh_u >= OH ? OH - 1 : oh_u);
-    const T* rp = b + static_cast<int64_t>(oh) * OW * dp;
-    Vec8<T> raw[4];
-#pragma unroll
-    for (int bb = 0; bb < 4; ++bb) raw[bb] = Vec8<T>::ldg(rp + static_cast<int64_t>(cols[bb]) * dp);
+  for (int k = 0; k < 2 * R + 2; ++k) {
+    const T* rp = tb + k * tcols * C;
     float d0[8], d1[8], d2[8], d3[8], hs[8];
-    raw[0].unpack(d0);
-    raw[1].unpack(d1);
-    raw[2].unpack(d2);
-    raw[3].unpack(d3);
+    Vec8<T>::lds(rp).unpack(d0);
+    Vec8<T>::lds(rp + C).unpack(d1);
+    Vec8<T>::lds(rp + 2 * C).unpack(d2);
+    Vec8<T>::lds(rp + 3 * C).unpack(d3);
 #pragma unroll
     for (int j = 0; j < 8; ++j) hs[j] = 0.25f * (d0[j] + d3[j]) + 0.75f * (d1[j] + d2[j]);
 #pragma unroll
-    for (int r = 0; r < kUpRows; ++r) {
+    for (int r = 0; r < R; ++r) {
       const int a = k - 2 * r;
       if (a >= 0 && a < 4) {
         const float wgt = (a == 0 || a == 3) ? 0.25f : 0.75f;
@@ -131,7 +178,7 @@
     }
   }
 #pragma unroll
-  for (int r = 0; r < kUpRows; ++r) {
+  for (int r = 0; r < R; ++r) {
     const int ih = ih0 + r;
     if (ih < H) Vec8<T>::st(dx + ((static_cast<int64_t>(n) * H + ih) * W + iw) * xp + c0, acc[r]);
   }
@@ -182,17 +229,19 @@
   pdl_launch_dependents();
   pdl_wait();
   const int n = blockIdx.y;
-  const int64_t p = static_cast<int64_t>(blockIdx.x) * 256 + threadIdx.x;
-  if (p >= HW) return;
-  float f[8];
-#pragma unroll
-  for (int c = 0; c < 8; ++c) f[c] = c < C ? __ldg(src + (static_cast<int64_t>(n) * C + c) * HW + p) : 0.f;
-  uint4* o = reinterpret_cast<uint4*>(dst + (static_cast<int64_t>(n) * HW + p) * 32);
-  o[0] = make_uint4(pack_bf16x2(f[0], f[1]), pack_bf16x2(f[2], f[3]), pack_bf16x2(f[4], f[5]), pack_bf16x2(f[6], f[7]));
-  const uint4 z = make_uint4(0u, 0u, 0u, 0u);
-  o[1] = z;
-  o[2] = z;
-  o[3] = z;
+  const int q = threadIdx.x & 3;
+  const int64_t p = static_cast<int64_t>(blockIdx.x) * 64 + (threadIdx.x >> 2);
+  const bool live = p < HW;
+  const float* s = src + (static_cast<int64_t>(n) * C + 2 * q) * HW + p;
+  const float f0 = (live && 2 * q < C) ? __ldg(s) : 0.f;
+  const float f1 = (live && 2 * q + 1 < C) ? __ldg(s + HW) : 0.f;
+  const uint32_t u = pack_bf16x2(f0, f1);
+  const uint32_t u1 = __shfl_down_sync(0xffffffffu, u, 1);
+  const uint32_t u2 = __shfl_down_sync(0xffffffffu, u, 2);
+  const uint32_t u3 = __shfl_down_sync(0xffffffffu, u, 3);
+  if (!live) return;
+  uint4* o = reinterpret_cast<uint4*>(dst + (static_cast<int64_t>(n) * HW + p) * 32) + q;
+  *o = q == 0 ? make_uint4(u, u1, u2, u3) : make_uint4(0u, 0u, 0u, 0u);
 }
 
 }
@@ -213,13 +262,23 @@
   const int c8n = C / 8, sh = ilog2_exact(c8n);
   B200_CHECK_ARG(sh >= 0, "upsample2x_fwd: C/8 = %d must be a power of two", c8n);
   B200_CHECK_ARG(H <= 65535 && N <= 65535, "upsample2x_fwd: H and N must fit the grid");
+  B200_CHECK_ARG(c8n <= 256, "upsample2x_fwd: C = %d must be at most 2048", C);
   const dim3 block(256);
-#define B200_UP_LAUNCH(RR)                                                                                             \
-  launch_k(upsample2x_fwd_kernel<T, RR>, dim3(ceil_div(W * c8n, 256), ceil_div(H, RR), N), block, 0,                     \
-           static_cast<cudaStream_t>(stream), static_cast<const T*>(x), x_pitch, static_cast<T*>(out), out_pitch, H, W,  \
-           c8n, sh, na, nb, slope)
-  if (H >= 64) B200_UP_LAUNCH(8);
-  else B200_UP_LAUNCH(2);
+  static size_t attr_bytes[2] = {0, 0};
+#define B200_UP_LAUNCH(RR, I)                                                                                          \
+  do {                                                                                                                 \
+    const size_t smem = up_fwd_smem<T>(RR, c8n);                                                                       \
+    if (smem > attr_bytes[I]) {                                                                                        \
+      B200_CUDA(cudaFuncSetAttribute(upsample2x_fwd_kernel<T, RR>, cudaFuncAttributeMaxDynamicSharedMemorySize,        \
+                                     static_cast<int>(smem)));                                                         \
+      attr_bytes[I] = smem;                                                                                            \
+    }                                                                                                                  \
+    launch_k(upsample2x_fwd_kernel<T, RR>, dim3(ceil_div(W * c8n, 256), ceil_div(H, RR), N), block, smem,              \
+             static_cast<cudaStream_t>(stream), static_cast<const T*>(x), x_pitch, static_cast<T*>(out), out_pitch, H,  \
+             W, c8n, sh, na, nb, slope);                                                                               \
+  } while (0)
+  if (H >= 64 && up_fwd_smem<T>(8, c8n) <= 200 * 1024) B200_UP_LAUNCH(8, 0);
+  else B200_UP_LAUNCH(2, 1);
 #undef B200_UP_LAUNCH
   B200_LAUNCH_CHECK("upsample2x_fwd_kernel");
   return 0;
@@ -233,8 +292,23 @@
   const int c8n = C / 8, sh = ilog2_exact(c8n);
   B200_CHECK_ARG(sh >= 0, "upsample2x_bwd: C/8 = %d must be a power of two", c8n);
   B200_CHECK_ARG(H <= 65535 && N <= 65535, "upsample2x_bwd: H and N must fit the grid");
-  launch_k(upsample2x_bwd_kernel<T>, dim3(ceil_div(W * c8n, 256), ceil_div(H, kUpRows), N), dim3(256), 0, static_cast<cudaStream_t>(stream), 
-      static_cast<const T*>(dout), dout_pitch, static_cast<T*>(dx), dx_pitch, H, W, c8n, sh);
+  B200_CHECK_ARG(c8n <= 256, "upsample2x_bwd: C = %d must be at most 2048", C);
+  static size_t attr_bytes[2] = {0, 0};
+#define B200_UPB_LAUNCH(RR, I)                                                                                         \
+  do {                                                                                                                 \
+    const size_t smem = up_bwd_smem<T>(RR, c8n);                                                                       \
+    if (smem > attr_bytes[I]) {                                                                                        \
+      B200_CUDA(cudaFuncSetAttribute(upsample2x_bwd_kernel<T, RR>, cudaFuncAttributeMaxDynamicSharedMemorySize,        \
+                                     static_cast<int>(smem)));                                                         \
+      attr_bytes[I] = smem;                                                                                            \
+    }                                                                                                                  \
+    launch_k(upsample2x_bwd_kernel<T, RR>, dim3(ceil_div(W * c8n, 256), ceil_div(H, RR), N), dim3(256), smem,          \
+             static_cast<cudaStream_t>(stream), static_cast<const T*>(dout), dout_pitch, static_cast<T*>(dx), dx_pitch, \
+             H, W, c8n, sh);                                                                                           \
+  } while (0)
+  if (up_bwd_smem<T>(4, c8n) <= 200 * 1024) B200_UPB_LAUNCH(4, 0);
+  else B200_UPB_LAUNCH(1, 1);
+#undef B200_UPB_LAUNCH
   B200_LAUNCH_CHECK("upsample2x_bwd_kernel");
   return 0;
 }
@@ -299,7 +373,7 @@
 extern "C" int b200unet_image_to_nhwc32_bf16(const float* src, void* dst, int N, int C, int64_t HW, void* stream) {
   B200_CHECK_ARG(src && dst, "image_to_nhwc32_bf16: null pointer");
   B200_CHECK_ARG(C >= 1 && C <= 8 && N <= 65535, "image_to_nhwc32_bf16: C must be in [1,8]");
-  launch_k(image_to_nhwc32_kernel, dim3((unsigned)ceil_div64(HW, 256), N), dim3(256), 0, static_cast<cudaStream_t>(stream), 
+  launch_k(image_to_nhwc32_kernel, dim3((unsigned)ceil_div64(HW, 64), N), dim3(256), 0, static_cast<cudaStream_t>(stream),
       src, static_cast<__nv_bfloat16*>(dst), C, HW);
   B200_LAUNCH_CHECK("image_to_nhwc32_kernel");
   return 0;
diff --git a/unet-implementations_b200/csrc/vec8.cuh b/unet-implementations_b200/csrc/vec8.cuh
--- a/unet-implementations_b200/csrc/vec8.cuh
+++ b/unet-implementations_b200/csrc/vec8.cuh
@@ -19,6 +19,11 @@
   __device__ __forceinline__ static Vec8 ldg(const __nv_bfloat16* p) {
     Vec8 v;
     v.r = __ldg(reinterpret_cast<const uint4*>(p));
+    return v;
+  }
+  __device__ __forceinline__ static Vec8 lds(const __nv_bfloat16* p) {
+    Vec8 v;
+    v.r = *reinterpret_cast<const uint4*>(p);
     return v;
   }
   __device__ __forceinline__ void unpack(float (&f)[8]) const {
@@ -44,6 +49,12 @@
     Vec8 v;
     v.a = __ldg(reinterpret_cast<const float4*>(p));
     v.b = __ldg(reinterpret_cast<const float4*>(p) + 1);
+    return v;
+  }
+  __device__ __forceinline__ static Vec8 lds(const float* p) {
+    Vec8 v;
+    v.a = reinterpret_cast<const float4*>(p)[0];
+    v.b = reinterpret_cast<const float4*>(p)[1];
     return v;
   }
   __device__ __forceinline__ void unpack(float (&f)[8]) const {
diff --git a/unet-implementations_b200/models/unet.py b/unet-implementations_b200/models/unet.py
--- a/unet-implementations_b200/models/unet.py
+++ b/unet-implementations_b200/models/unet.py
@@ -636,10 +636,13 @@
     if dlogits.dtype != torch.float32:
         dlogits = dlogits.float()
     ext_part = None
+    head_dz = None
     if model.head_kind == "seg1x1":
         if ctx.head_norm is not None and model.producer_sums:
             dz, dwh, dbh, ext_part = ops.head_backward(dlogits, ctx.z_last, head.weight, norm=ctx.head_norm,
-                                                       out_dw=dest(head.weight), out_db=dest(head.bias), want_bwd_part=True)
+                                                       out_dw=dest(head.weight), out_db=dest(head.bias), want_bwd_part=True,
+                                                       want_dz=btrace is not None)
+            head_dz = (dlogits, head.weight)
         else:
             dz, dwh, dbh = ops.head_backward(dlogits, ctx.z_last, head.weight, norm=ctx.head_norm, out_dw=dest(head.weight),
                                              out_db=dest(head.bias))
@@ -706,10 +709,17 @@
         if dgd is None or dbd is None:
             dgd = dbd = None
         defer = overlap and (wants(norm.weight) or wants(norm.bias))
-        res = ops.in_backward(dz, dz2, rec["y"], rec["a"], rec["b"], rec["mean"], rec["rstd"], rec["scale"],
-                              norm.weight, rec["slope"], out_dgamma=dgd, out_dbeta=dbd,
-                              ext_part=ext_part if dz2 is None else None, defer_params=defer)
+        if head_dz is not None:
+            assert dz2 is None
+            res = ops.in_backward(None, None, rec["y"], rec["a"], rec["b"], rec["mean"], rec["rstd"], rec["scale"],
+                                  norm.weight, rec["slope"], out_dgamma=dgd, out_dbeta=dbd, ext_part=ext_part,
+                                  defer_params=defer, head=head_dz)
+        else:
+            res = ops.in_backward(dz, dz2, rec["y"], rec["a"], rec["b"], rec["mean"], rec["rstd"], rec["scale"],
+                                  norm.weight, rec["slope"], out_dgamma=dgd, out_dbeta=dbd,
+                                  ext_part=ext_part if dz2 is None else None, defer_params=defer)
         ext_part = None
+        head_dz = None
         rec_y = rec["y"]
         rec["y"] = None
         collect()
diff --git a/unet-implementations_b200/ops.py b/unet-implementations_b200/ops.py
--- a/unet-implementations_b200/ops.py
+++ b/unet-implementations_b200/ops.py
@@ -248,7 +248,7 @@
 
 
 def in_backward(dz, dz2, y, a, b, mean, rstd, drop_scale, gamma, slope, out_dgamma=None, out_dbeta=None,
-                ext_part=None, ext_part2=None, defer_params=False):
+                ext_part=None, ext_part2=None, defer_params=False, head=None):
     n, h, w, c = y.shape
     hw = h * w
     nbytes = _lib.call("b200unet_in_backward_workspace", n, hw, c)
@@ -259,17 +259,27 @@
     else:
         dgb = torch.empty((2, c), dtype=torch.float32, device=y.device)
     dy = torch.empty((n, h, w, c), dtype=y.dtype, device=y.device)
-    assert dz.dtype == y.dtype and (dz2 is None or dz2.dtype == y.dtype)
+    if head is not None:
+        assert dz is None and dz2 is None and ext_part is not None
+    else:
+        assert dz.dtype == y.dtype and (dz2 is None or dz2.dtype == y.dtype)
     ep, ep2 = ext_part, ext_part2
     if ep is not None:
         assert ep.dtype == torch.float32 and ep.is_contiguous() and ep.shape[0] == n and tuple(ep.shape[2:]) == (c, 2)
     if ep2 is not None:
         assert ep2.dtype == torch.float32 and ep2.is_contiguous() and ep2.shape[0] == n and tuple(ep2.shape[2:]) == (c, 2)
-    args = InBwdArgs(_p(dz), pitch_of(dz), _p(dz2), pitch_of(dz2) if dz2 is not None else 0, _p(y), pitch_of(y), _p(a),
-                     _p(b), _p(mean), _p(rstd), _p(drop_scale), _p(_f32(gamma.detach())), float(slope), _p(dy),
-                     pitch_of(dy), _p(dgb[0]), _p(dgb[1]), _p(ws), nbytes, n, hw, c,
+    hk, hdl, hwt = 0, None, None
+    if head is not None:
+        hdl, hwt = head
+        hk = hwt.shape[0]
+        hdl = _f32(hdl.contiguous())
+        assert tuple(hdl.shape) == (n, hk, h, w)
+        hwt = _f32(hwt.detach().reshape(hk, c))
+    args = InBwdArgs(_p(dz), pitch_of(dz) if dz is not None else 0, _p(dz2), pitch_of(dz2) if dz2 is not None else 0,
+                     _p(y), pitch_of(y), _p(a), _p(b), _p(mean), _p(rstd), _p(drop_scale), _p(_f32(gamma.detach())),
+                     float(slope), _p(dy), pitch_of(dy), _p(dgb[0]), _p(dgb[1]), _p(ws), nbytes, n, hw, c,
                      _p(ep), ep.shape[1] if ep is not None else 0, _p(ep2), ep2.shape[1] if ep2 is not None else 0,
-                     1 if defer_params else 0)
+                     1 if defer_params else 0, _p(hdl), _p(hwt), hk)
     _lib.call("b200unet_in_backward" + _sfx(y), ctypes.byref(args), _stream())
     if defer_params:
         def finish_params():
@@ -331,13 +341,14 @@
     return logits
 
 
-def head_backward(dlogits, z, weight, norm=None, out_dw=None, out_db=None, want_bwd_part=False):
+def head_backward(dlogits, z, weight, norm=None, out_dw=None, out_db=None, want_bwd_part=False, want_dz=True):
     n, h, w, c = z.shape
     k = weight.shape[0]
     dl = _f32(dlogits.contiguous())
     nbytes = _lib.call("b200unet_head_bwd_workspace", n, h * w, c, k)
     ws = torch.empty((nbytes // 4,), dtype=torch.float32, device=z.device)
-    dz = torch.empty((n, h, w, c), dtype=z.dtype, device=z.device)
+    assert want_dz or (norm is not None and want_bwd_part)
+    dz = torch.empty((n, h, w, c), dtype=z.dtype, device=z.device) if want_dz else None
     dw = out_dw if out_dw is not None else torch.empty((k, c, 1, 1), dtype=torch.float32, device=z.device)
     db = out_db if out_db is not None else torch.empty((k,), dtype=torch.float32, device=z.device)
     assert dw.numel() == k * c and db.numel() == k and dw.is_contiguous() and db.is_contiguous()
@@ -349,7 +360,8 @@
         slots = _lib.call("b200unet_head_bwd_stat_slots", n, h * w)
         part = torch.empty((n, slots, c, 2), dtype=torch.float32, device=z.device)
         _lib.call("b200unet_head_norm_bwd_stats" + _sfx(z), _p(dl), _p(z), pitch_of(z), _p(a), _p(b), float(slope),
-                  _p(_f32(weight.detach().reshape(k, c))), _p(dz), pitch_of(dz), _p(dw), _p(db), _p(ws), nbytes, _p(part),
+                  _p(_f32(weight.detach().reshape(k, c))), _p(dz), pitch_of(dz) if want_dz else 0, _p(dw), _p(db), _p(ws),
+                  nbytes, _p(part),
                   n, h * w, c, k, _stream())
         return dz, dw, db, part
     else:
```

Measured after the change: 1559, median of 6. -1.8%, worse.
